# latentnetworks/vimure

Hardware: AMD Instinct MI355X
Metric: CAVI iterations/sec (L=4 N=2000 M=200 K=2 synthetic, mutuality on) (higher is better)
Workload: dtype f64

## Files before the change

include/vimure_hip.h:

```cpp
#ifndef VIMURE_HIP_H
#define VIMURE_HIP_H

#include <stdint.h>

#ifdef __cplusplus
extern "C" {
#endif

typedef struct vmr_ctx* vmr_handle;

enum {
  VMR_OK = 0,
  VMR_EINVAL = -1,
  VMR_EHIP = -2,
  VMR_ENAN = -3,
  VMR_ESTATE = -4
};

enum { VMR_STEP_GAMMA = 0, VMR_STEP_PHI = 1, VMR_STEP_RHO = 2, VMR_STEP_NU = 3 };

enum { VMR_READ_RHO_MAX = 0, VMR_READ_RHO_MEAN = 1, VMR_READ_THRESHOLD = 2 };

enum {
  VMR_KERNEL_GAMMA_MASK = 0,
  VMR_KERNEL_GAMMA_COUNTS = 1,
  VMR_KERNEL_PHI = 2,
  VMR_KERNEL_RHO = 3,
  VMR_KERNEL_ELBO = 4,
  VMR_KERNEL_FINALIZE = 5,
  VMR_KERNEL_RHO_ELBO = 6,
  VMR_KERNEL_RHO_NOSTORE = 7,
  VMR_KERNEL_COUNT = 8
};

int vmr_create(vmr_handle* out, int device, int L, int N, int M, int K, int mutuality,
               const uint8_t* X, const uint8_t* R, int data_on_device, double eps);

int vmr_create_coo(vmr_handle* out, int device, int L, int N, int M, int K, int mutuality,
                   int64_t nx, const int32_t* xl, const int32_t* xi, const int32_t* xj, const int32_t* xm, const int32_t* xv,
                   int64_t nr, const int32_t* rl, const int32_t* ri, const int32_t* rj, const int32_t* rm,
                   int data_on_device, double eps);

void vmr_destroy(vmr_handle h);

const char* vmr_last_error(vmr_handle h);

int vmr_data_stats(vmr_handle h, double* sum_x, uint8_t* coverage);

int vmr_set_priors(vmr_handle h, const double* alpha_theta, const double* beta_theta,
                   const double* alpha_lambda, const double* beta_lambda,
                   double alpha_eta, double beta_eta);

int vmr_set_state(vmr_handle h, const double* gamma_shp, const double* gamma_rte,
                  const double* phi_shp, const double* phi_rte, double nu_shp, double nu_rte,
                  const double* pr_rho, int pr_rho_on_device);

int vmr_draw_pr_rho(vmr_handle h, int nblk, const int64_t* tie_cuts, const uint32_t* mt_keys, const int32_t* mt_pos,
                    double bias0, int undirected, double* out, int out_on_device);

int vmr_step(vmr_handle h, int n_iters, double* elbo_out);

int vmr_fit_loop(vmr_handle h, int max_iter, double tol, int decision, int cap, int* n_rows, int* row_iter, double* row_elbo,
                 double* row_runtime, int* row_reached, double* elbo, int* iters, int* converged);

int vmr_fit_loop_batch(vmr_handle* hs, int n, int max_iter, double tol, int decision, int cap, int* n_rows, int* row_iter,
                       double* row_elbo, double* row_runtime, int* row_reached, double* elbo, int* iters, int* converged, int* rc);

int vmr_elbo(vmr_handle h, double* out);

int vmr_sweep_local(vmr_handle h, int want_elbo, double* out3);
int vmr_commit_nu(vmr_handle h, double nu_partial_total);

int vmr_sweep_local_dev(vmr_handle h, int want_elbo, double* out3_dev);
int vmr_commit_nu_dev(vmr_handle h, const double* nu_partial_total_dev);
void* vmr_stream(vmr_handle h);

int vmr_sub_step(vmr_handle h, int which);

int vmr_get_state(vmr_handle h, double* gamma_shp, double* gamma_rte, double* phi_shp,
                  double* phi_rte, double* nu_shp, double* nu_rte, double* rho);

int vmr_snapshot(vmr_handle h);
int vmr_restore(vmr_handle h);

int vmr_readout(vmr_handle h, int method, double threshold, void* out, int out_on_device);

int vmr_sample(vmr_handle h, uint64_t seed, int n_trials, uint8_t* out, int out_on_device);

int vmr_mean_poisson_size(vmr_handle h, int layer, uint64_t* n);
int vmr_mean_poisson(vmr_handle h, int layer, uint64_t n, int32_t* sl, int32_t* si, int32_t* sj, int32_t* sm,
                     double* vals, int out_on_device);

int vmr_report_auc(vmr_handle h, int layer, double* auc, uint64_t* n_pos, uint64_t* n_neg);

int vmr_sample_stats(vmr_handle h, uint64_t seed, int n_samples, int n_trials, const uint8_t* y_ref, int y_ref_on_device,
                     uint64_t* counts, int32_t* deg_out, int32_t* deg_in);

int vmr_expected_stats(vmr_handle h, double* out);

#define VMR_PPC_NSTAT 6
int vmr_ppc_replicates(vmr_handle h, int n_rep, uint64_t seed_y, uint64_t seed_x, int n_trials, const double* theta,
                       const double* lambda, const double* eta, uint64_t* counts, uint64_t* by_reporter);
int vmr_ppc_observed(vmr_handle h, uint64_t* counts, uint64_t* by_reporter);

enum { VMR_EDGE_REPORTED = 1, VMR_EDGE_INFERRED = 2 };
int vmr_edge_table_size(vmr_handle h, int method, double threshold, int select, int layer, uint64_t* n);
int vmr_edge_table(vmr_handle h, int method, double threshold, int select, int layer, uint64_t n,
                   int32_t* sl, int32_t* si, int32_t* sj,
                   uint8_t* y, double* prob, double* mean,
                   uint32_t* n_rep, uint64_t* total, uint32_t* n_mask, uint32_t* ego, uint32_t* alter,
                   uint8_t* y_T, uint32_t* n_rep_T, uint64_t* total_T, int out_on_device);

int vmr_get_geometric(vmr_handle h, double* g_theta, double* g_lambda, double* g_nu, double* g_nu_cache);

int vmr_sync(vmr_handle h);

int vmr_profile(vmr_handle h, int enable);
int vmr_profile_read(vmr_handle h, int kernel_class, double* total_ms, int64_t* launches);

int vmr_kernel_bytes(vmr_handle h, int kernel_class, double* bytes);

int vmr_data_format(vmr_handle h, int* sparse, uint64_t* nnz);

int vmr_mask_format(vmr_handle h, int* lists, uint64_t* listed);

int vmr_sweep_shape(vmr_handle h, int* passes, int* lds_levels, uint64_t* far_reports);

int vmr_generate_y(int device, int L, int N, int K, int C, const double* w, const int32_t* grp, uint64_t seed, uint8_t* Y_dev);
int vmr_generate_x(int device, int L, int N, int M, const uint8_t* Y_dev, const double* lam_dev, const double* theta, double eta,
                   double lambda_diff, uint64_t seed, int self_reporter, uint8_t* X_dev);

const char* vmr_version(void);

#ifdef __cplusplus
}
#endif
#endif
```

vimure_amd/_lib.py:

```python
import ctypes as C
import os

HERE = os.path.dirname(os.path.abspath(__file__))
LIB_PATH = os.environ.get("VMR_LIB", os.path.join(HERE, "libvimure_hip.so"))

VMR_OK, VMR_EINVAL, VMR_EHIP, VMR_ENAN, VMR_ESTATE = 0, -1, -2, -3, -4
STEP_GAMMA, STEP_PHI, STEP_RHO, STEP_NU = 0, 1, 2, 3
KERNEL_GAMMA_MASK, KERNEL_GAMMA_COUNTS, KERNEL_PHI, KERNEL_RHO, KERNEL_ELBO, KERNEL_FINALIZE, KERNEL_RHO_ELBO, KERNEL_RHO_NOSTORE = range(8)
READ_RHO_MAX, READ_RHO_MEAN, READ_THRESHOLD = 0, 1, 2
PPC_NSTAT = 6
EDGE_REPORTED, EDGE_INFERRED = 1, 2
PPC_STAT_NAMES = ["n_pos", "total", "sumsq", "mutual", "ties_reported", "ties_agreed"]
KERNEL_NAMES = ["gamma_mask", "gamma_counts", "phi", "rho", "elbo", "finalize", "rho_elbo", "rho_nostore"]

_dp = C.POINTER(C.c_double)
_u8p = C.c_void_p

SIGNATURES = {
    "vmr_create": (C.c_int, [C.POINTER(C.c_void_p), C.c_int, C.c_int, C.c_int, C.c_int, C.c_int, C.c_int,
                             _u8p, _u8p, C.c_int, C.c_double]),
    "vmr_create_coo": (C.c_int, [C.POINTER(C.c_void_p), C.c_int, C.c_int, C.c_int, C.c_int, C.c_int, C.c_int,
                                 C.c_int64, C.c_void_p, C.c_void_p, C.c_void_p, C.c_void_p, C.c_void_p,
                                 C.c_int64, C.c_void_p, C.c_void_p, C.c_void_p, C.c_void_p, C.c_int, C.c_double]),
    "vmr_destroy": (None, [C.c_void_p]),
    "vmr_last_error": (C.c_char_p, [C.c_void_p]),
    "vmr_data_stats": (C.c_int, [C.c_void_p, _dp, C.c_void_p]),
    "vmr_set_priors": (C.c_int, [C.c_void_p, C.c_void_p, C.c_void_p, C.c_void_p, C.c_void_p, C.c_double, C.c_double]),
    "vmr_set_state": (C.c_int, [C.c_void_p, C.c_void_p, C.c_void_p, C.c_void_p, C.c_void_p, C.c_double, C.c_double,
                                C.c_void_p, C.c_int]),
    "vmr_draw_pr_rho": (C.c_int, [C.c_void_p, C.c_int, C.c_void_p, C.c_void_p, C.c_void_p, C.c_double, C.c_int, C.c_void_p, C.c_int]),
    "vmr_step": (C.c_int, [C.c_void_p, C.c_int, _dp]),
    "vmr_elbo": (C.c_int, [C.c_void_p, _dp]),
    "vmr_fit_loop": (C.c_int, [C.c_void_p, C.c_int, C.c_double, C.c_int, C.c_int, C.POINTER(C.c_int), C.c_void_p, C.c_void_p,
                               C.c_void_p, C.c_void_p, _dp, C.POINTER(C.c_int), C.POINTER(C.c_int)]),
    "vmr_fit_loop_batch": (C.c_int, [C.POINTER(C.c_void_p), C.c_int, C.c_int, C.c_double, C.c_int, C.c_int, C.c_void_p, C.c_void_p, C.c_void_p,
                                     C.c_void_p, C.c_void_p, C.c_void_p, C.c_void_p, C.c_void_p, C.c_void_p]),
    "vmr_sub_step": (C.c_int, [C.c_void_p, C.c_int]),
    "vmr_sweep_local": (C.c_int, [C.c_void_p, C.c_int, _dp]),
    "vmr_commit_nu": (C.c_int, [C.c_void_p, C.c_double]),
    "vmr_sweep_local_dev": (C.c_int, [C.c_void_p, C.c_int, C.c_void_p]),
    "vmr_commit_nu_dev": (C.c_int, [C.c_void_p, C.c_void_p]),
    "vmr_stream": (C.c_void_p, [C.c_void_p]),
    "vmr_sample": (C.c_int, [C.c_void_p, C.c_uint64, C.c_int, C.c_void_p, C.c_int]),
    "vmr_sample_stats": (C.c_int, [C.c_void_p, C.c_uint64, C.c_int, C.c_int, C.c_void_p, C.c_int, C.c_void_p, C.c_void_p, C.c_void_p]),
    "vmr_expected_stats": (C.c_int, [C.c_void_p, C.c_void_p]),
    "vmr_ppc_replicates": (C.c_int, [C.c_void_p, C.c_int, C.c_uint64, C.c_uint64, C.c_int, C.c_void_p, C.c_void_p, C.c_void_p,
                                     C.c_void_p, C.c_void_p]),
    "vmr_ppc_observed": (C.c_int, [C.c_void_p, C.c_void_p, C.c_void_p]),
    "vmr_get_state": (C.c_int, [C.c_void_p] + [C.c_void_p] * 7),
    "vmr_get_geometric": (C.c_int, [C.c_void_p, C.c_void_p, C.c_void_p, C.c_void_p, C.c_void_p]),
    "vmr_sync": (C.c_int, [C.c_void_p]),
    "vmr_readout": (C.c_int, [C.c_void_p, C.c_int, C.c_double, C.c_void_p, C.c_int]),
    "vmr_mean_poisson_size": (C.c_int, [C.c_void_p, C.c_int, C.POINTER(C.c_uint64)]),
    "vmr_mean_poisson": (C.c_int, [C.c_void_p, C.c_int, C.c_uint64, C.c_void_p, C.c_void_p, C.c_void_p, C.c_void_p, C.c_void_p,
                                   C.c_int]),
    "vmr_report_auc": (C.c_int, [C.c_void_p, C.c_int, _dp, C.POINTER(C.c_uint64), C.POINTER(C.c_uint64)]),
    "vmr_edge_table_size": (C.c_int, [C.c_void_p, C.c_int, C.c_double, C.c_int, C.c_int, C.POINTER(C.c_uint64)]),
    "vmr_edge_table": (C.c_int, [C.c_void_p, C.c_int, C.c_double, C.c_int, C.c_int, C.c_uint64] + [C.c_void_p] * 14 + [C.c_int]),
    "vmr_snapshot": (C.c_int, [C.c_void_p]),
    "vmr_restore": (C.c_int, [C.c_void_p]),
    "vmr_profile": (C.c_int, [C.c_void_p, C.c_int]),
    "vmr_profile_read": (C.c_int, [C.c_void_p, C.c_int, _dp, C.POINTER(C.c_int64)]),
    "vmr_kernel_bytes": (C.c_int, [C.c_void_p, C.c_int, _dp]),
    "vmr_data_format": (C.c_int, [C.c_void_p, C.POINTER(C.c_int), C.POINTER(C.c_uint64)]),
    "vmr_mask_format": (C.c_int, [C.c_void_p, C.POINTER(C.c_int), C.POINTER(C.c_uint64)]),
    "vmr_sweep_shape": (C.c_int, [C.c_void_p, C.POINTER(C.c_int), C.POINTER(C.c_int), C.POINTER(C.c_uint64)]),
    "vmr_generate_y": (C.c_int, [C.c_int, C.c_int, C.c_int, C.c_int, C.c_int, C.c_void_p, C.c_void_p, C.c_uint64, C.c_void_p]),
    "vmr_generate_x": (C.c_int, [C.c_int, C.c_int, C.c_int, C.c_int, C.c_void_p, C.c_void_p, C.c_void_p, C.c_double, C.c_double,
                                 C.c_uint64, C.c_int, C.c_void_p]),
    "vmr_version": (C.c_char_p, []),
}

_lib = None


def load():
    global _lib
    if _lib is not None:
        return _lib
    if not os.path.exists(LIB_PATH):
        raise RuntimeError(
            f"{LIB_PATH} is missing: the HIP engine has not been built. Run `python -m vimure_amd.build` "
            "(needs hipcc, --offload-arch=gfx950). vimure_amd has no CPU fallback.")
    try:
        import torch
    except ImportError:
        pass
    lib = C.CDLL(LIB_PATH)
    for name, (res, args) in SIGNATURES.items():
        if os.environ.get("VMR_LIB_LAX") and not hasattr(lib, name):
            continue
        fn = getattr(lib, name)
        fn.restype = res
        fn.argtypes = args
    _lib = lib
    return lib
```

vimure_amd/csrc/sorted_lists.hip:

```cpp
#include "sweep_sl.h"

__global__ __launch_bounds__(256) void k_sl_keys(const unsigned* __restrict__ cnt, unsigned* __restrict__ keys, unsigned* __restrict__ vals, size_t T) {
  for (size_t t = (size_t)blockIdx.x * 256 + threadIdx.x; t < T; t += (size_t)gridDim.x * 256) { keys[t] = cnt[t]; vals[t] = (unsigned)t; }
}
__global__ __launch_bounds__(256) void k_sl_level_keys(unsigned* __restrict__ keys, const unsigned* __restrict__ rpl, const unsigned* __restrict__ E,
                                                       size_t T, unsigned rows0, int nb) {
  for (size_t t = (size_t)blockIdx.x * 256 + threadIdx.x; t < T; t += (size_t)gridDim.x * 256) {
    const unsigned r0 = rpl[t], n = rpl[t + 1] - r0;
    unsigned n1 = 0;
    for (unsigned r = 0; r < n; ++r) n1 += SL_YM(E[(size_t)r0 + r]) >= rows0 ? 1u : 0u;
    keys[t] = (n << nb) | n1;
  }
}
__global__ __launch_bounds__(256) void k_sl_steps(const unsigned* __restrict__ keys_sorted, const unsigned* __restrict__ vals_sorted,
                                                  unsigned* __restrict__ sz, unsigned* __restrict__ perm, size_t T, size_t NS, int nb) {
  for (size_t q = (size_t)blockIdx.x * 256 + threadIdx.x; q < NS * 64; q += (size_t)gridDim.x * 256) {
    perm[q] = q < T ? vals_sorted[q] : 0xffffffffu;
    if ((q & 63) == 0) sz[q >> 6] = 64u * (keys_sorted[q] >> nb);
  }
  if (blockIdx.x == 0 && threadIdx.x == 0) sz[NS] = 0u;
}
__global__ __launch_bounds__(256) void k_sl_place(const unsigned* __restrict__ perm, const unsigned* __restrict__ rpl ,
                                                  const unsigned* __restrict__ rsl, const unsigned* __restrict__ Ein,
                                                  unsigned* __restrict__ Eout, const unsigned* __restrict__ Ein2, unsigned* __restrict__ Eout2,
                                                  unsigned* __restrict__ syl, size_t T, size_t NS, int Mp) {
  const int lane = threadIdx.x & 63;
  for (size_t s = (size_t)blockIdx.x * 4 + (threadIdx.x >> 6); s < NS; s += (size_t)gridDim.x * 4) {
    const unsigned t = perm[s * 64 + lane];
    const bool ok = t != 0xffffffffu;
    const unsigned r0 = ok ? rpl[t] : 0u, n = ok ? rpl[t + 1] - r0 : 0u;
    const unsigned ea = rsl[s], R = (rsl[s + 1] - ea) >> 6;
    unsigned rot = 0;
    if (n > 1) { unsigned hsh = t * 0x9E3779B1u; hsh ^= hsh >> 15; hsh *= 0x85EBCA77u; hsh ^= hsh >> 13; rot = hsh % n; }
    unsigned ymx = 0;
    for (unsigned r = 0; r < R; ++r) {
      unsigned q = r + rot;
      if (q >= n) q -= n;
      const unsigned e = n > r ? Ein[(size_t)r0 + q] : 0u;
      Eout[(size_t)ea + r * 64 + lane] = e;
      if (Ein2) Eout2[(size_t)ea + r * 64 + lane] = n > r ? Ein2[(size_t)r0 + q] : 0u;
      ymx = max(ymx, (Ein2 ? e : SL_YM(e)) / (unsigned)Mp);
    }
#pragma unroll
    for (int o2 = 32; o2 > 0; o2 >>= 1) ymx = max(ymx, (unsigned)__shfl_xor((int)ymx, o2, 64));
    if (lane == 0) syl[s] = ymx;
  }
}

template <class V>
__global__ __launch_bounds__(256) void k_sl_gather(const unsigned* __restrict__ perm, const V* __restrict__ in, V* __restrict__ out,
                                                   size_t T, size_t NS, int L) {
  for (size_t q = (size_t)blockIdx.x * 256 + threadIdx.x; q < (size_t)L * T; q += (size_t)gridDim.x * 256) {
    const size_t l = q / T, pos = q - l * T;
    out[q] = in[l * T + perm[l * NS * 64 + pos]];
  }
}
__global__ __launch_bounds__(256) void k_sl_rows(const unsigned* __restrict__ perm, const double* __restrict__ in, double* __restrict__ out,
                                                 size_t T, size_t NS, int L, int K, int to_pos) {
  const size_t n = (size_t)L * T * K;
  for (size_t q = (size_t)blockIdx.x * 256 + threadIdx.x; q < n; q += (size_t)gridDim.x * 256) {
    const size_t row = q / K, k = q - row * K, l = row / T, pos = row - l * T;
    const size_t t = perm[l * NS * 64 + pos];
    if (to_pos) out[q] = in[(l * T + t) * K + k]; else out[(l * T + t) * K + k] = in[q];
  }
}

int sl_permute_u8(vmr_ctx* h, const uint8_t* in, uint8_t* out) {
  const Geo& g = h->g;
  const size_t T = (size_t)g.N * g.N, NS = (T + 63) / 64;
  hipLaunchKernelGGL(k_sl_gather<uint8_t>, dim3((unsigned)std::min<size_t>(8192, (g.L * T + 255) / 256)), dim3(256), 0, h->stream, h->perm, in, out, T, NS, g.L);
  CK(hipGetLastError());
  return VMR_OK;
}
int sl_permute_u32(vmr_ctx* h, const unsigned* in, unsigned* out) {
  const Geo& g = h->g;
  const size_t T = (size_t)g.N * g.N, NS = (T + 63) / 64;
  hipLaunchKernelGGL(k_sl_gather<unsigned>, dim3((unsigned)std::min<size_t>(8192, (g.L * T + 255) / 256)), dim3(256), 0, h->stream, h->perm, in, out, T, NS, g.L);
  CK(hipGetLastError());
  return VMR_OK;
}
int sl_permute_rows(vmr_ctx* h, const double* in, double* out, bool to_pos) {
  const Geo& g = h->g;
  const size_t T = (size_t)g.N * g.N, NS = (T + 63) / 64, n = (size_t)g.L * T * g.K;
  hipLaunchKernelGGL(k_sl_rows, dim3((unsigned)std::min<size_t>(16384, (n + 255) / 256)), dim3(256), 0, h->stream, h->perm, in, out, T, NS, g.L, g.K, to_pos ? 1 : 0);
  HIPCHK(h, hipGetLastError());
  return VMR_OK;
}

int sl_place_entries(vmr_ctx* h, unsigned* rp, const std::vector<unsigned long long>& nl, unsigned* etmp_all, unsigned* etmp2_all, const SlFill* fill) {
  Geo& g = h->g;
  const int L = g.L;
  const size_t T = (size_t)g.N * g.N, n = T + 1, NS = (T + 63) / 64;
  unsigned *keys = nullptr, *keys2 = nullptr, *vals = nullptr, *vals2 = nullptr, *bsum = nullptr, *etmp = nullptr, *etmp2 = nullptr;
  void* tmp = nullptr;
  const bool wide = g.wide != 0;
  auto cleanup = [&]() { void* p[] = {keys, keys2, vals, vals2, bsum, etmp, etmp2, tmp}; for (void* q : p) if (q) (void)hipFree(q); };
#define CKS(call) do { hipError_t e_ = (call); if (e_ != hipSuccess) { g_create_err = std::string(#call) + ": " + hipGetErrorString(e_); (void)hipGetLastError(); cleanup(); return VMR_EHIP; } } while (0)
  if (T >= 0x7fffffffull) return fail(nullptr, VMR_EINVAL, "more than 2^31 ties in one layer");
  CKS(hipMalloc(&keys, T * 4)); CKS(hipMalloc(&keys2, T * 4)); CKS(hipMalloc(&vals, T * 4)); CKS(hipMalloc(&vals2, T * 4));
  CKS(hipMalloc(&bsum, (std::max(n, NS + 1) + 2047) / 2048 * 4));
  CKS(hipMalloc(&h->rs, (size_t)L * (NS + 1) * 4));
  CKS(hipMalloc(&h->perm, (size_t)L * NS * 64 * 4));
  CKS(hipMalloc(&h->sy, (size_t)L * NS * 4));
  size_t tb = 0;
  int bits = 1;
  while (bits < 32 && (1ull << bits) <= (unsigned long long)g.M) ++bits;
  const bool level_keys_ok = !wide && g.mut && 2 * bits <= 30 && !h->opt.no_level_sort;
  CKS(hipcub::DeviceRadixSort::SortPairsDescending(nullptr, tb, keys, keys2, vals, vals2, (int)T, 0, level_keys_ok ? 2 * bits : bits, h->stream));
  CKS(hipMalloc(&tmp, tb ? tb : 8));
  const unsigned tgrid = (unsigned)std::min<size_t>(8192, (T + 255) / 256), sgrid = (unsigned)std::min<size_t>(8192, (NS + 3) / 4);
  if (!etmp_all) {
    unsigned long long nlmax = 0;
    for (int l = 0; l < L; ++l) nlmax = std::max(nlmax, nl[l]);
    CKS(hipMalloc(&etmp, ((size_t)nlmax + 64) * 4));
    if (wide) CKS(hipMalloc(&etmp2, ((size_t)nlmax + 64) * 4));
  }
  unsigned long long off1 = 0;
  for (int l = 0; l < L; ++l) {
    unsigned* rpl = rp + (size_t)l * n;
    unsigned* rsl = h->rs + (size_t)l * (NS + 1);
    const bool by_level = level_keys_ok && (double)nl[l] > (double)SL_PF * (double)T;
    const int nb = by_level ? bits : 0;
    int rc;
    hipLaunchKernelGGL(k_sl_keys, dim3(tgrid), dim3(256), 0, h->stream, rpl, keys, vals, T);
    if (by_level) {
      if ((rc = scan_u32(h, rpl, bsum, n))) { cleanup(); return rc; }
      if (!etmp_all) (*fill)(l, rpl, etmp, etmp2);
      hipLaunchKernelGGL(k_sl_level_keys, dim3(tgrid), dim3(256), 0, h->stream, keys, rpl, etmp_all ? etmp_all + off1 : etmp, T, (unsigned)g.Mp, nb);
    }
    CKS(hipcub::DeviceRadixSort::SortPairsDescending(tmp, tb, keys, keys2, vals, vals2, (int)T, 0, bits + nb, h->stream));
    hipLaunchKernelGGL(k_sl_steps, dim3((unsigned)std::min<size_t>(8192, (NS * 64 + 255) / 256)), dim3(256), 0, h->stream, keys2, vals2, rsl,
                       h->perm + (size_t)l * NS * 64, T, NS, nb);
    CKS(hipGetLastError());
    if ((rc = scan_u32(h, rsl, bsum, NS + 1)) || (!by_level && (rc = scan_u32(h, rpl, bsum, n)))) { cleanup(); return rc; }
    off1 += nl[l];
  }
  CKS(hipStreamSynchronize(h->stream));
  std::vector<unsigned> slots(L);
  for (int l = 0; l < L; ++l) CKS(hipMemcpy(&slots[l], h->rs + (size_t)l * (NS + 1) + NS, 4, hipMemcpyDeviceToHost));
  std::vector<unsigned long long> eb(L);
  h->n_slots = 0;
  for (int l = 0; l < L; ++l) {
    eb[l] = h->n_slots; h->n_slots += slots[l];
    if ((double)slots[l] < (double)nl[l]) { cleanup(); return fail(nullptr, VMR_EINVAL, "more than 2^32 report slots in one layer"); }
  }
  CKS(hipMalloc(&h->ebase, (size_t)L * 8));
  CKS(hipMemcpy(h->ebase, eb.data(), (size_t)L * 8, hipMemcpyHostToDevice));
  CKS(hipMalloc(&h->E, ((size_t)h->n_slots + SL_SLACK) * 4));
  CKS(hipMemsetAsync(h->E + h->n_slots, 0, (size_t)SL_SLACK * 4, h->stream));
  if (wide) {
    CKS(hipMalloc(&h->EX, ((size_t)h->n_slots + SL_SLACK) * 4));
    CKS(hipMemsetAsync(h->EX + h->n_slots, 0, (size_t)SL_SLACK * 4, h->stream));
  }
  unsigned long long off = 0;
  for (int l = 0; l < L; ++l) {
    unsigned* src = etmp_all ? etmp_all + off : etmp;
    unsigned* src2 = wide ? (etmp_all ? etmp2_all + off : etmp2) : nullptr;
    if (!etmp_all) (*fill)(l, rp + (size_t)l * n, etmp, etmp2);
    hipLaunchKernelGGL(k_sl_place, dim3(sgrid), dim3(256), 0, h->stream, h->perm + (size_t)l * NS * 64, rp + (size_t)l * n,
                       h->rs + (size_t)l * (NS + 1), src, h->E + eb[l], src2, wide ? h->EX + eb[l] : nullptr, h->sy + (size_t)l * NS, T, NS, g.Mp);
    off += nl[l];
  }
  CKS(hipGetLastError());
  CKS(hipStreamSynchronize(h->stream));
#undef CKS
  cleanup();
  return VMR_OK;
}

#define SL_DECL(K_) __attribute__((weak)) int vmr_sl_launch_k##K_(vmr_ctx* h, int mode, const SlShape& sh, SlArgs& a);
SL_DECL(2) SL_DECL(3) SL_DECL(4) SL_DECL(5) SL_DECL(6) SL_DECL(7) SL_DECL(8)
#define SL_DECLB(K_) __attribute__((weak)) int vmr_sl_launch_batch_k##K_(vmr_ctx* h, hipStream_t st, int mode, int allfull, const SlUnit* units, const int* blk_unit, int nblocks, int tpb, size_t smem);
SL_DECLB(2) SL_DECLB(3) SL_DECLB(4) SL_DECLB(5) SL_DECLB(6) SL_DECLB(7) SL_DECLB(8)
sl_launch_batch_fn vmr_sl_batch_launcher(int K) {
  switch (K) {
    case 2: return vmr_sl_launch_batch_k2; case 3: return vmr_sl_launch_batch_k3; case 4: return vmr_sl_launch_batch_k4; case 5: return vmr_sl_launch_batch_k5;
    case 6: return vmr_sl_launch_batch_k6; case 7: return vmr_sl_launch_batch_k7; case 8: return vmr_sl_launch_batch_k8;
    default: return nullptr;
  }
}
sl_launch_fn vmr_sl_launcher(int K) {
  switch (K) {
    case 2: return vmr_sl_launch_k2; case 3: return vmr_sl_launch_k3; case 4: return vmr_sl_launch_k4; case 5: return vmr_sl_launch_k5;
    case 6: return vmr_sl_launch_k6; case 7: return vmr_sl_launch_k7; case 8: return vmr_sl_launch_k8;
    default: return nullptr;
  }
}
```

vimure_amd/csrc/sweep_sl.h:

```cpp
#ifndef VMR_SWEEP_SL_H
#define VMR_SWEEP_SL_H

#include "vmr_internal.h"
#include <functional>

#define SL_YM(e) ((e) & 0xfffffu)
#define SL_INR(e) (((e) >> 20) & 1u)
#define SL_X(e) ((e) >> 21)
#define SL_XMAX 2047u
#define SL_YM_ROWS (1u << 20)
#define SL_PF 8
#ifndef SL_PFW
#define SL_PFW 8
#endif
constexpr int sl_pf(int K) { return K <= 2 ? SL_PF : SL_PFW; }
#define SL_SLACK (64 * 64)

struct SlArgs {
  const unsigned* E; const unsigned* rs; const unsigned long long* ebase; const unsigned* perm;
  const unsigned* sy;
  const uint8_t* cls;
  const unsigned* Qt;
  const uint64_t* Rb; const unsigned* rq; const unsigned short* Rm; const unsigned long long* rbase;
  const unsigned* rm2;
  double* rho; const double* logpr;
  const double* par; double* slotR; const double* lutg; double* Hg; double* slotF; double* slotA;
  int Gl;
  int do_hist;
  int yt, hc;
  int sum_a;
  double* nu_acc; double* elbo_dev; int commit_nu;
  int nu_stale;
  unsigned long long* det;
  int lp0;
  int farl;
  double* h0s;
  const unsigned* x0p;
  int lv0r;
  const unsigned* Ez;
  int elbo_cur;
  const double* lpd; const double* lpb;
#ifdef SL_DEBUG
  unsigned long long* dbg_t;
#endif
};

struct SlShape { int tpb, yt, hc; size_t smem; };
struct SlUnit { SlArgs a; Geo g; int blk0, nblk; };

#ifndef SL_LIGHT_UPD_K
#define SL_LIGHT_UPD_K 2
#endif
constexpr bool sl_light(int K, bool elbo, bool allfull, bool update) { return !elbo && allfull && (K <= SL_LIGHT_UPD_K || (!update && K <= 4)); }
#ifndef SL_ELBO3_K
#define SL_ELBO3_K 2
#endif
#ifndef SL_ELBO3
#define SL_ELBO3 1
#endif
constexpr int sl_tpb_max(int K, bool elbo, bool allfull, bool update = true) {
  return elbo ? ((SL_ELBO3 && K <= SL_ELBO3_K) ? 768 : (K <= 4 ? 512 : 256)) : (sl_light(K, elbo, allfull, update) ? 1024 : (K <= 3 ? 768 : (K <= 7 ? 512 : 256)));
}
constexpr int sl_tpb_max_b(int K, bool elbo, bool allfull) { return elbo ? sl_tpb_max(K, true, allfull) : (K <= 2 ? 768 : (K <= 7 ? 512 : 256)); }
constexpr int sl_wpe_b(int K, bool elbo, bool allfull) { return elbo ? ((SL_ELBO3 && K <= SL_ELBO3_K) ? 3 : (K <= 4 ? 2 : 1)) : (K <= 2 ? 3 : (K <= 7 ? 2 : 1)); }
constexpr int sl_wpe(int K, bool elbo, bool allfull, bool update = true) {
  return elbo ? ((SL_ELBO3 && K <= SL_ELBO3_K) ? 3 : (K <= 4 ? 2 : 1)) : (sl_light(K, elbo, allfull, update) ? 4 : (K <= 3 ? 3 : (K <= 7 ? 2 : 1)));
}

static inline size_t sl_smem(const Geo& g, int yt, int hc, bool update, bool elbo, bool hist) {
  const size_t lb = (size_t)g.Mp * g.K * 8;
  return (update ? (size_t)yt * lb : 0) + (hist ? (size_t)hc * lb : 0) + (size_t)g.Mp * 8 * (update ? 2 : 1) +
         (size_t)g.W * 8 + 128 + (g.ml ? lb + (size_t)g.Mp * 8 : 0) + (size_t)(64 + (elbo ? 256 : 0)) * 8 + 16;
}

typedef int (*sl_launch_fn)(vmr_ctx* h, int mode, const SlShape& sh, SlArgs& a);
sl_launch_fn vmr_sl_launcher(int K);
typedef int (*sl_launch_batch_fn)(vmr_ctx* h, hipStream_t st, int mode, int allfull, const SlUnit* units, const int* blk_unit, int nblocks,
                                  int tpb, size_t smem);
sl_launch_batch_fn vmr_sl_batch_launcher(int K);

typedef std::function<void(int l, const unsigned* rpl, unsigned* etmp, unsigned* etmp2)> SlFill;
int sl_place_entries(vmr_ctx* h, unsigned* rp, const std::vector<unsigned long long>& nl, unsigned* etmp_all, unsigned* etmp2_all, const SlFill* fill);
int sl_permute_u8(vmr_ctx* h, const uint8_t* in, uint8_t* out);
int sl_permute_u32(vmr_ctx* h, const unsigned* in, unsigned* out);
int sl_permute_rows(vmr_ctx* h, const double* in, double* out, bool to_pos);

#endif
```

vimure_amd/csrc/sweep_sl.hip:

```cpp
#include "sweep_sl.h"

#ifndef VMR_K
#error "compile with -DVMR_K=<number of categories>"
#endif
#ifndef SL_WPE
#define SL_WPE sl_wpe(2, false, true)
#endif

template <int K>
struct StepIn {
  double v[K];
  double w[K];
  unsigned cls, qt, tie;
  unsigned x0;
  unsigned e[sl_pf(K)];
};

template <int R> struct RC { static constexpr int value = R; };
template <class V> __device__ __forceinline__ const V* at_bytes(const V* p, unsigned off) {
  return reinterpret_cast<const V*>(reinterpret_cast<const char*>(p) + off);
}
template <class V> __device__ __forceinline__ V* at_bytes(V* p, unsigned off) {
  return reinterpret_cast<V*>(reinterpret_cast<char*>(p) + off);
}
__device__ __forceinline__ double rcp_nr2(double d) {
  double r = __builtin_amdgcn_rcp(d);
  r = fma(fma(-d, r, 1.0), r, r);
  return fma(fma(-d, r, 1.0), r, r);
}
#define SL_INL __attribute__((always_inline))
#ifndef SL_BATCH2
#define SL_BATCH2 8
#endif
template <int K> struct Batch { static constexpr int value = K <= 2 ? SL_BATCH2 : (K <= 4 ? 4 : 2); };

template <int K, bool UPDATE, bool ELBO, bool ALLFULL, bool STORE = true, bool DET = false, bool LPD = false>
__device__ __forceinline__ void sweep_body(const SlArgs& a, const Geo& g, const unsigned bx, const unsigned gx) {
  extern __shared__ __align__(16) unsigned char smem[];
  constexpr int PFK = sl_pf(K);
  constexpr bool LV0 = !UPDATE && !ELBO && !DET;
  constexpr bool LV0R = UPDATE && K >= 3;
  const int tid = threadIdx.x, lane = tid & 63, nthr = (int)blockDim.x;
  const int wv = __builtin_amdgcn_readfirstlane(tid >> 6), nw = nthr >> 6;
  const int Mp = g.Mp;
  const unsigned ytm = UPDATE ? (unsigned)a.yt * (unsigned)Mp : 0u;
  const unsigned hcm = a.do_hist ? (unsigned)a.hc * (unsigned)Mp : 0u;
  size_t off = 0;
  double* F = reinterpret_cast<double*>(smem + off); off += (size_t)ytm * K * 8;
  const int nHc = (int)hcm * K;
  double* Hc = reinterpret_cast<double*>(smem + off); off += (size_t)nHc * 8;
  double* Gth = reinterpret_cast<double*>(smem + off); off += (size_t)Mp * 8;
  double* Lth = reinterpret_cast<double*>(smem + off); off += UPDATE ? (size_t)Mp * 8 : 0;
  double* As = reinterpret_cast<double*>(smem + off); off += a.sum_a ? (size_t)Mp * K * 8 : 0;
  double* wsum = reinterpret_cast<double*>(smem + off); off += (size_t)g.W * 8;
  double* red = reinterpret_cast<double*>(smem + off); off += 16 * 8;
  double* xt = reinterpret_cast<double*>(smem + off); off += 64 * 8;
  double* lt = reinterpret_cast<double*>(smem + off); off += ELBO ? 256 * 8 : 0;
  double* EthL = reinterpret_cast<double*>(smem + off); off += a.rq ? (size_t)Mp * 8 : 0;
  const ParOff o = par_off(g.L, g.Mp, g.K);
  const int l = (int)bx / a.Gl, gb = (int)bx - l * a.Gl;
#ifdef SL_DEBUG
  unsigned long long* dbt = a.dbg_t ? a.dbg_t + ((size_t)bx * nw + wv) * 8 : nullptr;
  if (dbt && lane == 0) dbt[0] = wall_clock64();
#endif
  const size_t T = (size_t)g.N * g.N;
  const long long NS = (long long)((T + 63) / 64);
  const double gnu = a.par[o.sc + ((UPDATE || a.elbo_cur) ? SC_G_NU : SC_G_NU_STALE)];
  bool gz = false;
  for (int m = tid; m < Mp; m += nthr) {
    const double gv = a.par[o.G_th + (size_t)l * Mp + m];
    Gth[m] = gv;
    if (LV0 || LV0R) gz = gz || (m < g.M && gv == 0.0);
    if (UPDATE) Lth[m] = a.par[o.l_th + (size_t)l * Mp + m];
  }
  for (int q = tid; q < nHc; q += nthr) Hc[q] = 0.0;
  if (a.sum_a) for (int q = tid; q < Mp * K; q += nthr) As[q] = 0.0;
  if (a.rq) for (int m = tid; m < Mp; m += nthr) EthL[m] = m < g.M ? a.par[o.E_th + (size_t)l * Mp + m] : 0.0;
  if (UPDATE || ELBO) sp_math_tables(xt, lt, tid, nthr, ELBO);
  const double* lut = a.lutg + (size_t)l * g.W * 256;
  for (int w = tid; w < g.W; w += nthr) {
    double v = 0.0;
    for (int n = 0; n < 16; ++n) v += lut[(w * 16 + n) * 16 + 15];
    wsum[w] = v;
  }
  double Ela[K], Gla[K], Lla[K];
#pragma unroll
  for (int k = 0; k < K; ++k) { Ela[k] = a.par[o.E_la + l * K + k]; Gla[k] = a.par[o.G_la + l * K + k]; Lla[k] = a.par[o.l_la + l * K + k]; if (LV0 || LV0R) gz = gz || Gla[k] == 0.0; }
  const double eps = g.eps;
  const double sc_h = DET ? __builtin_amdgcn_ldexp(1.0, g.det_sh) : 0.0, sc_r = DET ? __builtin_amdgcn_ldexp(1.0, g.det_shr) : 0.0;
  const double sc_a = DET ? __builtin_amdgcn_ldexp(1.0, DET_SH_A) : 0.0;
  auto fxm = [](double v, double scale) SL_INL -> unsigned long long {
    return (unsigned long long)(__double_as_longlong(fma(v, scale, 6755399441055744.0)) - 0x4338000000000000ll);
  };
  auto lds_add = [&](double* p, double v, double scale) SL_INL {
    if (DET) atomicAdd(reinterpret_cast<unsigned long long*>(p), fxm(v, scale)); else atomicAdd(p, v);
  };
  const float rcp_mp = 1.0f / (float)Mp, hrcp_mp = 0.5f * rcp_mp;
  auto row_level = [&](unsigned ym) SL_INL -> unsigned { return (unsigned)__builtin_fmaf((float)ym, rcp_mp, hrcp_mp); };
  const double lp0_0 = log(1.0 + eps), lp0_k = log(eps);
  double e_lin = 0.0, e_q = 0.0, e_log = 0.0;
  double accF[K], acc0[K];
#pragma unroll
  for (int k = 0; k < K; ++k) { accF[k] = 0.0; acc0[k] = 0.0; }
  unsigned long long ie_lin = 0ull, ie_q = 0ull, ie_log = 0ull, iaccF[K];
#pragma unroll
  for (int k = 0; k < K; ++k) iaccF[k] = 0ull;
  double* Hl = a.Hg + ((size_t)l * NH + (gb % NH)) * g.Y * Mp * K;
  auto det_H = [&]() SL_INL { return a.det + (size_t)l * g.Y * Mp * K; };
  auto det_A = [&]() SL_INL { return a.det + (size_t)g.L * g.Y * Mp * K + (size_t)l * g.W * 64 * K; };
  auto det_F = [&]() SL_INL { return a.det + (size_t)g.L * g.Y * Mp * K + (size_t)g.L * g.W * 64 * K + (size_t)l * K; };
  auto det_R = [&]() SL_INL { return a.det + (size_t)g.L * g.Y * Mp * K + (size_t)g.L * g.W * 64 * K + (size_t)g.L * K; };
  const unsigned* rsl = a.rs + (size_t)l * (NS + 1);
  const unsigned* syl = a.sy + (size_t)l * NS;
  const unsigned* El = a.E + a.ebase[l];
  const unsigned* pl = (a.rm2 ? a.rm2 : a.perm) + (size_t)l * NS * 64;
  const uint8_t* cl = ALLFULL ? nullptr : a.cls + (size_t)l * T;
  const unsigned* Ql = a.Qt ? a.Qt + (size_t)l * T : nullptr;
  const uint64_t* Rl = a.Rb ? a.Rb + (size_t)l * T * g.W : nullptr;
  double* rl = a.rho + (size_t)l * T * K;
  double* rho_slack = a.rho + (size_t)g.L * T * K;
  const double* lpl = a.logpr + (size_t)l * T * K;
  constexpr bool LPDV = LPD && K == 2 && UPDATE && !ELBO;
  const double* lpdl = LPDV ? a.lpd + (size_t)l * T : nullptr;
  const double lpb0 = (K == 2 && UPDATE) ? a.lpb[2 * l] : 0.0, lpb1 = (K == 2 && UPDATE) ? a.lpb[2 * l + 1] : 0.0;
  const unsigned* rql = a.rq ? a.rq + (size_t)l * (T + 1) : nullptr;
  const unsigned short* Rml = a.rq ? a.Rm + a.rbase[l] : nullptr;
  const unsigned lim_y = UPDATE ? (a.do_hist ? (unsigned)min(a.yt, a.hc) : (unsigned)a.yt) : (a.do_hist ? (unsigned)a.hc : 0xffffffffu);
  const unsigned lim1 = (UPDATE && a.yt < g.Y) ? (unsigned)a.yt : 0xffffffffu;
  const unsigned lim2 = (a.do_hist && a.hc < g.Y) ? (unsigned)a.hc : 0xffffffffu;

  const long long Gl_ = a.Gl;
  unsigned* tick = reinterpret_cast<unsigned*>(smem + off); off += 16;
  if (tid == 0) { tick[0] = 2u * (unsigned)nw; tick[1] = 0u; }
  auto step_of = [&](unsigned t) SL_INL -> long long { return (long long)gb + (long long)t * Gl_; };
  auto draw = [&]() SL_INL -> long long {
    unsigned t = 0u;
    if (lane == 0) t = atomicAdd(tick, 1u);
    return step_of((unsigned)__builtin_amdgcn_readfirstlane((int)t));
  };
  long long s = step_of((unsigned)wv), sn = step_of((unsigned)(nw + wv));
  unsigned ea = 0;
  int R = 0;
  unsigned ymax = 0;
  unsigned rgv = 0;
  StepIn<K> P;

  const unsigned lane4 = (unsigned)lane * 4u, laneK8 = (unsigned)lane * (unsigned)(K * 8);
  const unsigned T32 = (unsigned)T;
  auto fetch_range = [&](long long st) SL_INL {
    const unsigned ra = rsl[st + (lane < 1 ? 0 : 1)], ry = syl[st];
    rgv = lane == 2 ? ry : ra;
  };
  auto fetch_tie = [&](StepIn<K>& d, long long st, const bool lp_const = false) SL_INL {
    const size_t row0 = (size_t)st * 64;
    const bool ok = (unsigned)row0 + (unsigned)lane < T32;
    d.qt = 0u; d.tie = 0u;
    if (ALLFULL) d.cls = ok ? 1u : 0u;
    else {
      const unsigned c = (unsigned)*at_bytes(cl + row0, (unsigned)lane);
      d.cls = ok ? c : 0u;
      d.tie = *at_bytes(pl + row0, lane4);
    }
    if (ELBO && Ql) d.qt = *at_bytes(Ql + row0, lane4);
    d.x0 = 0u;
    if (LV0 && a.x0p) d.x0 = *at_bytes(a.x0p + (size_t)l * NS * 64 + row0, lane4);
#pragma unroll
    for (int k = 0; k < K; ++k) { d.v[k] = 0.0; d.w[k] = 0.0; }
    if (LPDV) {
      if (lp_const) d.v[0] = lp0_k - lp0_0;
      else d.v[0] = *at_bytes(lpdl + row0, (unsigned)lane * 8u);
    } else if (UPDATE || ELBO) {
      if (lp_const) {
#pragma unroll
        for (int k = 0; k < K; ++k) d.v[k] = k == 0 ? lp0_0 : lp0_k;
      } else load_k<K>(at_bytes(lpl + row0 * K, laneK8), d.v);
    }
    if (!UPDATE && a.do_hist != 2) load_k<K>(at_bytes(static_cast<const double*>(rl) + row0 * K, laneK8), d.w);
  };
  auto fetch_ent = [&](StepIn<K>& d, unsigned base, auto cntc) SL_INL {
    constexpr int CNT = decltype(cntc)::value;
    const unsigned* pe = El + base;
#pragma unroll
    for (int j = 0; j < CNT; ++j) d.e[j] = *at_bytes(pe + j * 64, lane4);
  };

  if (s < NS) {
    ea = rsl[s];
    R = (int)((rsl[s + 1] - ea) >> 6);
    ymax = syl[s];
    fetch_range(sn < NS ? sn : s);
    fetch_tie(P, s);
    fetch_ent(P, ea, RC<PFK>{});
  }
#ifdef SL_DEBUG
  if (dbt && lane == 0) dbt[4] = wall_clock64();
#endif
  __builtin_amdgcn_s_waitcnt(0x0F70);
  bool lv0_off = false;
  if (LV0 || LV0R) lv0_off = __syncthreads_or(gz ? 1 : 0) != 0;
  else __syncthreads();
#ifdef SL_DEBUG
  if (dbt && lane == 0) dbt[5] = wall_clock64();
#endif
  const double gnu_f = a.par[o.sc + (a.nu_stale ? SC_G_NU_STALE : SC_G_NU)];
  if (UPDATE) {
    for (int q = tid; q < (int)ytm; q += nthr) {
      const int y = q / Mp, m = q - y * Mp;
#pragma unroll
      for (int k = 0; k < K; ++k) F[q * K + k] = (m < g.M) ? f_entry(g.mut, Lth[m], Gth[m], Lla[k], Gla[k], gnu_f, y) : 0.0;
    }
    __syncthreads();
  }
  double Tfull = 0.0;
  for (int w = 0; w < g.W; ++w) Tfull += wsum[w];
#ifdef SL_DEBUG
  if (dbt && lane == 0) dbt[1] = wall_clock64();
#endif

  auto add_lists = [&](unsigned t, bool on, const double (&rr)[K]) SL_INL {
    if (a.rm2) {
#pragma unroll
      for (int h_ = 0; h_ < 2; ++h_) {
        const unsigned m = h_ ? (t >> 16) : (t & 0xffffu);
        const bool v = on && m != 0xffffu;
        const unsigned long long vm = __ballot(v);
        if (vm == 0ull) continue;
        const int m0 = __builtin_amdgcn_readlane((int)m, __builtin_ctzll(vm));
        if (__all(!v || (int)m == m0)) {
#pragma unroll
          for (int k = 0; k < K; ++k) {
            const double sm_ = wave_sum(v ? rr[k] : 0.0);
            if (lane == 0) lds_add(&As[m0 * K + k], sm_, sc_a);
          }
        } else if (v) {
#pragma unroll
          for (int k = 0; k < K; ++k) lds_add(&As[m * K + k], rr[k], sc_a);
        }
      }
      return;
    }
    unsigned q0 = 0, q1 = 0;
    if (on) { q0 = rql[t]; q1 = rql[t + 1]; }
    for (unsigned i = 0;; ++i) {
      const bool v = q0 + i < q1;
      const unsigned long long vm = __ballot(v);
      if (vm == 0ull) break;
      const int m = v ? (int)Rml[q0 + i] : -1;
      const int m0 = __builtin_amdgcn_readlane(m, __builtin_ctzll(vm));
      if (__all(!v || m == m0)) {
#pragma unroll
        for (int k = 0; k < K; ++k) {
          const double sm_ = wave_sum(v ? rr[k] : 0.0);
          if (lane == 0) lds_add(&As[m0 * K + k], sm_, sc_a);
        }
      } else if (v) {
#pragma unroll
        for (int k = 0; k < K; ++k) lds_add(&As[m * K + k], rr[k], sc_a);
      }
    }
  };
  auto mask_sum = [&](unsigned cls, unsigned tie) SL_INL -> double {
    if (ALLFULL) return Tfull;
    double Tt = 0.0;
    if (cls == 1u) Tt = Tfull;
    else if (cls == 2u && a.rm2) {
      const unsigned m0 = tie & 0xffffu, m1 = tie >> 16;
      Tt = (m0 != 0xffffu ? EthL[m0] : 0.0) + (m1 != 0xffffu ? EthL[m1] : 0.0);
    } else if (cls == 2u && rql) {
      const unsigned q0 = rql[tie], q1 = rql[tie + 1];
      for (unsigned q = q0; q < q1; ++q) Tt += EthL[Rml[q]];
    } else if (cls == 2u) {
      const uint64_t* rwt = Rl + (size_t)tie * g.W;
      for (int w = 0; w < g.W; ++w) {
        uint64_t bits = rwt[w];
        if (bits == ~0ull) { Tt += wsum[w]; continue; }
        for (int n = 0; bits != 0; ++n, bits >>= 4) Tt += lut[((w * 16 + n) << 4) + (unsigned)(bits & 15u)];
      }
    }
    return Tt;
  };
  const double gnu_cur = a.par[o.sc + SC_G_NU];
  auto w2_at = [&](unsigned ym, int k) SL_INL -> double {
    const unsigned y = row_level(ym);
    const double z2 = gnu_cur * (double)y, den = Gth[ym - y * (unsigned)Mp] * Gla[k] + z2;
    return (y == 0u || den == 0.0) ? 0.0 : z2 / den;
  };
  auto f_far = [&](unsigned ym, double (&f)[K]) SL_INL {
    const unsigned y = row_level(ym);
    const unsigned m = ym - y * (unsigned)Mp;
    const double lt = Lth[m], gt = Gth[m];
#pragma unroll
    for (int k = 0; k < K; ++k) f[k] = f_entry(g.mut, lt, gt, Lla[k], Gla[k], gnu_f, (int)y);
  };
  auto elbo_inner = [&](unsigned ent, const double (&er)[2]) SL_INL -> double {
    const unsigned ym = SL_YM(ent);
    const unsigned y = row_level(ym);
    const double z2 = gnu * (double)y, gt = Gth[ym - y * (unsigned)Mp];
    const double inner = fma(gt, er[0], z2 * er[1]);
    return (SL_INR(ent) ? inner : 0.0) + eps;
  };
  auto walk1_near = [&](const unsigned* e, auto npc, double (&U)[K]) SL_INL {
    constexpr int NP = decltype(npc)::value, BT = Batch<K>::value;
#pragma unroll
    for (int j0 = 0; j0 < NP; j0 += BT) {
      double f[BT][K];
#pragma unroll
      for (int u = 0; u < BT; ++u) {
        if (j0 + u < NP) {
#pragma unroll
          for (int k = 0; k < K; ++k) f[u][k] = F[SL_YM(e[j0 + u]) * K + k];
        }
      }
#pragma unroll
      for (int u = 0; u < BT; ++u) {
        if (j0 + u < NP) {
          const double dx = (double)SL_X(e[j0 + u]);
#pragma unroll
          for (int k = 0; k < K; ++k) U[k] = fma(dx, f[u][k], U[k]);
        }
      }
    }
  };
  auto walk2_near = [&](const unsigned* e, auto npc, const double (&r)[K], const double (&er)[2]) SL_INL {
#ifndef SL_LG
#define SL_LG 2
#endif
    constexpr int NP = decltype(npc)::value, LG = SL_LG;
#pragma unroll
    for (int j0 = 0; j0 < NP; j0 += LG) {
      double in_[LG];
#pragma unroll
      for (int u = 0; u < LG; ++u) {
        if (j0 + u < NP) {
          const unsigned ym = SL_YM(e[j0 + u]);
          const double dx = (double)SL_X(e[j0 + u]);
          if (a.do_hist) {
#pragma unroll
            for (int k = 1; k < K; ++k) lds_add(&Hc[(unsigned)k * hcm + ym], dx * r[k], sc_h);
          }
          if (ELBO) in_[u] = elbo_inner(e[j0 + u], er);
        }
      }
      if (ELBO) {
#pragma unroll
        for (int u = 0; u < LG; ++u) if (j0 + u < NP) {
          const double term = (double)SL_X(e[j0 + u]) * log_tab(in_[u], lt);
          if (DET) ie_log += fxm(term, sc_r); else e_log += term;
        }
        __builtin_amdgcn_sched_barrier(0);
      }
    }
  };
  auto deficit = [&](unsigned ent, double dfc) SL_INL {
    lds_add(&Hc[SL_YM(ent)], (double)SL_X(ent) * dfc, sc_h);
  };
  auto compute = [&](auto rct, const StepIn<K>& cur, const size_t row0, const bool act, const unsigned ea_c, const int Rr, const unsigned sy_word) SL_INL {
    const unsigned ymax = sy_word & 0xffffu, nf = a.farl ? sy_word >> 16 : 0x7fffffffu;
    const unsigned n1 = (LV0 && a.h0s && !lv0_off) ? sy_word >> 16 : 0x7fffffffu;
    constexpr int RCT = decltype(rct)::value;
    constexpr int NP = RCT < 0 ? PFK : RCT;
    const unsigned cls = cur.cls, qt = cur.qt, tie = cur.tie;
    const unsigned* pe = El + ea_c;
    auto rounds = [&](auto gbc, auto&& use, const int Rr) SL_INL {
      constexpr int GB = decltype(gbc)::value;
      unsigned rg[PFK];
#pragma unroll
      for (int i = 0; i < PFK; ++i) rg[i] = i < Rr ? cur.e[i] : 0u;
      for (int j0 = 0; j0 < Rr; j0 += PFK) {
#pragma unroll
        for (int gi = 0; gi < PFK; gi += GB) {
          unsigned c[GB];
#pragma unroll
          for (int u = 0; u < GB; ++u) {
            c[u] = rg[gi + u];
            const int jn = j0 + gi + u + PFK;
            rg[gi + u] = *at_bytes(jn < Rr ? pe + (size_t)jn * 64 : a.Ez, lane4);
          }
          if (j0 + gi < Rr) use(c, (unsigned)(j0 + gi));
        }
      }
    };
    double r[K], er[2] = {0.0, 0.0};
#pragma unroll
    for (int k = 0; k < K; ++k) r[k] = act ? cur.w[k] : 0.0;
    if (a.do_hist == 2) {
#pragma unroll
      for (int k = 0; k < K; ++k) r[k] = (k == 1) ? 1.0 : 0.0;
    }
    double Tt = 0.0;
    if (UPDATE || ELBO) Tt = mask_sum(cls, tie);
    double dfc = 0.0;
    bool irr = false;

    if (UPDATE) {
      double U[K];
#pragma unroll
      for (int k = 0; k < K; ++k) U[k] = 0.0;
#ifdef SL_DEBUG
      if (g.dbg & 16) {} else
#endif
      if (RCT >= 0) walk1_near(cur.e, RC<NP>{}, U);
      else {
        constexpr int GB = Batch<K>::value < 4 ? Batch<K>::value : 4;
        const unsigned n1u = (LV0R && a.lv0r && !lv0_off) ? sy_word >> 16 : 0x7fffffffu;
        double sl0 = 0.0, sx1 = 0.0;
        rounds(RC<GB>{}, [&](const unsigned (&c)[GB], const unsigned j) SL_INL {
          if (LV0R && j >= n1u) {
            double l0[GB];
#pragma unroll
            for (int u = 0; u < GB; ++u) l0[u] = Lth[SL_YM(c[u])];
#pragma unroll
            for (int u = 0; u < GB; ++u) { const double dx = (double)SL_X(c[u]); sl0 = fma(dx, l0[u], sl0); sx1 += dx; }
            return;
          }
          if (ymax < lim1 || j >= nf) { walk1_near(c, RC<GB>{}, U); return; }
          double f[GB][K];
          bool fr[GB];
#pragma unroll
          for (int u = 0; u < GB; ++u) {
            const unsigned ym = SL_YM(c[u]);
            fr[u] = ym >= ytm;
#pragma unroll
            for (int k = 0; k < K; ++k) f[u][k] = F[(fr[u] ? 0u : ym) * K + k];
          }
#pragma unroll
          for (int u = 0; u < GB; ++u) {
            const double dx = fr[u] ? 0.0 : (double)SL_X(c[u]);
#pragma unroll
            for (int k = 0; k < K; ++k) U[k] = fma(dx, f[u][k], U[k]);
          }
#pragma unroll
          for (int u = 0; u < GB; ++u) {
            if (__any(fr[u])) {
              if (fr[u]) {
                double ff[K];
                f_far(SL_YM(c[u]), ff);
                const double dx = (double)SL_X(c[u]);
#pragma unroll
                for (int k = 0; k < K; ++k) U[k] = fma(dx, ff[k], U[k]);
              }
            }
          }
        }, Rr);
        if (LV0R && a.lv0r && !lv0_off) {
#pragma unroll
          for (int k = 0; k < K; ++k) U[k] += fma(Lla[k], sx1, sl0);
        }
      }
      double aa[K];
      bool done = false;
      if (K == 2) {
        double c[K];
#pragma unroll
        for (int k = 0; k < K; ++k) c[k] = fma(-Tt, Ela[k], U[k]);
        const double d = ((LPDV ? cur.v[0] : cur.v[K - 1] - cur.v[0]) + c[K - 1]) - c[0];
        bool safe = fabs(c[0]) + lpb0 < 700.0 && fabs(c[K - 1]) + lpb1 < 700.0 && fabs(d) < 700.0;
        if (!__all(safe)) {
          double v[K];
#pragma unroll
          for (int k = 0; k < K; ++k) v[k] = cur.v[k];
          if (LPDV) load_k<K>(at_bytes(lpl + row0 * K, laneK8), v);
#pragma unroll
          for (int k = 0; k < K; ++k) aa[k] = v[k] + c[k];
          safe = fabs(aa[0]) < 700.0 && fabs(aa[K - 1]) < 700.0 && fabs(d) < 700.0;
        }
        if (__all(safe)) {
          const double e = exp_tab(d, xt);
          r[0] = rcp_nr2(1.0 + e);
          r[K - 1] = e * r[0];
          done = true;
        }
      } else {
#pragma unroll
        for (int k = 0; k < K; ++k) aa[k] = (cur.v[k] + U[k]) - Tt * Ela[k];
      }
      if (!done) {
        double sum = 0.0;
        bool tame = true;
#pragma unroll
        for (int k = 0; k < K; ++k) tame = tame && fabs(aa[k]) < 700.0;
        tame = __all(tame);
        if (tame) {
#pragma unroll
          for (int k = 0; k < K; ++k) r[k] = exp_tab(aa[k], xt);
        } else {
#pragma unroll
          for (int k = 0; k < K; ++k) r[k] = exp(aa[k]);
        }
#pragma unroll
        for (int k = 0; k < K; ++k) sum += r[k];
        if (sum > 0.0) {
#pragma unroll
          for (int k = 0; k < K; ++k) r[k] /= sum;
        }
        if (a.do_hist) {
          double sm = 0.0;
#pragma unroll
          for (int k = 0; k < K; ++k) sm += r[k];
          dfc = 1.0 - sm;
          if (fabs(dfc) <= 1e-14 || !act) dfc = 0.0;
          irr = __any(dfc != 0.0);
          if (irr && lane == 0) tick[1] = 1u;
        }
      }
      if (STORE) store_k<K>(act ? at_bytes(rl + row0 * K, laneK8) : at_bytes(rho_slack, laneK8), r);
      if (act && (ALLFULL || cls == 1u)) {
#pragma unroll
        for (int k = 0; k < K; ++k) { if (DET) iaccF[k] += fxm(r[k], sc_a); else accF[k] += r[k]; }
      }
      if (!ALLFULL && a.sum_a) add_lists(tie, act && cls == 2u, r);
    } else if (a.do_hist) {
      double sm = 0.0;
#pragma unroll
      for (int k = 0; k < K; ++k) sm += r[k];
      dfc = 1.0 - sm;
      if (fabs(dfc) <= 1e-14 || !act) dfc = 0.0;
      irr = __any(dfc != 0.0);
      if (irr && lane == 0) tick[1] = 1u;
      if (!ELBO && a.do_hist == 1 && act && (ALLFULL || cls == 1u)) {
#pragma unroll
        for (int k = 0; k < K; ++k) { if (DET) iaccF[k] += fxm(r[k], sc_a); else accF[k] += r[k]; }
      }
      if (!ALLFULL && !ELBO && a.sum_a) add_lists(tie, act && cls == 2u, r);
    }
    if (ELBO) {
#pragma unroll
      for (int k = 0; k < K; ++k) { const double ek = exp_tab(r[k], xt); er[0] = fma(ek, Gla[k], er[0]); er[1] += ek; }
    }
#ifdef SL_DEBUG
    if (g.dbg & 32) {} else
#endif
    if (a.do_hist || ELBO) {
      if (RCT >= 0) {
        walk2_near(cur.e, RC<NP>{}, r, er);
        if (irr) {
#pragma unroll
          for (int j = 0; j < NP; ++j) deficit(cur.e[j], dfc);
        }
      } else {
        const bool skip0 = LV0 && a.x0p != nullptr && a.do_hist == 1 && n1 != 0x7fffffffu && !irr;
        const int Rw = skip0 ? min(Rr, (int)n1) : Rr;
        double sx0 = skip0 ? (double)cur.x0 : 0.0;
        rounds(RC<1>{}, [&](const unsigned (&c1)[1], const unsigned j) SL_INL {
          const unsigned c = c1[0], ym = SL_YM(c), x = SL_X(c);
          const bool far_round = j < nf && lim2 != 0xffffffffu;
          const bool fr = far_round && ym >= hcm;
          const double dx = (double)x;
          if (LV0 && a.do_hist && j >= n1) {
            sx0 += dx;
            if (irr) lds_add(&Hc[ym], dx * dfc, sc_h);
          } else if (a.do_hist) {
            if (!fr) {
              if (!(skip0 && ym < (unsigned)Mp)) {
#pragma unroll
                for (int k = 1; k < K; ++k) lds_add(&Hc[(unsigned)k * hcm + ym], dx * r[k], sc_h);
              }
              if (irr) lds_add(&Hc[ym], dx * dfc, sc_h);
            }
            if (far_round && !a.farl && __any(fr)) {
              if (fr && x != 0u) {
                if (DET) {
                  unsigned long long* d0 = a.det;
                  asm volatile("" : "+s"(d0));
                  unsigned long long* d = d0 + (size_t)l * g.Y * Mp * K + (size_t)ym * K;
#pragma unroll
                  for (int k = 1; k < K; ++k) atomicAdd(&d[k], fxm((double)x * r[k], sc_h));
                  if (dfc != 0.0) atomicAdd(&d[0], fxm((double)x * dfc, sc_h));
                } else {
                  double* d = Hl + (size_t)ym * K;
#pragma unroll
                  for (int k = 1; k < K; ++k) atomicAdd(&d[k], (double)x * r[k]);
                  if (dfc != 0.0) atomicAdd(&d[0], (double)x * dfc);
                }
              }
              asm volatile("" ::: "memory");
            }
          }
          if (ELBO) { const double term = (double)x * log_tab(elbo_inner(c, er), lt); if (DET) ie_log += fxm(term, sc_r); else e_log += term; }
        }, Rw);
        if (LV0 && a.h0s && a.do_hist == 1 && act) {
#pragma unroll
          for (int k = 1; k < K; ++k) acc0[k] = fma(r[k], sx0, acc0[k]);
        }
      }
    }
    if (ELBO && act) {
      double sr = 0.0, se = 0.0, en = 0.0;
#pragma unroll
      for (int k = 0; k < K; ++k) {
        sr += r[k]; se += r[k] * Ela[k];
        en += r[k] * cur.v[k] - r[k] * log_tab(r[k] + eps, lt);
      }
      if (DET) { ie_lin += det_fx(en - se * Tt, g.det_shr); if (Ql) ie_q += det_fx(sr * (double)qt, g.det_shr); }
      else { e_lin += en - se * Tt; if (Ql) e_q += sr * (double)qt; }
    }
  };
  auto body = [&](auto rct) SL_INL {
    constexpr int RCT = decltype(rct)::value;
    constexpr int NP = RCT < 0 ? PFK : RCT;
    const size_t row0 = (size_t)s * 64;
    const bool act = (unsigned)row0 + (unsigned)lane < T32;
    const unsigned ea_c = ea;
    const int Rr = RCT < 0 ? R : RCT;
    const StepIn<K> cur = P;
    const long long s2 = sn, s3 = draw();
    const bool more = s2 < NS;
    const unsigned ea2 = more ? (unsigned)__builtin_amdgcn_readlane((int)rgv, 0) : ea_c;
    const int R2 = more ? (int)(((unsigned)__builtin_amdgcn_readlane((int)rgv, 1) - ea2) >> 6) : 0;
    const unsigned ym2 = more ? (unsigned)__builtin_amdgcn_readlane((int)rgv, 2) : 0u;
    fetch_range(s3 < NS ? s3 : s);
    fetch_tie(P, more ? s2 : s, RCT == 0 && a.lp0 != 0);
    if (RCT >= 0 || PFK <= 8) fetch_ent(P, ea2, RC<NP>{});
    else {
      const unsigned* pe = El + ea2;
#pragma unroll
      for (int j0 = 0; j0 < PFK; j0 += 8) {
        if (j0 == 0 || j0 < R2) {
#pragma unroll
          for (int j = j0; j < j0 + 8; ++j) P.e[j] = *at_bytes(pe + j * 64, lane4);
        }
      }
    }
    compute(rct, cur, row0, act, ea_c, Rr, ymax);
    constexpr int NST = (UPDATE && STORE) ? (K % 2 == 0 ? K / 2 : K) : 0;
    static_assert(NST <= 8, "vmcnt immediate below");
    if (RCT >= 0) __builtin_amdgcn_s_waitcnt(0x0F70 | NST);
    else __builtin_amdgcn_s_waitcnt(0x0F70);
    s = s2; sn = s3; ea = ea2; R = R2; ymax = ym2;
  };
  auto run = [&](auto rct) SL_INL {
    constexpr int RCT = decltype(rct)::value;
    do { body(rct); } while (s < NS && R == RCT && (ymax & 0xffffu) < lim_y);
  };
  while (s < NS) {
    if (R > SL_PF || (ymax & 0xffffu) >= lim_y) { body(RC<-1>{}); continue; }
    switch (R) {
      case 0: run(RC<0>{}); break;
      case 1: run(RC<1>{}); break;
      case 2: run(RC<2>{}); break;
      case 3: run(RC<3>{}); break;
      case 4: run(RC<4>{}); break;
      case 5: run(RC<5>{}); break;
      case 6: run(RC<6>{}); break;
      case 7: run(RC<7>{}); break;
      default: run(RC<8>{}); break;
    }
  }

#ifdef SL_DEBUG
  if (dbt && lane == 0) dbt[2] = wall_clock64();
#endif
  const bool nu_here = a.nu_acc && a.do_hist == 1;
  if (nu_here) asm volatile("s_waitcnt vmcnt(0)" ::: "memory");
  __syncthreads();
  if (nu_here) {
    double a0p = 0.0;
    for (int q = (tick[1] ? 0 : (int)hcm) + tid; q < nHc; q += nthr) {
      const double v = DET ? det_back(reinterpret_cast<const unsigned long long*>(Hc)[q], g.det_sh) : Hc[q];
      if (v != 0.0) {
        const int k = q / (int)hcm;
        const unsigned ym = (unsigned)(q - k * (int)hcm);
        a0p += ((k ? w2_at(ym, k) : 0.0) - w2_at(ym, 0)) * v;
      }
    }
    a0p = block_sum_n(a0p, red);
    if (tid == 0) {
      if (DET) atomicAdd(&det_R()[4], det_fx(a0p, g.det_sh)); else atomicAdd(&a.nu_acc[0], a0p);
    }
  }
#ifdef SL_DEBUG
  if (dbt && lane == 0) dbt[6] = wall_clock64();
#endif
  const int f0 = (nu_here && nw > 1) ? 64 : 0;
#ifdef SL_DEBUG
  if (g.dbg & 8) {} else
#endif
  if (a.do_hist && tid >= f0) {
    for (int q = (tick[1] ? 0 : (int)hcm) + tid - f0; q < nHc; q += nthr - f0) {
      if (DET) {
        const unsigned long long iv = reinterpret_cast<const unsigned long long*>(Hc)[q];
        if (iv != 0ull) { const int k = q / (int)hcm, ym = q - k * (int)hcm; atomicAdd(&det_H()[(size_t)ym * K + k], iv); }
        continue;
      }
      const double v = Hc[q];
      if (v != 0.0) {
        const int k = q / (int)hcm, ym = q - k * (int)hcm;
        atomicAdd(&Hl[(size_t)ym * K + k], v);
      }
    }
  }
  if (a.sum_a && tid >= f0) {
    double* out = a.slotA + ((size_t)l * NSLOT + (gb % NSLOT)) * (size_t)g.W * 64 * K;
    for (int q = tid - f0; q < g.M * K; q += nthr - f0) {
      if (DET) { const unsigned long long iv = reinterpret_cast<const unsigned long long*>(As)[q]; if (iv != 0ull) atomicAdd(&det_A()[q], iv); continue; }
      const double v = As[q];
      if (v != 0.0) atomicAdd(&out[q], v);
    }
  }
#ifdef SL_DEBUG
  if (dbt && lane == 0) dbt[7] = wall_clock64();
#endif
  if (nu_here) {
    __shared__ int nu_last;
    if (tid == 0) {
      asm volatile("s_waitcnt vmcnt(0)" ::: "memory");
      const double t = atomicAdd(&a.nu_acc[1], 1.0);
      nu_last = (t == (double)(gx - 1u));
      if (nu_last) __builtin_amdgcn_fence(__ATOMIC_ACQUIRE, "agent");
      asm volatile("s_waitcnt vmcnt(0)" ::: "memory");
    }
    __syncthreads();
    if (nu_last && a.farl) {
      if (tid == 0) a.nu_acc[1] = 0.0;
    } else if (nu_last) {
      double far = 0.0;
      const size_t hcs = (size_t)g.Y * Mp * K;
      const int y0 = max(1, a.hc);
      if (a.hc < g.Y) {
        for (int ll = 0; ll < g.L; ++ll) {
          const double* H0 = a.Hg + (size_t)ll * NH * hcs;
          const double* gthl = a.par + o.G_th + (size_t)ll * Mp;
          for (int it = y0 * Mp + tid; it < g.Y * Mp; it += nthr) {
            const int y = it / Mp, m = it - y * Mp;
            double v0[NH], vk[NH][K > 1 ? K - 1 : 1];
#pragma unroll
            for (int c = 0; c < NH; ++c) {
              v0[c] = H0[(size_t)c * hcs + (size_t)it * K];
#pragma unroll
              for (int k = 1; k < K; ++k) vk[c][k - 1] = H0[(size_t)c * hcs + (size_t)it * K + k];
            }
            if (DET) {
              const unsigned long long* hi = a.det + (size_t)ll * hcs + (size_t)it * K;
              v0[0] += det_back(hi[0], g.det_sh);
#pragma unroll
              for (int k = 1; k < K; ++k) vk[0][k - 1] += det_back(hi[k], g.det_sh);
            }
            double h_[K];
#pragma unroll
            for (int k = 0; k < K; ++k) h_[k] = 0.0;
#pragma unroll
            for (int c = 0; c < NH; ++c) {
              h_[0] += v0[c];
#pragma unroll
              for (int k = 1; k < K; ++k) h_[k] += vk[c][k - 1];
            }
            bool any = h_[0] != 0.0;
#pragma unroll
            for (int k = 1; k < K; ++k) any = any || h_[k] != 0.0;
            if (any && m < g.M) {
              const double z2 = gnu_cur * (double)y, gt = gthl[m];
              const double d0 = gt * a.par[o.G_la + ll * K] + z2, w0 = d0 == 0.0 ? 0.0 : z2 / d0;
              far -= w0 * h_[0];
#pragma unroll
              for (int k = 1; k < K; ++k) {
                const double dk = gt * a.par[o.G_la + ll * K + k] + z2;
                far += ((dk == 0.0 ? 0.0 : z2 / dk) - w0) * h_[k];
              }
            }
          }
        }
      }
      far = block_sum_n(far, red);
      if (tid == 0) {
        double tot = far;
        if (DET) { unsigned long long* dR = det_R(); tot += det_back(atomicAdd(&dR[4], 0ull), g.det_sh); dR[4] = 0ull; } else tot += atomicAdd(&a.nu_acc[0], 0.0);
        for (int ll = 0; ll < g.L; ++ll) tot += a.nu_acc[2 + ll];
        a.nu_acc[0] = 0.0; a.nu_acc[1] = 0.0;
        a.elbo_dev[1] = tot;
        if (a.commit_nu) {
          double* sc = const_cast<double*>(a.par) + o.sc;
          sc[SC_G_NU_STALE] = sc[SC_G_NU];
          sc[SC_NU_SHP] = sc[SC_A_ETA] + tot;
          sc[SC_G_NU] = exp(digamma_pos(sc[SC_NU_SHP]) - log(sc[SC_NU_RTE]));
          sc[SC_E_NU] = sc[SC_NU_SHP] / sc[SC_NU_RTE];
        }
      }
    }
  }
  auto wave_isum = [&](unsigned long long v) SL_INL -> unsigned long long {
#pragma unroll
    for (int o2 = 32; o2 > 0; o2 >>= 1) {
      const unsigned lo = (unsigned)__shfl_xor((int)(unsigned)v, o2, 64), hi = (unsigned)__shfl_xor((int)(unsigned)(v >> 32), o2, 64);
      v += ((unsigned long long)hi << 32) | lo;
    }
    return v;
  };
  if ((UPDATE || (!ELBO && a.do_hist == 1)) && a.slotF) {
#pragma unroll
    for (int k = 0; k < K; ++k) {
      if (DET) { const unsigned long long v = wave_isum(iaccF[k]); if (lane == 0 && v != 0ull) atomicAdd(&det_F()[k], v); continue; }
      double v = block_sum_n(accF[k], red);
      if (tid == 0) atomicAdd(&a.slotF[((size_t)l * NSLOT + (gb % NSLOT)) * K + k], v);
    }
  }
  if (LV0 && a.h0s && a.do_hist == 1) {
#pragma unroll
    for (int k = 1; k < K; ++k) {
      const double v = block_sum_n(acc0[k], red);
      if (tid == 0 && v != 0.0) atomicAdd(&a.h0s[((size_t)l * NSLOT + (gb % NSLOT)) * K + k], v);
    }
  }
  if (ELBO) {
    if (DET) {
      const unsigned long long v1 = wave_isum(ie_lin), v2 = wave_isum(ie_log), v3 = wave_isum(ie_q);
      if (lane == 0) { unsigned long long* dR = det_R(); atomicAdd(&dR[1], v1); atomicAdd(&dR[2], v2); atomicAdd(&dR[3], v3); }
    } else {
      double v1 = block_sum_n(e_lin, red);
      double v2 = block_sum_n(e_log, red);
      double v3 = block_sum_n(e_q, red);
      if (tid == 0) {
        double* out = a.slotR + (size_t)(bx % NSLOT) * 4;
        atomicAdd(&out[1], v1); atomicAdd(&out[2], v2); atomicAdd(&out[3], v3);
      }
    }
  }
#ifdef SL_DEBUG
  if (dbt && lane == 0) dbt[3] = wall_clock64();
#endif
}

#define SL_BOUNDS(K, UPDATE, ELBO, ALLFULL) \
  __launch_bounds__(sl_tpb_max(K, ELBO, ALLFULL, UPDATE), (K == 2 && !ELBO && ALLFULL) ? SL_WPE : sl_wpe(K, ELBO, ALLFULL, UPDATE))
template <int K, bool UPDATE, bool ELBO, bool ALLFULL, bool STORE = true, bool DET = false, bool LPD = false>
__global__ SL_BOUNDS(K, UPDATE, ELBO, ALLFULL) void k_sweep_sl(SlArgs a, Geo g) {
  sweep_body<K, UPDATE, ELBO, ALLFULL, STORE, DET, LPD>(a, g, blockIdx.x, gridDim.x);
}
template <int K, bool UPDATE, bool ELBO, bool ALLFULL, bool STORE = true, bool LPD = false>
__global__ __launch_bounds__(sl_tpb_max_b(K, ELBO, ALLFULL), sl_wpe_b(K, ELBO, ALLFULL)) void k_sweep_sl_b(const SlUnit* __restrict__ units, const int* __restrict__ blk_unit) {
  const SlUnit& u = units[blk_unit[blockIdx.x]];
  sweep_body<K, UPDATE, ELBO, ALLFULL, STORE, false, LPD>(u.a, u.g, blockIdx.x - (unsigned)u.blk0, (unsigned)u.nblk);
}

template <bool UPDATE, bool ELBO, bool ALLFULL, bool STORE = true, bool DET = false, bool LPD = false>
static int sl_launch_one_(vmr_ctx* h, const SlShape& sh, SlArgs& a) {
  constexpr int K = VMR_K;
  const Geo& g = h->g;
  const long long NS = ((long long)g.N * g.N + 63) / 64, nw = sh.tpb / 64;
  int rc = grid_per_layer(h, k_sweep_sl<K, UPDATE, ELBO, ALLFULL, STORE, DET, LPD>, sh.smem, &a.Gl, (NS + nw - 1) / nw, sh.tpb);
  if (rc) return rc;
#ifdef SL_DEBUG
  static unsigned long long* dbg_buf = nullptr;
  const char* tf = h->opt.debug_times[0] ? h->opt.debug_times : nullptr;
  const size_t nwv = (size_t)g.L * a.Gl * nw;
  a.dbg_t = nullptr;
  if (tf) {
    if (!dbg_buf) (void)hipMalloc(&dbg_buf, (size_t)1 << 22);
    if (nwv * 64 <= ((size_t)1 << 22)) a.dbg_t = dbg_buf;
  }
#endif
  hipLaunchKernelGGL((k_sweep_sl<K, UPDATE, ELBO, ALLFULL, STORE, DET, LPD>), dim3(g.L * a.Gl), dim3(sh.tpb), sh.smem, h->stream, a, g);
#ifdef SL_DEBUG
  if (a.dbg_t) {
    std::vector<unsigned long long> t(nwv * 8);
    (void)hipStreamSynchronize(h->stream);
    (void)hipMemcpy(t.data(), dbg_buf, nwv * 64, hipMemcpyDeviceToHost);
    if (FILE* f = fopen(tf, "a")) {
      fprintf(f, "launch %d%d hist %d waves %zu tpb %d\n", (int)UPDATE, (int)ELBO, a.do_hist, nwv, sh.tpb);
      for (size_t i = 0; i < nwv; ++i) fprintf(f, "%llu %llu %llu %llu %llu %llu %llu %llu\n", t[i * 8], t[i * 8 + 1], t[i * 8 + 2], t[i * 8 + 3], t[i * 8 + 4], t[i * 8 + 5], t[i * 8 + 6], t[i * 8 + 7]);
      fclose(f);
    }
  }
#endif
  return VMR_OK;
}

template <bool UPDATE, bool ELBO, bool ALLFULL, bool STORE = true, bool DET = false>
static int sl_launch_one(vmr_ctx* h, const SlShape& sh, SlArgs& a) {
  if (VMR_K == 2 && UPDATE && !ELBO && a.lpd) return sl_launch_one_<UPDATE, ELBO, ALLFULL, STORE, DET, VMR_K == 2 && UPDATE && !ELBO>(h, sh, a);
  return sl_launch_one_<UPDATE, ELBO, ALLFULL, STORE, DET>(h, sh, a);
}

#define SL_CAT2(a, b) a##b
#define SL_CAT(a, b) SL_CAT2(a, b)
int SL_CAT(vmr_sl_launch_k, VMR_K)(vmr_ctx* h, int mode, const SlShape& sh, SlArgs& a) {
  if (a.det) {
    if (a.cls == nullptr) {
      switch (mode) {
        case 0: return sl_launch_one<true, false, true, true, true>(h, sh, a);
        case 4: return sl_launch_one<true, false, true, false, true>(h, sh, a);
        case 1: return sl_launch_one<true, true, true, true, true>(h, sh, a);
        case 2: return sl_launch_one<false, true, true, true, true>(h, sh, a);
        default: return sl_launch_one<false, false, true, true, true>(h, sh, a);
      }
    }
    switch (mode) {
      case 0: return sl_launch_one<true, false, false, true, true>(h, sh, a);
      case 4: return sl_launch_one<true, false, false, false, true>(h, sh, a);
      case 1: return sl_launch_one<true, true, false, true, true>(h, sh, a);
      case 2: return sl_launch_one<false, true, false, true, true>(h, sh, a);
      default: return sl_launch_one<false, false, false, true, true>(h, sh, a);
    }
  }
  if (a.cls == nullptr) {
    switch (mode) {
      case 0: return sl_launch_one<true, false, true>(h, sh, a);
      case 1: return sl_launch_one<true, true, true>(h, sh, a);
      case 2: return sl_launch_one<false, true, true>(h, sh, a);
      case 4: return sl_launch_one<true, false, true, false>(h, sh, a);
      default: return sl_launch_one<false, false, true>(h, sh, a);
    }
  }
  switch (mode) {
    case 0: return sl_launch_one<true, false, false>(h, sh, a);
    case 1: return sl_launch_one<true, true, false>(h, sh, a);
    case 2: return sl_launch_one<false, true, false>(h, sh, a);
    case 4: return sl_launch_one<true, false, false, false>(h, sh, a);
    default: return sl_launch_one<false, false, false>(h, sh, a);
  }
}

template <bool UPDATE, bool ELBO, bool ALLFULL, bool STORE = true, bool LPD = false>
static int sl_launch_batch_one_(vmr_ctx* h, hipStream_t st, const SlUnit* units, const int* blk_unit, int nblocks, int tpb, size_t smem) {
  constexpr int K = VMR_K;
  if (smem > 48 * 1024)
    HIPCHK(h, hipFuncSetAttribute(reinterpret_cast<const void*>(k_sweep_sl_b<K, UPDATE, ELBO, ALLFULL, STORE, LPD>), hipFuncAttributeMaxDynamicSharedMemorySize, (int)smem));
  hipLaunchKernelGGL((k_sweep_sl_b<K, UPDATE, ELBO, ALLFULL, STORE, LPD>), dim3(nblocks), dim3(tpb), smem, st, units, blk_unit);
  return VMR_OK;
}
template <bool UPDATE, bool ELBO, bool ALLFULL, bool STORE = true>
static int sl_launch_batch_one(vmr_ctx* h, hipStream_t st, bool lpd, const SlUnit* units, const int* blk_unit, int nblocks, int tpb, size_t smem) {
  if (VMR_K == 2 && UPDATE && !ELBO && lpd) return sl_launch_batch_one_<UPDATE, ELBO, ALLFULL, STORE, VMR_K == 2 && UPDATE && !ELBO>(h, st, units, blk_unit, nblocks, tpb, smem);
  return sl_launch_batch_one_<UPDATE, ELBO, ALLFULL, STORE>(h, st, units, blk_unit, nblocks, tpb, smem);
}
int SL_CAT(vmr_sl_launch_batch_k, VMR_K)(vmr_ctx* h, hipStream_t st, int mode, int allfull, const SlUnit* units, const int* blk_unit, int nblocks,
                                          int tpb, size_t smem) {
  const bool lpd = h->lpd != nullptr;
  if (mode == 3) return allfull ? sl_launch_batch_one<false, false, true>(h, st, lpd, units, blk_unit, nblocks, tpb, smem)
                                : sl_launch_batch_one<false, false, false>(h, st, lpd, units, blk_unit, nblocks, tpb, smem);
  if (mode == 4) return allfull ? sl_launch_batch_one<true, false, true, false>(h, st, lpd, units, blk_unit, nblocks, tpb, smem)
                                : sl_launch_batch_one<true, false, false, false>(h, st, lpd, units, blk_unit, nblocks, tpb, smem);
  if (allfull) return mode ? sl_launch_batch_one<true, true, true>(h, st, lpd, units, blk_unit, nblocks, tpb, smem)
                           : sl_launch_batch_one<true, false, true>(h, st, lpd, units, blk_unit, nblocks, tpb, smem);
  return mode ? sl_launch_batch_one<true, true, false>(h, st, lpd, units, blk_unit, nblocks, tpb, smem)
              : sl_launch_batch_one<true, false, false>(h, st, lpd, units, blk_unit, nblocks, tpb, smem);
}
```

vimure_amd/csrc/vimure_hip.hip:

```cpp
#include "vmr_internal.h"
#include "sweep_sl.h"
#include "sweep_gen.h"
#include "sample_draw.h"

thread_local std::string g_create_err;



template <int SH>
__device__ __forceinline__ unsigned nz_flags16(uint4 v) {
  const unsigned M = 0x7f7f7f7fu;
  unsigned t0 = ((v.x & M) + M) | v.x, t1 = ((v.y & M) + M) | v.y;
  unsigned t2 = ((v.z & M) + M) | v.z, t3 = ((v.w & M) + M) | v.w;
  unsigned f = (t0 >> (7 - SH)) & (0x01010101u << SH);
  f |= (t1 >> (6 - SH)) & (0x02020202u << SH);
  f |= (t2 >> (5 - SH)) & (0x04040404u << SH);
  f |= (t3 >> (4 - SH)) & (0x08080808u << SH);
  return f;
}
__device__ __forceinline__ void flag_pos(int bit, int& chunk, int& byte) {
  const int lo = bit & 31;
  chunk = ((bit >> 5) << 1) | ((lo >> 2) & 1);
  byte = ((lo & 3) << 2) | (lo >> 3);
}
// ... 1421 lines not shown
    }
  }
  if (do_elbo) {
    for (int m = gs * TPB + threadIdx.x; m < g.M; m += FR_G * TPB) {
      const size_t q = (size_t)l * g.Mp + m;
      gt += gamma_elbo_term(par[o.a_th + q], par[o.b_th + q], par[o.g_shp + q], par[o.g_rte + q]);
    }
    if (gs == 0) {
      for (int k = threadIdx.x; k < g.K; k += TPB) {
        const int q = l * g.K + k;
        gt += gamma_elbo_term(par[o.a_la + q], par[o.b_la + q], par[o.p_shp + q], par[o.p_rte + q]);
      }
    }
  }
  a0 = block_sum(a0, red);
  gt = block_sum(gt, red);
  if (threadIdx.x == 0) {
    if (slots) { slots[2 * bx] = a0; slots[2 * bx + 1] = gt; __builtin_amdgcn_fence(__ATOMIC_RELEASE, "agent"); }
    else { atomicAdd(&fin[0], a0); atomicAdd(&fin[1], gt); }
    asm volatile("s_waitcnt vmcnt(0)" ::: "memory");
    const double t = atomicAdd(&fin[2], 1.0);
    last = (t == (double)(gx - 1));
  }
  __syncthreads();
  if (!last) return;
  double a1 = 0, a2 = 0, a3 = 0;
  if (g.gen && g.det) {
    if (threadIdx.x == 0) {
      unsigned long long* pi = reinterpret_cast<unsigned long long*>(slotR);
      unsigned long long s[6] = {0ull, 0ull, 0ull, 0ull, 0ull, 0ull};
      for (int q = 0; q < NSLOT; ++q) {
        const int w = q < NSLOT / 2 ? 0 : 3;
        for (int i = 1; i <= 3; ++i) { s[w + i - 1] += pi[q * 4 + i]; pi[q * 4 + i] = 0ull; }
        pi[q * 4] = 0ull;
      }
      a1 = det_back(s[0], g.det_shr) + det_back(s[3], g.det_shr + DET_SH2);
      a2 = det_back(s[1], g.det_shr) + det_back(s[4], g.det_shr + DET_SH2);
      a3 = det_back(s[2], g.det_shr) + det_back(s[5], g.det_shr + DET_SH2);
    }
  } else if (threadIdx.x < NSLOT) {
    double* ps = slotR + (size_t)threadIdx.x * 4;
    a1 = ps[1]; a2 = ps[2]; a3 = ps[3];
    ps[0] = ps[1] = ps[2] = ps[3] = 0.0;
  }
  a1 = block_sum(a1, red); a2 = block_sum(a2, red); a3 = block_sum(a3, red);
  if (threadIdx.x == 0) {
    if (slots) {
      __builtin_amdgcn_fence(__ATOMIC_ACQUIRE, "agent");
      a0 = 0.0; gt = 0.0;
      for (int q = 0; q < gx; ++q) { a0 += __builtin_nontemporal_load(&slots[2 * q]); gt += __builtin_nontemporal_load(&slots[2 * q + 1]); }
    } else {
      a0 = atomicAdd(&fin[0], 0.0);
      gt = atomicAdd(&fin[1], 0.0);
    }
    fin[0] = 0.0; fin[1] = 0.0; fin[2] = 0.0;
    if (do_nu && g.mut) {
      sc[SC_G_NU_STALE] = sc[SC_G_NU];
      sc[SC_NU_SHP] = sc[SC_A_ETA] + a0;
      sc[SC_G_NU] = exp(digamma_pos(sc[SC_NU_SHP]) - log(sc[SC_NU_RTE]));
      sc[SC_E_NU] = sc[SC_NU_SHP] / sc[SC_NU_RTE];
    }
    if (do_elbo) {
      double e = a1 + a2 - sc[SC_E_NU] * a3 + gt;
      e += gamma_elbo_term(sc[SC_A_ETA], sc[SC_B_ETA], sc[SC_NU_SHP], sc[SC_NU_RTE]);
      elbo_out[0] = e;
    }
    if (!skip_nu) elbo_out[1] = a0;
    elbo_out[2] = a1 + a2 + gt;
    elbo_out[3] = a3;
  }
}
__global__ __launch_bounds__(TPB) void k_fin_rho(double* par, double* Hg, const double* Cg, double* slotR, double* elbo_out,
                                                 double* fin, int do_nu, int do_elbo, int fold, int skip_nu, Geo g, double* slots) {
  fin_rho_body(par, Hg, Cg, slotR, elbo_out, fin, do_nu, do_elbo, fold, skip_nu, g, (int)blockIdx.x, (int)gridDim.x, slots);
}
__global__ __launch_bounds__(TPB) void k_fin_rho_b(const FinUnit* __restrict__ units, const int* __restrict__ blk_unit) {
  const FinUnit& u = units[blk_unit[blockIdx.x]];
  fin_rho_body(u.par, u.Hg, u.Cg, u.slotR, u.elbo, u.elbo + 4, 0, 1, 0, 1, u.g, (int)blockIdx.x - u.fr_blk0, u.fr_nblk);
}

__global__ void k_commit_nu(double* par, double nu_partial_total, const double* total_dev, Geo g) {
  const ParOff o = par_off(g.L, g.Mp, g.K);
  double* sc = par + o.sc;
  if (total_dev) nu_partial_total = total_dev[0];
  if (threadIdx.x == 0 && blockIdx.x == 0 && g.mut) {
    sc[SC_G_NU_STALE] = sc[SC_G_NU];
    sc[SC_NU_SHP] = sc[SC_A_ETA] + nu_partial_total;
    sc[SC_G_NU] = exp(digamma_pos(sc[SC_NU_SHP]) - log(sc[SC_NU_RTE]));
    sc[SC_E_NU] = sc[SC_NU_SHP] / sc[SC_NU_RTE];
  }
}

__global__ __launch_bounds__(256) void k_readout(const double* __restrict__ rho, void* __restrict__ out, size_t ties, int K,
                                                 int method, double threshold, const unsigned* __restrict__ perm, size_t T, size_t NS) {
  for (size_t q = (size_t)blockIdx.x * blockDim.x + threadIdx.x; q < ties; q += (size_t)gridDim.x * blockDim.x) {
    const double* r = rho + q * K;
    size_t t = q;
    if (perm) { const size_t l = q / T, pos = q - l * T; t = l * T + perm[l * NS * 64 + pos]; }
    if (method == VMR_READ_RHO_MAX) {
      int best = 0;
      double bv = r[0];
      for (int k = 1; k < K; ++k) if (r[k] > bv) { bv = r[k]; best = k; }
      reinterpret_cast<uint8_t*>(out)[t] = (uint8_t)best;
    } else if (method == VMR_READ_RHO_MEAN) {
      double m = 0.0;
      for (int k = 1; k < K; ++k) m += (double)k * r[k];
      reinterpret_cast<double*>(out)[t] = m;
    } else {
      reinterpret_cast<uint8_t*>(out)[t] = r[1] >= threshold ? 1 : 0;
    }
  }
}


__global__ __launch_bounds__(256) void k_sample(const double* __restrict__ rho, uint8_t* __restrict__ out, size_t ties, int K, int n_trials,
                                                unsigned long long seed, const unsigned* __restrict__ perm, size_t T, size_t NS) {
  for (size_t q = (size_t)blockIdx.x * blockDim.x + threadIdx.x; q < ties; q += (size_t)gridDim.x * blockDim.x) {
    const double* r = rho + q * K;
    size_t t = q;
    if (perm) { const size_t l = q / T, pos = q - l * T; t = l * T + perm[l * NS * 64 + pos]; }
    const int best = draw_tie<false>(r, K, n_trials, seed, t, nullptr);
    out[t] = (uint8_t)best;
  }
}


static size_t shmem_ct(const Geo& g) { return g.mut ? (size_t)g.Mp * g.K * 8 : 0; }
static size_t shmem_q() { return (size_t)(TPB / 64) * 64 * QCAP * 2; }
static size_t shmem_hc(const Geo& g) { return (size_t)g.hc * g.Mp * g.K * 8; }
static size_t shmem_hist(const Geo& g) {
  return (size_t)g.nt * g.stride + (size_t)g.nt * g.K * 8 + shmem_hc(g) + shmem_q() + 16;
}
static size_t shmem_rho(const Geo& g, bool update, bool elbo) {
  size_t n = (size_t)g.nt * g.stride + (size_t)g.nt * g.W * 8 + (size_t)g.W * 8 + (size_t)g.Mp * 8 + 64 + shmem_ct(g) +
             2 * (size_t)g.nt * g.K * 8 + shmem_q();
  if (update && !g.two_pass) n += shmem_hc(g);
  if (elbo) n += (size_t)g.Mp * 8 + (size_t)g.nt * 4;
  return n + 16;
}

#define SP_LDS_MAX (160 * 1024)

static SlShape sl_shape(const vmr_ctx* h, bool update, bool elbo, bool hist) {
  const Geo& g = h->g;
  SlShape s{std::max(64, std::min((update || elbo) ? h->sp_tpb : h->st_tpb, sl_tpb_max(g.K, elbo, h->all_full != 0, update)) & ~63), update ? g.yt : 0, hist ? g.hc : 0, 0};
  auto bytes = [&]() { return sl_smem(g, s.yt, s.hc, update, elbo, hist); };
  while (bytes() > SP_LDS_MAX && (s.yt > 0 || s.hc > 0)) { if (s.yt >= s.hc && s.yt > 0) --s.yt; else --s.hc; }
  s.smem = bytes();
  return s;
}
static SlArgs sl_args(const vmr_ctx* h, const SlShape& sh, int do_hist, int sum_a = 0) {
  return SlArgs{h->E, h->rs, h->ebase, h->perm, h->sy, h->cls_p, h->Qt_p, h->Rb, h->rq, h->Rm, h->rbase, h->rm2, h->rho, h->logpr, h->par, h->slotR,
                h->lutg, h->Hg, h->slotF, h->slotA, 1, do_hist, sh.yt, sh.hc, sum_a, nullptr, nullptr, 0, 0, nullptr, h->lp0 ? 1 : 0, h->g.farl, (do_hist == 1 && h->g.two_pass && sh.hc >= 1) ? h->h0s : nullptr, (do_hist == 1 && h->g.two_pass && sh.hc >= 1 && h->h0s) ? h->x0p : nullptr,
                (h->h0s && h->g.two_pass && !h->opt.no_lv0r) ? 1 : 0, h->E + h->n_slots, 0, h->lpd, h->lpb};
}
static int sl_launch(vmr_ctx* h, int mode, const SlShape& sh, SlArgs& a) {
  sl_launch_fn fn = vmr_sl_launcher(h->g.K);
  if (!fn) return fail(h, VMR_EINVAL, "this build of libvimure_hip.so holds no sweep kernel for this K");
  return fn(h, mode, sh, a);
}

#ifdef VMR_DEV
#define DISPATCH_K(K_, ...)                         \
  switch (K_) {                                     \
    case 2: { constexpr int KK = 2; __VA_ARGS__; } break; \
    default: break;                                 \
  }
#else
#define DISPATCH_K(K_, ...)                         \
  switch (K_) {                                     \
    case 2: { constexpr int KK = 2; __VA_ARGS__; } break; \
    case 3: { constexpr int KK = 3; __VA_ARGS__; } break; \
    case 4: { constexpr int KK = 4; __VA_ARGS__; } break; \
    case 5: { constexpr int KK = 5; __VA_ARGS__; } break; \
    case 6: { constexpr int KK = 6; __VA_ARGS__; } break; \
    case 7: { constexpr int KK = 7; __VA_ARGS__; } break; \
    case 8: { constexpr int KK = 8; __VA_ARGS__; } break; \
    default: break;                                 \
  }
#endif
#define DISPATCH_KP(K_, PF_, ...)                                     \
  switch (PF_) {                                                      \
    case 4: { constexpr int PP = 4; DISPATCH_K(K_, __VA_ARGS__); } break;   \
    case 8: { constexpr int PP = 8; DISPATCH_K(K_, __VA_ARGS__); } break;   \
    default: { constexpr int PP = 12; DISPATCH_K(K_, __VA_ARGS__); } break; \
  }



__global__ __launch_bounds__(256) void k_stat_slots(const unsigned* __restrict__ rsl, const unsigned* __restrict__ syl, size_t NS, unsigned long long* __restrict__ out) {
  unsigned long long v = 0;
  for (size_t s = (size_t)blockIdx.x * 256 + threadIdx.x; s < NS; s += (size_t)gridDim.x * 256) {
    const unsigned R = (rsl[s + 1] - rsl[s]) >> 6, n1 = syl[s] >> 16;
    v += 64ull * (unsigned long long)min(R, n1);
  }
  if (v) atomicAdd(out, v);
}
__global__ __launch_bounds__(256) void k_far_first(unsigned* __restrict__ E, const unsigned* __restrict__ rsl, unsigned* __restrict__ syl, size_t NS, unsigned rows_near,
                                                   unsigned* __restrict__ x0) {
  const int lane = threadIdx.x & 63;
  for (size_t s = (size_t)blockIdx.x * 4 + (threadIdx.x >> 6); s < NS; s += (size_t)gridDim.x * 4) {
    const unsigned ea = rsl[s], R = (rsl[s + 1] - ea) >> 6;
    unsigned* col = E + (size_t)ea + lane;
    unsigned f = 0;
    unsigned xs = 0;
    for (unsigned r = 0; r < R; ++r) {
      const unsigned e = col[(size_t)r * 64];
      if (e != 0u && SL_YM(e) >= rows_near) {
        if (f != r) { const unsigned o = col[(size_t)f * 64]; col[(size_t)f * 64] = e; col[(size_t)r * 64] = o; }
        ++f;
      } else xs += SL_X(e);
    }
    if (x0) x0[s * 64 + (unsigned)lane] = xs;
#pragma unroll
    for (int o2 = 32; o2 > 0; o2 >>= 1) f = max(f, (unsigned)__shfl_xor((int)f, o2, 64));
    if (lane == 0) syl[s] = (syl[s] & 0xffffu) | (min(f, 0xffffu) << 16);
  }
}

__global__ __launch_bounds__(256) void k_far_collect(const unsigned* __restrict__ E, const unsigned* __restrict__ rsl, size_t NS, unsigned rows_near,
                                                     unsigned* __restrict__ far_pos, unsigned* __restrict__ far_ent, unsigned long long* __restrict__ counter) {
  const int lane = threadIdx.x & 63;
  for (size_t s = (size_t)blockIdx.x * 4 + (threadIdx.x >> 6); s < NS; s += (size_t)gridDim.x * 4) {
    const unsigned ea = rsl[s], R = (rsl[s + 1] - ea) >> 6;
    for (unsigned r = 0; r < R; ++r) {
      const unsigned e = E[(size_t)ea + r * 64 + lane];
      const bool far = e != 0u && SL_X(e) != 0u && SL_YM(e) >= rows_near;
      const unsigned long long bal = __ballot(far);
      if (bal == 0ull) continue;
      unsigned long long base = 0ull;
      if (lane == 0) base = atomicAdd(counter, (unsigned long long)__popcll(bal));
      base = ((unsigned long long)(unsigned)__shfl((int)(unsigned)(base >> 32), 0, 64) << 32) | (unsigned)__shfl((int)(unsigned)base, 0, 64);
      if (far) {
        const unsigned long long at = base + (unsigned long long)__popcll(bal & ((1ull << lane) - 1ull));
        far_pos[at] = (unsigned)(s * 64 + (unsigned)lane);
        far_ent[at] = e;
      }
    }
  }
}

template <int K>
__global__ __launch_bounds__(1024) void k_far_hist(const unsigned* __restrict__ far_pos, const unsigned* __restrict__ far_ent,
                                                   const unsigned long long* __restrict__ fbase, const double* __restrict__ rho, double* Hg, double* par,
                                                   double* nu_acc, double* elbo_dev, int count, int commit_nu, int Gl, int LF, Geo g) {
  extern __shared__ double Hf[];
  const int Mp = g.Mp, tid = threadIdx.x, nthr = (int)blockDim.x;
  const int l = (int)blockIdx.x / Gl, gb = (int)blockIdx.x - l * Gl;
  const unsigned lfm = (unsigned)LF * (unsigned)Mp, hcm = (unsigned)g.hc * (unsigned)Mp;
  double* red = Hf + (size_t)K * lfm;
  for (unsigned q = tid; q < (unsigned)K * lfm; q += nthr) Hf[q] = 0.0;
  __syncthreads();
  const ParOff o = par_off(g.L, Mp, g.K);
  const size_t T = (size_t)g.N * g.N;
  double Gla[K];
#pragma unroll
  for (int k = 0; k < K; ++k) Gla[k] = par[o.G_la + l * K + k];
  const double gnu = par[o.sc + SC_G_NU];
  const double* gth = par + o.G_th + (size_t)l * Mp;
  const double* rl = rho + (size_t)l * T * K;
  double* Hl = Hg + ((size_t)l * NH + (gb % NH)) * g.Y * Mp * K;
  double share = 0.0;
  const unsigned long long i1 = fbase[l + 1];
  constexpr int FB = 4;
  for (unsigned long long i0 = fbase[l] + (unsigned long long)gb * nthr * FB + tid; i0 < i1; i0 += (unsigned long long)Gl * nthr * FB) {
    unsigned pos[FB], ent[FB];
    double r[FB][K];
#pragma unroll
    for (int u = 0; u < FB; ++u) {
      const unsigned long long i = i0 + (unsigned long long)u * nthr;
      const bool on = i < i1;
      pos[u] = on ? far_pos[i] : 0u;
      ent[u] = on ? far_ent[i] : 0u;
    }
#pragma unroll
    for (int u = 0; u < FB; ++u) {
#pragma unroll
      for (int k = 0; k < K; ++k) r[u][k] = count ? (k == 1 ? 1.0 : 0.0) : (ent[u] ? rl[(size_t)pos[u] * K + k] : 0.0);
    }
#pragma unroll
    for (int u = 0; u < FB; ++u) {
      if (ent[u] == 0u) continue;
      const unsigned ym = SL_YM(ent[u]), rel = ym - hcm;
      const double dx = (double)SL_X(ent[u]);
      double sm = 0.0;
#pragma unroll
      for (int k = 0; k < K; ++k) sm += r[u][k];
      double dfc = 1.0 - sm;
      if (fabs(dfc) <= 1e-14) dfc = 0.0;
      if (rel < lfm) {
#pragma unroll
        for (int k = 1; k < K; ++k) atomicAdd(&Hf[(unsigned)k * lfm + rel], dx * r[u][k]);
        if (dfc != 0.0) atomicAdd(&Hf[rel], dx * dfc);
      } else {
        double* d = Hl + (size_t)ym * K;
#pragma unroll
        for (int k = 1; k < K; ++k) atomicAdd(&d[k], dx * r[u][k]);
        if (dfc != 0.0) atomicAdd(&d[0], dx * dfc);
      }
      if (nu_acc) {
        const unsigned y = ym / (unsigned)Mp, m = ym - y * (unsigned)Mp;
        const double z2 = gnu * (double)y, gt = gth[m];
        const double d0 = gt * Gla[0] + z2, w0 = d0 == 0.0 ? 0.0 : z2 / d0;
        share -= w0 * dx * dfc;
#pragma unroll
        for (int k = 1; k < K; ++k) {
          const double dk = gt * Gla[k] + z2;
          share += ((dk == 0.0 ? 0.0 : z2 / dk) - w0) * dx * r[u][k];
        }
      }
    }
  }
  __syncthreads();
  for (unsigned q = tid; q < (unsigned)K * lfm; q += nthr) {
    const double v = Hf[q];
    if (v != 0.0) { const unsigned k = q / lfm, rel = q - k * lfm; atomicAdd(&Hl[(size_t)(hcm + rel) * K + k], v); }
  }
  if (!nu_acc) return;
  share = block_sum_n(share, red);
  __shared__ int last;
  if (tid == 0) {
    atomicAdd(&nu_acc[0], share);
    asm volatile("s_waitcnt vmcnt(0)" ::: "memory");
    const double t = atomicAdd(&nu_acc[1], 1.0);
    last = (t == (double)(gridDim.x - 1u));
    if (last) {
      __builtin_amdgcn_fence(__ATOMIC_ACQUIRE, "agent");
      asm volatile("s_waitcnt vmcnt(0)" ::: "memory");
      double tot = atomicAdd(&nu_acc[0], 0.0);
      for (int ll = 0; ll < g.L; ++ll) tot += nu_acc[2 + ll];
      nu_acc[0] = 0.0; nu_acc[1] = 0.0;
      elbo_dev[1] = tot;
      if (commit_nu) {
        double* sc = par + o.sc;
        sc[SC_G_NU_STALE] = sc[SC_G_NU];
        sc[SC_NU_SHP] = sc[SC_A_ETA] + tot;
        sc[SC_G_NU] = exp(digamma_pos(sc[SC_NU_SHP]) - log(sc[SC_NU_RTE]));
        sc[SC_E_NU] = sc[SC_NU_SHP] / sc[SC_NU_RTE];
      }
    }
  }
}
__global__ __launch_bounds__(256) void k_level0_spread(double* Hg, const double* __restrict__ Cg, double* h0s, Geo g) {
  __shared__ double Sk[KMAX];
  const int l = blockIdx.x, K = g.K, Mp = g.Mp;
  if ((int)threadIdx.x < K) {
    double s = 0.0;
    for (int sl = 0; sl < NSLOT; ++sl) { s += h0s[((size_t)l * NSLOT + sl) * K + threadIdx.x]; h0s[((size_t)l * NSLOT + sl) * K + threadIdx.x] = 0.0; }
    const double tot = h0s[(size_t)g.L * NSLOT * K + l];
    Sk[threadIdx.x] = tot > 0.0 ? s / tot : 0.0;
  }
  __syncthreads();
  double* H0 = Hg + (size_t)l * NH * g.Y * Mp * K;
  const double* C0 = Cg + (size_t)l * g.Y * Mp;
  for (int q = threadIdx.x; q < g.M * (K - 1); q += 256) {
    const int m = q / (K - 1), k = 1 + (q - m * (K - 1));
    const double c = C0[m];
    if (c != 0.0 && Sk[k] != 0.0) H0[(size_t)m * K + k] += c * Sk[k];
  }
}
__global__ __launch_bounds__(256) void k_level0_total(const double* __restrict__ Cg, double* h0s, Geo g) {
  __shared__ double red[16];
  const int l = blockIdx.x;
  double s = 0.0;
  for (int m = threadIdx.x; m < g.M; m += 256) s += Cg[(size_t)l * g.Y * g.Mp + m];
  s = block_sum_n(s, red);
  if (threadIdx.x == 0) h0s[(size_t)g.L * NSLOT * g.K + l] = s;
}

static int launch_far(vmr_ctx* h, int count, int nu) {
  const Geo& g = h->g;
  if (!g.farl || h->far_off.empty() || h->far_off.back() == 0ull) {
    if (nu >= 0 && g.farl) return fail(h, VMR_ESTATE, "far lists missing");
    return VMR_OK;
  }
  const size_t lb = (size_t)g.Mp * g.K * 8;
  const int LF = (int)std::max<size_t>(1, std::min<size_t>((size_t)(g.Y - g.hc), ((size_t)150 * 1024 - 256) / lb));
  const size_t sm = (size_t)LF * lb + 16 * 8;
  unsigned long long most = 0;
  for (int l = 0; l < g.L; ++l) most = std::max(most, h->far_off[l + 1] - h->far_off[l]);
  const int Gl = (int)std::max<unsigned long long>(1, std::min<unsigned long long>((most + 4095) / 4096, std::max(1, h->ncu / g.L)));
  double* nu_acc = (nu >= 0 && g.mut) ? h->nu_acc : nullptr;
  Prof p(h, VMR_KERNEL_GAMMA_COUNTS);
  DISPATCH_K(g.K, if (sm > 48 * 1024) HIPCHK(h, hipFuncSetAttribute(reinterpret_cast<const void*>(k_far_hist<KK>), hipFuncAttributeMaxDynamicSharedMemorySize, (int)sm));
             hipLaunchKernelGGL((k_far_hist<KK>), dim3(g.L * Gl), dim3(1024), sm, h->stream, h->far_pos, h->far_ent, h->far_base, h->rho, h->Hg, h->par,
                                nu_acc, h->elbo_dev, count, nu > 0 ? 1 : 0, Gl, LF, g));
  HIPCHK(h, hipGetLastError());
  return VMR_OK;
}

static int launch_fin_rho(vmr_ctx* h, int do_nu, int do_elbo, int skip_nu = 0) {
  const Geo& g = h->g;
  const int fold = (!skip_nu && h->h_valid && !h->h_reduced && !g.gen) ? 1 : 0;
  {
    Prof p(h, VMR_KERNEL_FINALIZE);
    hipLaunchKernelGGL(k_fin_rho, dim3(g.L * FR_G), dim3(TPB), 0, h->stream, h->par, h->Hg, h->Cg, h->slotR, h->elbo_dev,
                       h->elbo_dev + 4, do_nu, do_elbo, fold, skip_nu, g, g.det ? h->fr_slots : nullptr);
  }
  HIPCHK(h, hipGetLastError());
  if (fold) h->h_reduced = true;
  return VMR_OK;
}
static int ensure_h_folded(vmr_ctx* h) {
  if (h->h_reduced) return VMR_OK;
  const Geo& g = h->g;
  const size_t n = (size_t)g.L * g.Y * g.Mp * g.K;
  hipLaunchKernelGGL(k_h_reduce, dim3((unsigned)std::min<size_t>(1024, (n + TPB - 1) / TPB)), dim3(TPB), 0, h->stream, h->Hg, h->Cg, g);
  HIPCHK(h, hipGetLastError());
  h->h_reduced = true;
  return VMR_OK;
}

static int begin_sum_a(vmr_ctx* h, hipStream_t st) {
  const Geo& g = h->g;
  if (!h->a_zero) HIPCHK(h, hipMemsetAsync(h->slotA, 0, (size_t)g.L * NSLOT * g.W * 64 * g.K * 8, st));
  h->a_zero = false;
  return VMR_OK;
}
__global__ __launch_bounds__(256) void k_det_fold(unsigned long long* __restrict__ d, double* __restrict__ Hg, double* __restrict__ slotA,
                                                 double* __restrict__ slotF, double* __restrict__ slotR, Geo g) {
  const size_t nH = (size_t)g.Y * g.Mp * g.K, nA = (size_t)g.W * 64 * g.K, L = (size_t)g.L, K = (size_t)g.K;
  const size_t tot = L * nH + L * nA + L * K + 4;
  for (size_t q = (size_t)blockIdx.x * 256 + threadIdx.x; q < tot; q += (size_t)gridDim.x * 256) {
    const unsigned long long u = d[q];
    if (u == 0ull) continue;
    d[q] = 0ull;
    if (q < L * nH) { const size_t l = q / nH, i = q - l * nH; Hg[l * NH * nH + i] += det_back(u, g.det_sh); }
    else if (q < L * nH + L * nA) { const size_t r = q - L * nH, l = r / nA, i = r - l * nA; slotA[l * NSLOT * nA + i] += det_back(u, DET_SH_A); }
    else if (q < L * nH + L * nA + L * K) { const size_t r = q - L * nH - L * nA, l = r / K, k = r - l * K; slotF[l * NSLOT * K + k] += det_back(u, DET_SH_A); }
    else { const size_t r = q - L * nH - L * nA - L * K; slotR[r] += det_back(u, g.det_shr); }
  }
}
static int det_fold(vmr_ctx* h) {
  const Geo& g = h->g;
  if (!g.det) return VMR_OK;
  const size_t tot = (size_t)g.L * g.Y * g.Mp * g.K + (size_t)g.L * g.W * 64 * g.K + (size_t)g.L * g.K + 4;
  hipLaunchKernelGGL(k_det_fold, dim3((unsigned)std::min<size_t>(1024, (tot + 255) / 256)), dim3(256), 0, h->stream, h->det_buf, h->Hg, h->slotA, h->slotF,
                     h->slotR, g);
  HIPCHK(h, hipGetLastError());
  return VMR_OK;
}

static int ensure_rho(vmr_ctx* h) {
  if (!h->rho_stale) return VMR_OK;
  const SlShape shs = sl_shape(h, true, false, false);
  SlArgs as = sl_args(h, shs, 0, 0);
  as.slotF = nullptr; as.slotA = nullptr;
  as.nu_stale = h->g.mut ? 1 : 0;
  int rc = sl_launch(h, 0, shs, as);
  if (rc) return rc;
  HIPCHK(h, hipGetLastError());
  h->rho_stale = false;
  return VMR_OK;
}

int ensure_rho_ext(vmr_ctx* h) { return ensure_rho(h); }

static int launch_hist(vmr_ctx* h, int nu = -1) {
  const Geo& g = h->g;
  if (g.gen) return gen_hist(h);
  { int rce = ensure_rho(h); if (rce) return rce; }
  HIPCHK(h, hipMemsetAsync(h->Hg, 0, (size_t)g.L * NH * g.Y * g.Mp * g.K * 8, h->stream));
  if (h->sparse) {
    HIPCHK(h, hipMemsetAsync(h->slotF, 0, (size_t)g.L * NSLOT * g.K * 8, h->stream));
    h->f_valid = g.fuse_full != 0;
    if (g.ml) { int rc = begin_sum_a(h, h->stream); if (rc) return rc; h->a_valid = true; }
    Prof p(h, VMR_KERNEL_GAMMA_COUNTS);
    const SlShape shs = sl_shape(h, false, false, true);
    SlArgs as = sl_args(h, shs, 1, g.ml);
    if (nu >= 0 && g.mut) { as.nu_acc = h->nu_acc; as.elbo_dev = h->elbo_dev; as.commit_nu = nu; }
    as.det = g.det ? h->det_buf : nullptr;
    int rcs = sl_launch(h, 3, shs, as);
    if (rcs) return rcs;
    HIPCHK(h, hipGetLastError());
    if (g.farl && (rcs = launch_far(h, 0, (nu >= 0 && g.mut) ? nu : -1))) return rcs;
    if (as.h0s) {
      hipLaunchKernelGGL(k_level0_spread, dim3(g.L), dim3(256), 0, h->stream, h->Hg, h->Cg, h->h0s, g);
      HIPCHK(h, hipGetLastError());
    }
    if ((rcs = det_fold(h))) return rcs;
  } else {
    Prof p(h, VMR_KERNEL_GAMMA_COUNTS);
    HistArgs a{h->X, h->rho, h->Hg, 1};
    size_t sm = shmem_hist(g);
    int rc = VMR_OK;
    if (g.mut) {
      DISPATCH_KP(g.K, g.pf, if ((rc = grid_per_layer(h, k_hist<KK, true, PP>, sm, &a.Gl))) return rc;
                  hipLaunchKernelGGL((k_hist<KK, true, PP>), dim3(g.L * a.Gl), dim3(TPB), sm, h->stream, a, g));
    } else {
      DISPATCH_KP(g.K, g.pf, if ((rc = grid_per_layer(h, k_hist<KK, false, PP>, sm, &a.Gl))) return rc;
                  hipLaunchKernelGGL((k_hist<KK, false, PP>), dim3(g.L * a.Gl), dim3(TPB), sm, h->stream, a, g));
    }
  }
  HIPCHK(h, hipGetLastError());
  h->h_valid = true;
  h->h_zero = false;
  h->h_reduced = false;
  return VMR_OK;
}

static int launch_gamma(vmr_ctx* h, bool with_phi) {
  const Geo& g = h->g;
  if (g.gen) return gen_gamma(h, with_phi);
  if (h->sparse && !h->h_valid) {
    int rc = launch_hist(h);
    if (rc) return rc;
  }
  hipStream_t ms = h->h_valid ? h->stream : h->stream2;
  if (ms != h->stream) {
    HIPCHK(h, hipEventRecord(h->ev_fork, h->stream));
    HIPCHK(h, hipStreamWaitEvent(ms, h->ev_fork, 0));
  }
  const int skip_full = (g.fuse_full && h->f_valid) ? 1 : 0;
  if (skip_full && h->n_partial > 0 && h->rq && h->a_valid) {
  } else if (skip_full && h->n_partial > 0 && h->rq) {
    { int rc = begin_sum_a(h, ms); if (rc) return rc; }
    Prof p(h, VMR_KERNEL_GAMMA_MASK, ms);
    const size_t T_ = (size_t)g.N * g.N;
    int gl = (int)std::min<size_t>(std::max<size_t>(1, (size_t)h->ncu / g.L), (T_ + 4 * TPB - 1) / (4 * TPB));
    const size_t lsm = (size_t)g.Mp * g.K * 8;
    if (lsm > 48 * 1024 && !h->ml_attr) {
      DISPATCH_K(g.K, HIPCHK(h, hipFuncSetAttribute(reinterpret_cast<const void*>(k_mask_lists<KK>),
                                                    hipFuncAttributeMaxDynamicSharedMemorySize, (int)lsm)));
      h->ml_attr = true;
    }
    DISPATCH_K(g.K, hipLaunchKernelGGL((k_mask_lists<KK>), dim3(g.L * gl), dim3(TPB), lsm, ms, h->rq, h->Rm, h->rbase,
                                       h->rcls, h->rho, h->slotA, gl, h->perm, g));
  } else if (!skip_full || h->n_partial > 0) {
    Prof p(h, VMR_KERNEL_GAMMA_MASK, ms);
    dim3 grid(g.L * g.Gm), blk(TPB);
    switch (g.W >= 4 ? 4 : g.W) {
      case 1: DISPATCH_K(g.K, hipLaunchKernelGGL((k_gamma_mask<KK, 1>), grid, blk, 0, ms, h->Rb, h->rho, h->rcls, h->slotA, skip_full, h->perm, g)); break;
      case 2: DISPATCH_K(g.K, hipLaunchKernelGGL((k_gamma_mask<KK, 2>), grid, blk, 0, ms, h->Rb, h->rho, h->rcls, h->slotA, skip_full, h->perm, g)); break;
      case 3: DISPATCH_K(g.K, hipLaunchKernelGGL((k_gamma_mask<KK, 3>), grid, blk, 0, ms, h->Rb, h->rho, h->rcls, h->slotA, skip_full, h->perm, g)); break;
      default: DISPATCH_K(g.K, hipLaunchKernelGGL((k_gamma_mask<KK, 4>), grid, blk, 0, ms, h->Rb, h->rho, h->rcls, h->slotA, skip_full, h->perm, g)); break;
    }
  }
  if (ms != h->stream) {
    HIPCHK(h, hipEventRecord(h->ev_join, ms));
    int rc = launch_hist(h);
    if (rc) return rc;
    HIPCHK(h, hipStreamWaitEvent(h->stream, h->ev_join, 0));
  } else if (!h->h_valid) {
    int rc = launch_hist(h);
    if (rc) return rc;
  }
  {
    Prof p(h, VMR_KERNEL_FINALIZE);
    const int consume = (with_phi && !g.two_pass) ? 1 : 0;
    const int nh = h->h_reduced ? 1 : NH;
    const size_t fsm = (size_t)2 * ((g.M + FG_G - 1) / FG_G) * 8;
    hipLaunchKernelGGL(g.det ? k_fin_gamma_det : k_fin_gamma, dim3(g.L * FG_G), dim3(FIN_TPB), fsm, h->stream, h->par, h->Hg, h->sparse ? h->Cg : nullptr,
                       (h->sparse && skip_full && h->n_partial == 0) ? nullptr : h->slotA,
                       h->slotF, h->lutg, nullptr, h->fin_g, h->sparse ? h->nu_acc : nullptr, nh,
                       with_phi ? 1 : 0, consume, g);
    h->a_valid = false; h->a_zero = true;
    if (consume) { h->h_valid = false; h->f_valid = false; h->h_zero = true; }
  }
  HIPCHK(h, hipGetLastError());
  return VMR_OK;
}

static int launch_phi(vmr_ctx* h) {
  const Geo& g = h->g;
  if (g.gen) return gen_phi(h);
  if (!g.mut) return VMR_OK;
  if (!h->h_valid) { int rc = launch_hist(h); if (rc) return rc; }
  { int rc = ensure_h_folded(h); if (rc) return rc; }
  {
    Prof p(h, VMR_KERNEL_FINALIZE);
    hipLaunchKernelGGL(k_fin_phi, dim3(g.L), dim3(TPB), 0, h->stream, h->par, h->Hg, g);
  }
  HIPCHK(h, hipGetLastError());
  return VMR_OK;
}

static int launch_rho(vmr_ctx* h, int mode, bool commit_nu, bool raw_nu = false, bool store = true) {
  const Geo& g = h->g;
  if (g.gen) return gen_rho(h, mode, commit_nu, raw_nu, [](vmr_ctx* hh, int do_nu, int do_elbo, int skip_nu) { return launch_fin_rho(hh, do_nu, do_elbo, skip_nu); });
  if (h->sparse && g.farl && h->elbo_split && mode == 1) {
    int rc2 = launch_rho(h, 0, commit_nu, raw_nu, true);
    if (rc2) return rc2;
    const SlShape she = sl_shape(h, false, true, false);
    SlArgs ae = sl_args(h, she, 0, 0);
    ae.elbo_cur = commit_nu ? 0 : 1;
    {
      Prof p(h, VMR_KERNEL_ELBO);
      if ((rc2 = sl_launch(h, 2, she, ae))) return rc2;
    }
    HIPCHK(h, hipGetLastError());
    return launch_fin_rho(h, 0, 1, 1);
  }
  RhoArgs a{h->X, h->Rb, h->rho, h->logpr, h->par, h->slotR, h->lutg, h->Hg, h->slotF, 1};
  size_t sm = shmem_rho(g, mode != 2, mode != 0);
  dim3 blk(TPB);
  int rc = VMR_OK;
  if (mode != 2 && !h->h_zero) {
    if (g.fuse_full) HIPCHK(h, hipMemsetAsync(h->slotF, 0, (size_t)g.L * NSLOT * g.K * 8, h->stream));
    if (!g.two_pass) HIPCHK(h, hipMemsetAsync(h->Hg, 0, (size_t)g.L * NH * g.Y * g.Mp * g.K * 8, h->stream));
  }
  if (mode != 2) h->h_zero = false;
  const bool nu_in_pass = h->sparse && g.mut && mode != 2 && (commit_nu || raw_nu);
  if (mode == 2 && (rc = ensure_rho(h))) return rc;
  if (h->sparse) {
    const int do_hist = (mode != 2 && !g.two_pass) ? 1 : 0;
    const int sum_a = (g.ml && do_hist) ? 1 : 0;
    if (mode != 2) h->a_valid = false;
    if (sum_a) { if ((rc = begin_sum_a(h, h->stream))) return rc; h->a_valid = true; }
    const SlShape shs = sl_shape(h, mode != 2, mode != 0, do_hist != 0);
    SlArgs as = sl_args(h, shs, do_hist, sum_a);
    if (nu_in_pass && do_hist) { as.nu_acc = h->nu_acc; as.elbo_dev = h->elbo_dev; as.commit_nu = commit_nu ? 1 : 0; }
    as.det = g.det ? h->det_buf : nullptr;
    const bool lazy = !store && mode == 0 && do_hist && (nu_in_pass ? commit_nu : !g.mut) && g.fuse_full && (h->n_partial == 0 || g.ml) &&
                      !g.farl && !h->opt.always_store_rho;
    {
      Prof p(h, lazy ? VMR_KERNEL_RHO_NOSTORE : mode == 2 ? VMR_KERNEL_ELBO : mode == 1 ? VMR_KERNEL_RHO_ELBO : VMR_KERNEL_RHO);
      if ((rc = sl_launch(h, lazy ? 4 : mode, shs, as))) return rc;
    }
    if (mode != 2) h->rho_stale = lazy;
    if (g.farl && do_hist && (rc = launch_far(h, 0, nu_in_pass ? (commit_nu ? 1 : 0) : -1))) return rc;
    if ((rc = det_fold(h))) return rc;
  } else {
    Prof p(h, mode == 2 ? VMR_KERNEL_ELBO : mode == 1 ? VMR_KERNEL_RHO_ELBO : VMR_KERNEL_RHO);
#define LRHO(MUT_, UPD_, ELB_)                                                                  \
  DISPATCH_KP(g.K, g.pf, if ((rc = grid_per_layer(h, k_rho<KK, MUT_, UPD_, ELB_, PP>, sm, &a.Gl))) return rc; \
              hipLaunchKernelGGL((k_rho<KK, MUT_, UPD_, ELB_, PP>), dim3(g.L * a.Gl), blk, sm, h->stream, a, g))
    if (g.mut) {
      if (mode == 0) { LRHO(true, true, false); } else if (mode == 1) { LRHO(true, true, true); } else { LRHO(true, false, true); }
    } else {
      if (mode == 0) { LRHO(false, true, false); } else if (mode == 1) { LRHO(false, true, true); } else { LRHO(false, false, true); }
    }
#undef LRHO
  }
  if (mode != 2) {
    h->f_valid = g.fuse_full != 0;
    h->h_valid = !g.two_pass;
    if (!g.two_pass) h->h_reduced = false;
    if (g.two_pass && (rc = launch_hist(h, nu_in_pass ? (commit_nu ? 1 : 0) : -1))) return rc;
  }
  HIPCHK(h, hipGetLastError());
  if (nu_in_pass || (h->sparse && mode != 2 && !g.mut)) {
    if (mode != 0 && (rc = launch_fin_rho(h, 0, 1, 1))) return rc;
  } else if (mode != 0 || commit_nu) {
    if ((rc = launch_fin_rho(h, (mode != 2 && commit_nu) ? 1 : 0, mode != 0 ? 1 : 0))) return rc;
  }
  return VMR_OK;
}

static int choose_geo(Geo& g, int ncu, std::string& err, bool lists_only) {
  g.Mp = (g.M + 15) / 16 * 16;
  g.nchunk = g.Mp / 16;
  g.stride = (g.nchunk % 2 == 1) ? g.Mp : g.Mp + 16;
  g.W = (g.M + 63) / 64;
  const size_t budget = 48 * 1024;
  const size_t tables = (size_t)g.Mp * 8 * (2 + (g.mut ? g.K : 0)) + (size_t)g.W * 8 + shmem_q() + 256;
  auto lds = [&](int b_) { return (size_t)2 * b_ * b_ * (g.stride + (size_t)g.W * 8 + 2 * g.K * 8 + 4) + tables; };
  int b = 8;
  while (b > 1 && ((size_t)2 * b * b * g.stride > budget || lds(b) > 160 * 1024)) b >>= 1;
  if ((size_t)2 * b * b * g.stride > budget && !lists_only) { err = "M too large for the LDS tile (M <= ~24500 supported)"; return VMR_EINVAL; }
  g.b = b; g.lb = (b == 8) ? 3 : (b == 4) ? 2 : (b == 2) ? 1 : 0;
  g.nb = (g.N + b - 1) / b;
  g.nt = 2 * b * b;
  g.S = TPB / g.nt; if (g.S > 64) g.S = 64;
  g.lS = 0; while ((1 << g.lS) < g.S) ++g.lS;
  g.P = (long long)g.nb * (g.nb + 1) / 2;
  g.Gl = 0;
  g.Y = 1;
  g.hc = 0;
  g.two_pass = 0;
  g.farl = 0;
  g.fuse_full = 0;
  long long T = (long long)g.N * g.N;
  long long gm = (long long)ncu * 8 / g.L; if (gm < 1) gm = 1;
  long long maxgm = (T + 255) / 256; if (gm > maxgm) gm = maxgm; if (gm < 1) gm = 1;
  g.Gm = (int)gm;
  int need = (g.nt * g.nchunk + TPB - 1) / TPB;
  g.pf = need <= 4 ? 4 : need <= 8 ? 8 : 12;
  return VMR_OK;
}

extern "C" {

const char* vmr_version(void) { return VMR_VERSION; }

const char* vmr_last_error(vmr_handle h) { return h ? h->err.c_str() : g_create_err.c_str(); }

}


static void read_opts(VmrOpts& o) {
  memset(&o, 0, sizeof o);
  auto set = [](const char* n) { return getenv(n) != nullptr; };
  auto num = [](const char* n, int dflt) { const char* e = getenv(n); return e ? atoi(e) : dflt; };
  if (const char* f = getenv("VMR_FORMAT")) o.format = !strcmp(f, "dense") ? 1 : !strcmp(f, "sparse") ? 2 : 0;
  o.deterministic = num("VMR_DETERMINISTIC", 0) != 0;
  o.graph = num("VMR_GRAPH", 0) != 0;
  o.debug = num("VMR_DEBUG", 0);
  o.levels = num("VMR_LEVELS", 64);
  o.two_pass = num("VMR_TWO_PASS", 0);
  o.farl = num("VMR_FARL", 0);
  o.yt = set("VMR_YT") ? std::max(0, num("VMR_YT", 0)) : -1;
  o.hc = set("VMR_HC") ? std::max(0, num("VMR_HC", 0)) : -1;
  o.tpb = num("VMR_TPB", 0);
  o.st_tpb = num("VMR_ST_TPB", 0);
  o.no_level0 = set("VMR_NO_LEVEL0");
  o.no_x0 = set("VMR_NO_X0");
  o.no_lv0r = set("VMR_NO_LV0R");
  o.no_level_sort = set("VMR_NO_LEVEL_SORT");
  o.no_rlists = set("VMR_NO_RLISTS");
  o.no_rm2 = set("VMR_NO_RM2");
  o.no_lp0 = set("VMR_NO_LP0");
  o.no_lpd = set("VMR_NO_LPD");
  o.always_store_rho = set("VMR_ALWAYS_STORE_RHO");
  o.debug_lazy_rho = set("VMR_DEBUG_LAZY_RHO");
  o.gen_hsum = num("VMR_GEN_HSUM", 0);
  o.gen_no_lds_h = set("VMR_GEN_NO_LDS_H");
  o.gen_dbg = num("VMR_GEN_DBG", 0);
  o.netstats_chunk = std::max(0, num("VMR_NETSTATS_CHUNK", 0));
  o.batch_fg = set("VMR_BATCH_FG") ? std::max(1, std::min(FG_G, num("VMR_BATCH_FG", 0))) : 0;
  if (const char* t = getenv("VMR_DEBUG_TIMES")) snprintf(o.debug_times, sizeof o.debug_times, "%s", t);
}

static int create_ctx(vmr_ctx** out, hipDeviceProp_t* prop, int device, int L, int N, int M, int K, int mutuality, double eps, bool lists_only = false) {
  if (L < 1 || N < 1 || M < 1) return fail(nullptr, VMR_EINVAL, "L, N, M must be positive");
  if (K < 2 || K > KGEN_MAX) return fail(nullptr, VMR_EINVAL, "K must be in [2, 256]");
  int ndev = 0;
  CK(hipGetDeviceCount(&ndev));
  if (device < 0 || device >= ndev) return fail(nullptr, VMR_EINVAL, "no such HIP device");
  CK(hipSetDevice(device));
  CK(hipGetDeviceProperties(prop, device));
  vmr_ctx* h = new vmr_ctx();
  *out = h;
  h->device = device;
  Geo& g = h->g;
  g.L = L; g.N = N; g.M = M; g.K = K; g.mut = mutuality ? 1 : 0; g.eps = eps;
  g.gen = K > KMAX ? 1 : 0; g.wide = 0;
  read_opts(h->opt);
  g.dbg = h->opt.debug;
  g.det = h->opt.deterministic ? 1 : 0; g.det_sh = 0; g.det_shr = 0; g.det_sha = 0;
  std::string err;
  if (choose_geo(g, prop->multiProcessorCount, err, lists_only) != VMR_OK) return fail(nullptr, VMR_EINVAL, err.c_str());
  memset(h->prof_ms, 0, sizeof h->prof_ms); memset(h->prof_n, 0, sizeof h->prof_n);
  CK(hipStreamCreateWithFlags(&h->stream, hipStreamNonBlocking));
  CK(hipStreamCreateWithFlags(&h->stream2, hipStreamNonBlocking));
  CK(hipEventCreateWithFlags(&h->ev_fork, hipEventDisableTiming));
  CK(hipEventCreateWithFlags(&h->ev_join, hipEventDisableTiming));
  h->ncu = prop->multiProcessorCount;
  h->use_graphs = h->opt.graph;
  const size_t rows = (size_t)L * N * N;
  CK(hipMalloc(&h->cov, rows));
  CK(hipMalloc(&h->rcls, rows));
  CK(hipMalloc(&h->sumx, 8));
  CK(hipMemsetAsync(h->sumx, 0, 8, h->stream));
  CK(hipMalloc(&h->xmax, 4));
  CK(hipMemsetAsync(h->xmax, 0, 4, h->stream));
  CK(hipMalloc(&h->npartial, 16));
  CK(hipMemsetAsync(h->npartial, 0, 16, h->stream));
  return VMR_OK;
}

static int create_state(vmr_ctx* h, unsigned* xm_out) {
  Geo& g = h->g;
  const size_t rows = (size_t)g.L * g.N * g.N;
  CK(hipMalloc(&h->rho, (rows + 64) * g.K * 8));
  CK(hipMalloc(&h->logpr, (rows + 64) * g.K * 8));
  CK(hipMemsetAsync(h->rho + rows * g.K, 0, (size_t)64 * g.K * 8, h->stream));
  CK(hipMemsetAsync(h->logpr + rows * g.K, 0, (size_t)64 * g.K * 8, h->stream));
  ParOff o = par_off(g.L, g.Mp, g.K);
  h->par_doubles = o.total;
  CK(hipMalloc(&h->par, o.total * 8));
  CK(hipMemsetAsync(h->par, 0, o.total * 8, h->stream));
  const size_t nA = (size_t)g.L * NSLOT * g.W * 64 * g.K * 8;
  CK(hipMalloc(&h->slotA, nA)); CK(hipMemsetAsync(h->slotA, 0, nA, h->stream));
  CK(hipMalloc(&h->slotR, NSLOT * 4 * 8)); CK(hipMemsetAsync(h->slotR, 0, NSLOT * 4 * 8, h->stream));
  g.fuse_full = 1;
  CK(hipMalloc(&h->slotF, (size_t)g.L * NSLOT * g.K * 8));
  CK(hipMemsetAsync(h->slotF, 0, (size_t)g.L * NSLOT * g.K * 8, h->stream));
  CK(hipStreamSynchronize(h->stream));
  unsigned xm = 0;
  unsigned long long np2[2] = {0, 0};
  CK(hipMemcpy(&xm, h->xmax, 4, hipMemcpyDeviceToHost));
  CK(hipMemcpy(np2, h->npartial, 16, hipMemcpyDeviceToHost));
  h->n_partial = np2[0];
  h->all_full = (np2[0] == 0 && np2[1] == 0) ? 1 : 0;
  g.Y = g.mut ? (int)xm + 1 : 1;
  *xm_out = xm;
  return VMR_OK;
}

int scan_u32(vmr_ctx* h, unsigned* a, unsigned* bsum, size_t n) {
  const unsigned nb = (unsigned)((n + 2047) / 2048);
  hipLaunchKernelGGL(k_scan_local, dim3(nb), dim3(256), 0, h->stream, a, bsum, n);
  hipLaunchKernelGGL(k_scan_bsum, dim3(1), dim3(256), 0, h->stream, bsum, (int)nb);
  hipLaunchKernelGGL(k_scan_add, dim3(nb), dim3(256), 0, h->stream, a, bsum, n);
  CK(hipGetLastError());
  return VMR_OK;
}


static int mask_lists_from_words(vmr_ctx* h) {
  Geo& g = h->g;
  const int L = g.L, K = g.K;
  const size_t T = (size_t)g.N * g.N, n = T + 1, rows = (size_t)L * T;
  if (!(h->n_partial > 0) || h->opt.no_rlists) return VMR_OK;
  unsigned long long* tot_dev = nullptr;
  unsigned* max_dev = nullptr;
  unsigned* bsum = nullptr;
  CK(hipMalloc(&h->rq, (size_t)L * n * 4));
  CK(hipMalloc(&tot_dev, (size_t)L * 8));
  CK(hipMalloc(&max_dev, 4));
  CK(hipMalloc(&bsum, (n + 2047) / 2048 * 4));
  CK(hipMemsetAsync(tot_dev, 0, (size_t)L * 8, h->stream));
  CK(hipMemsetAsync(max_dev, 0, 4, h->stream));
  const unsigned rgrid = (unsigned)std::min<size_t>(4096, (T + 255) / 256);
  for (int l = 0; l < L; ++l)
    hipLaunchKernelGGL(k_rm_count, dim3(rgrid), dim3(256), 0, h->stream, h->Rb + (size_t)l * T * g.W,
                       h->rcls + (size_t)l * T, h->rq + (size_t)l * n, tot_dev + l, max_dev, T, g.W);
  CK(hipGetLastError());
  CK(hipStreamSynchronize(h->stream));
  std::vector<unsigned long long> rl_(L), rb_(L);
  unsigned maxrow = 0;
  CK(hipMemcpy(rl_.data(), tot_dev, (size_t)L * 8, hipMemcpyDeviceToHost));
  CK(hipMemcpy(&maxrow, max_dev, 4, hipMemcpyDeviceToHost));
  h->rm_maxrow = maxrow;
  CK(hipFree(tot_dev));
  CK(hipFree(max_dev));
  bool ok32 = true;
  h->n_rm = 0;
  for (int l = 0; l < L; ++l) { rb_[l] = h->n_rm; h->n_rm += rl_[l]; ok32 = ok32 && rl_[l] < 0xffffffffull; }
  const double list_bytes = 2.0 * (double)h->n_rm + 4.0 * (double)rows, word_bytes = (double)h->n_partial * g.W * 8.0;
  if (ok32 && maxrow <= 64 && (list_bytes * 4.0 <= word_bytes || g.N <= 1024) && (size_t)g.Mp * K * 8 <= 160 * 1024) {
    for (int l = 0; l < L; ++l) { int rc = scan_u32(h, h->rq + (size_t)l * n, bsum, n); if (rc) return rc; }
    CK(hipMalloc(&h->rbase, (size_t)L * 8));
    CK(hipMemcpyAsync(h->rbase, rb_.data(), (size_t)L * 8, hipMemcpyHostToDevice, h->stream));
    CK(hipMalloc(&h->Rm, ((size_t)h->n_rm + 64) * 2));
    for (int l = 0; l < L; ++l)
      hipLaunchKernelGGL(k_rm_fill, dim3(rgrid), dim3(256), 0, h->stream, h->Rb + (size_t)l * T * g.W,
                         h->rcls + (size_t)l * T, h->rq + (size_t)l * n, h->Rm + rb_[l], T, g.W);
    CK(hipGetLastError());
    CK(hipStreamSynchronize(h->stream));
  } else {
    CK(hipFree(h->rq));
    h->rq = nullptr;
    h->n_rm = 0;
  }
  CK(hipFree(bsum));
  return VMR_OK;
}

__global__ __launch_bounds__(256) void k_level_hist(const unsigned* __restrict__ E, unsigned long long n, int Mp, unsigned long long* __restrict__ hist) {
  __shared__ unsigned long long sh[65];
  for (int i = threadIdx.x; i < 65; i += 256) sh[i] = 0;
  __syncthreads();
  for (unsigned long long i = (unsigned long long)blockIdx.x * 256 + threadIdx.x; i < n; i += (unsigned long long)gridDim.x * 256) {
    const unsigned e = E[i];
    if (e == 0u) continue;
    const unsigned y = SL_YM(e) / (unsigned)Mp;
    atomicAdd(&sh[y < 64u ? y : 64u], 1ull);
  }
  __syncthreads();
  for (int i = threadIdx.x; i < 65; i += 256) if (sh[i]) atomicAdd(&hist[i], sh[i]);
}

static int build_far_lists(vmr_ctx* h) {
  const Geo& g = h->g;
  const size_t T = (size_t)g.N * g.N, NS = (T + 63) / 64;
  unsigned long long* cnt = nullptr;
  unsigned long long* hd = nullptr;
  struct Tmp { unsigned long long*& a; unsigned long long*& b; ~Tmp() { if (a) (void)hipFree(a); if (b) (void)hipFree(b); } } tmp_guard{cnt, hd};
  CK(hipMalloc(&cnt, 8));
  std::vector<unsigned long long> hist(65, 0);
  CK(hipMalloc(&hd, 65 * 8));
  CK(hipMemsetAsync(hd, 0, 65 * 8, h->stream));
  hipLaunchKernelGGL(k_level_hist, dim3(1024), dim3(256), 0, h->stream, h->E, h->n_slots, g.Mp, hd);
  CK(hipGetLastError());
  CK(hipMemcpyAsync(hist.data(), hd, 65 * 8, hipMemcpyDeviceToHost, h->stream));
  CK(hipStreamSynchronize(h->stream));
  unsigned long long far = 0;
  for (int y = std::min(g.hc, 64); y < 65; ++y) far += hist[y];
  CK(hipMalloc(&h->far_pos, (size_t)(far + 64) * 4));
  CK(hipMalloc(&h->far_ent, (size_t)(far + 64) * 4));
  h->far_off.assign(g.L + 1, 0ull);
  std::vector<unsigned long long> eb(g.L);
  CK(hipMemcpy(eb.data(), h->ebase, (size_t)g.L * 8, hipMemcpyDeviceToHost));
  for (int l = 0; l < g.L; ++l) {
    hipLaunchKernelGGL(k_far_first, dim3((unsigned)std::min<size_t>(8192, (NS + 3) / 4)), dim3(256), 0, h->stream, h->E + eb[l], h->rs + (size_t)l * (NS + 1),
                       h->sy + (size_t)l * NS, NS, (unsigned)g.hc * (unsigned)g.Mp, (unsigned*)nullptr);
    CK(hipGetLastError());
    CK(hipMemsetAsync(cnt, 0, 8, h->stream));
    hipLaunchKernelGGL(k_far_collect, dim3((unsigned)std::min<size_t>(8192, (NS + 3) / 4)), dim3(256), 0, h->stream, h->E + eb[l], h->rs + (size_t)l * (NS + 1), NS,
                       (unsigned)g.hc * (unsigned)g.Mp, h->far_pos + h->far_off[l], h->far_ent + h->far_off[l], cnt);
    CK(hipGetLastError());
    unsigned long long n = 0;
    CK(hipMemcpyAsync(&n, cnt, 8, hipMemcpyDeviceToHost, h->stream));
    CK(hipStreamSynchronize(h->stream));
    h->far_off[l + 1] = h->far_off[l] + n;
    if (h->far_off[l + 1] > far) return fail(nullptr, VMR_EHIP, "far lists: more reports than counted");
  }
  CK(hipMalloc(&h->far_base, (size_t)(g.L + 1) * 8));
  CK(hipMemcpy(h->far_base, h->far_off.data(), (size_t)(g.L + 1) * 8, hipMemcpyHostToDevice));
  return VMR_OK;
}

__global__ __launch_bounds__(256) void k_rm2(const unsigned* __restrict__ perm, const unsigned* __restrict__ rq, const unsigned short* __restrict__ Rm,
                                             const unsigned long long* __restrict__ rbase, unsigned* __restrict__ out, size_t T, size_t NS, int L) {
  const size_t n = (size_t)L * NS * 64;
  for (size_t q = (size_t)blockIdx.x * 256 + threadIdx.x; q < n; q += (size_t)gridDim.x * 256) {
    const size_t l = q / (NS * 64);
    const unsigned tie = perm[q];
    unsigned w = 0xffffffffu;
    if (tie != 0xffffffffu) {
      const unsigned q0 = rq[l * (T + 1) + tie], q1 = rq[l * (T + 1) + tie + 1];
      const unsigned short* r = Rm + rbase[l];
      const unsigned m0 = q1 > q0 ? r[q0] : 0xffffu, m1 = q1 > q0 + 1 ? r[q0 + 1] : 0xffffu;
      w = m0 | (m1 << 16);
    }
    out[q] = w;
  }
}

static int sl_finish(vmr_ctx* h) {
  const Geo& g = h->g;
  const size_t rows = (size_t)g.L * g.N * g.N;
  int rc = VMR_OK;
  if (!h->all_full) {
    CK(hipMalloc(&h->cls_p, rows + 64));
    CK(hipMemsetAsync(h->cls_p + rows, 0, 64, h->stream));
    if ((rc = sl_permute_u8(h, h->rcls, h->cls_p))) return rc;
  }
  if (g.mut && h->Qt) {
    CK(hipMalloc(&h->Qt_p, (rows + 64) * 4));
    CK(hipMemsetAsync(h->Qt_p + rows, 0, 64 * 4, h->stream));
    if ((rc = sl_permute_u32(h, h->Qt, h->Qt_p))) return rc;
    CK(hipStreamSynchronize(h->stream));
    CK(hipFree(h->Qt)); h->Qt = nullptr;
  }
  return VMR_OK;
}

static int det_scales(vmr_ctx* h, int xbits) {
  Geo& g = h->g;
  unsigned long long sx = 0;
  CK(hipMemcpyAsync(&sx, h->sumx, 8, hipMemcpyDeviceToHost, h->stream));
  CK(hipStreamSynchronize(h->stream));
  int bits = 1;
  while (bits < 62 && (sx >> bits) != 0ull) ++bits;
  g.det_sh = std::max(0, std::min(51 - xbits, 61 - bits));
  const unsigned long long eb = 64ull * (sx + (unsigned long long)g.L * g.N * g.N * g.K);
  int rbits = 1;
  while (rbits < 62 && (eb >> rbits) != 0ull) ++rbits;
  g.det_shr = std::min(34, std::max(0, 61 - rbits));
  return VMR_OK;
}

static int create_tail(vmr_ctx* h, const hipDeviceProp_t& prop) {
  Geo& g = h->g;
  const int L = g.L, K = g.K;
  g.ml = (h->sparse && h->rq) ? 1 : 0;
  if (g.ml && (!g.gen || g.Mp > 8192) && h->rm_maxrow <= 2 && !h->opt.no_rm2) {
    const size_t T_ = (size_t)g.N * g.N, NS_ = (T_ + 63) / 64, n_ = (size_t)L * NS_ * 64;
    CK(hipMalloc(&h->rm2, n_ * 4));
    hipLaunchKernelGGL(k_rm2, dim3((unsigned)std::min<size_t>(4096, (n_ + 255) / 256)), dim3(256), 0, h->stream, h->perm, h->rq, h->Rm, h->rbase, h->rm2, T_, NS_, L);
    CK(hipGetLastError());
  }
  if (g.gen) {
    g.ml = 0; g.hc = 0; g.yt = 0; g.two_pass = 0;
    const double hb = (double)L * g.Y * g.Mp * K * 8.0;
    size_t fr = 0, tot = 0;
    CK(hipMemGetInfo(&fr, &tot));
    if (hb > 0.5 * (double)fr) {
      char msg[256];
      snprintf(msg, sizeof msg, "the statistics table H[L][max count + 1][M][K] would take %.1f GB (largest count %d, M = %d, K = %d): more than half "
               "of the device memory left", hb / 1e9, g.Y - 1, g.M, K);
      return fail(nullptr, VMR_EINVAL, msg);
    }
    CK(hipMalloc(&h->Hg, (size_t)hb));
    CK(hipMemsetAsync(h->Hg, 0, (size_t)hb, h->stream));
    CK(hipMalloc(&h->gen_s1, (size_t)L * (g.Mp + K + 1) * 8));
    CK(hipMemsetAsync(h->gen_s1, 0, (size_t)L * (g.Mp + K + 1) * 8, h->stream));
    CK(hipMalloc(&h->elbo_dev, 8 * 8));
    CK(hipMemsetAsync(h->elbo_dev, 0, 8 * 8, h->stream));
    CK(hipMalloc(&h->nu_acc, (size_t)(3 + L) * 8));
    CK(hipMemsetAsync(h->nu_acc, 0, (size_t)(3 + L) * 8, h->stream));
    CK(hipMalloc(&h->lutg, (size_t)L * g.W * 256 * 8));
    CK(hipMemsetAsync(h->lutg, 0, (size_t)L * g.W * 256 * 8, h->stream));
    if (g.det) {
      if (!h->sparse) return fail(nullptr, VMR_EINVAL, "VMR_DETERMINISTIC=1 needs the report lists (a sparse tensor)");
      unsigned xm = 0;
      CK(hipMemcpyAsync(&xm, h->xmax, 4, hipMemcpyDeviceToHost, h->stream));
      CK(hipStreamSynchronize(h->stream));
      int xbits = 1;
      while (xbits < 32 && (xm >> xbits) != 0u) ++xbits;
      int rc = det_scales(h, xbits);
      if (rc) return rc;
      const unsigned long long T_ = (unsigned long long)g.N * g.N;
      int tbits = 1;
      while (tbits < 62 && (T_ >> tbits) != 0ull) ++tbits;
      g.det_sha = std::min(50, 62 - tbits);
      CK(hipMalloc(&h->fr_slots, (size_t)L * FR_G * 2 * 8));
      CK(hipMemsetAsync(h->fr_slots, 0, (size_t)L * FR_G * 2 * 8, h->stream));
    }
    CK(hipStreamSynchronize(h->stream));
    return VMR_OK;
  }
  g.hc = g.Y < HC_MAX ? g.Y : HC_MAX;
  g.yt = 0;
  g.two_pass = 0;
  size_t need = 0;
  if (h->sparse) {
    const VmrOpts& o = h->opt;
    const int want = std::max(1, std::min(g.Y, o.levels));
    auto cap_of = [&](bool upd) { return sl_tpb_max(K, false, h->all_full != 0, upd); };
    auto wcu_of = [&](bool upd) { return 4 * sl_wpe(K, false, h->all_full != 0, upd); };
    auto waves = [&](int tpb, int yt, int hc, bool upd, bool hist) {
      const size_t b = sl_smem(g, yt, hc, upd, false, hist);
      if (b > SP_LDS_MAX || tpb > cap_of(upd)) return 0;
      const int nw = tpb / 64, wgs = std::min((int)(SP_LDS_MAX / b), wcu_of(upd) / nw);
      return wgs * nw;
    };
    auto best = [&](bool upd, bool hist, int min_waves, int& lv_out, int& tpb_out) {
      min_waves = std::min(min_waves, wcu_of(upd));
      for (int lv = want; lv >= 1; --lv) {
        int bw = 0, bt = 256;
        for (int tpb : {1024, 768, 512, 256}) { const int w = waves(tpb, upd ? lv : 0, hist ? lv : 0, upd, hist); if (w > bw) { bw = w; bt = tpb; } }
        if (bw >= min_waves) { lv_out = lv; tpb_out = bt; return true; }
      }
      return false;
    };
    int lv1 = 0, t1 = 256, lvr = 0, tr = 256, lvh = 0, th = 256;
    bool want_farl = false;
    bool one = best(true, true, 16, lv1, t1);
    if (one && lv1 < want && g.N > 1024) {
      std::vector<unsigned long long> hist(65, 0);
      unsigned long long* hd = nullptr;
      CK(hipMalloc(&hd, 65 * 8));
      CK(hipMemsetAsync(hd, 0, 65 * 8, h->stream));
      hipLaunchKernelGGL(k_level_hist, dim3(1024), dim3(256), 0, h->stream, h->E, h->n_slots, g.Mp, hd);
      CK(hipGetLastError());
      CK(hipMemcpyAsync(hist.data(), hd, 65 * 8, hipMemcpyDeviceToHost, h->stream));
      CK(hipStreamSynchronize(h->stream));
      CK(hipFree(hd));
      unsigned long long tot = 0, far = 0;
      for (int y = 0; y < 65; ++y) { tot += hist[y]; if (y >= lv1) far += hist[y]; }
      if ((double)far > (double)tot / 1024.0) {
        if (g.mut && !g.det && o.farl && (double)far <= 0.125 * (double)tot) want_farl = true;
        else one = false;
      }
    }
    one = one && !o.two_pass;
    if (one) { g.yt = g.hc = lv1; h->sp_tpb = h->st_tpb = t1; g.farl = want_farl ? 1 : 0; }
    else {
      g.two_pass = 1;
      if (!best(true, false, 16, lvr, tr) && !best(true, false, 4, lvr, tr)) { lvr = 0; tr = 256; }
      if (!best(false, true, 16, lvh, th) && !best(false, true, 4, lvh, th)) { lvh = 0; th = 256; }
      g.yt = lvr; g.hc = lvh; h->sp_tpb = tr; h->st_tpb = th;
    }
    {
      const long long NS = ((long long)g.N * g.N + 63) / 64;
      for (int* t : {&h->sp_tpb, &h->st_tpb})
        while (*t > 64 && NS * L < (long long)h->ncu * (*t / 64)) *t = std::max(64, (*t / 2) & ~63);
    }
    g.yt = std::max(0, std::min(g.Y, o.yt >= 0 ? o.yt : g.yt));
    g.hc = std::max(0, std::min(g.Y, o.hc >= 0 ? o.hc : g.hc));
    if (o.tpb >= 64 && o.tpb <= 1024 && o.tpb % 64 == 0) h->sp_tpb = o.tpb;
    if (o.st_tpb >= 64 && o.st_tpb <= 1024 && o.st_tpb % 64 == 0) h->st_tpb = o.st_tpb;
    for (int v = 0; v < 4; ++v) need = std::max(need, sl_shape(h, v != 3, v == 1 || v == 2, v == 0 || v == 1 || v == 3).smem);
    if (g.two_pass && g.mut && !g.det && g.Y > 1 && !o.no_level0) {
      const size_t T_ = (size_t)g.N * g.N, NS_ = (T_ + 63) / 64;
      std::vector<unsigned long long> eb(L);
      CK(hipMemcpy(eb.data(), h->ebase, (size_t)L * 8, hipMemcpyDeviceToHost));
      if (!o.no_x0) CK(hipMalloc(&h->x0p, (size_t)L * NS_ * 64 * 4));
      for (int l = 0; l < L; ++l)
        hipLaunchKernelGGL(k_far_first, dim3((unsigned)std::min<size_t>(8192, (NS_ + 3) / 4)), dim3(256), 0, h->stream, h->E + eb[l], h->rs + (size_t)l * (NS_ + 1),
                           h->sy + (size_t)l * NS_, NS_, (unsigned)g.Mp, h->x0p ? h->x0p + (size_t)l * NS_ * 64 : nullptr);
      CK(hipGetLastError());
      if (h->x0p) {
        unsigned long long* ss = nullptr;
        CK(hipMalloc(&ss, 8));
        CK(hipMemsetAsync(ss, 0, 8, h->stream));
        for (int l = 0; l < L; ++l)
          hipLaunchKernelGGL(k_stat_slots, dim3(256), dim3(256), 0, h->stream, h->rs + (size_t)l * (NS_ + 1), h->sy + (size_t)l * NS_, NS_, ss);
        hipError_t es = hipMemcpyAsync(&h->stat_slots, ss, 8, hipMemcpyDeviceToHost, h->stream);
        if (es == hipSuccess) es = hipStreamSynchronize(h->stream);
        (void)hipFree(ss);
        CK(es);
      }
      const size_t n0 = (size_t)L * NSLOT * K + L;
      CK(hipMalloc(&h->h0s, n0 * 8));
      CK(hipMemsetAsync(h->h0s, 0, n0 * 8, h->stream));
    }
    if (g.farl) {
      bool same = g.hc >= 1 && g.hc < g.Y;
      for (int v : {0, 3}) same = same && sl_shape(h, v != 3, false, true).hc == g.hc;
      h->elbo_split = sl_shape(h, true, true, true).hc != g.hc || sl_shape(h, true, true, true).yt != g.yt;
      if (!same) g.farl = 0;
      else { int rcf = build_far_lists(h); if (rcf) return rcf; }
    }
  } else {
    if (shmem_rho(g, true, false) > 80000) {
      g.two_pass = 1;
      while (g.hc > 0 && shmem_hist(g) > 160000) --g.hc;
    }
    need = std::max(shmem_rho(g, true, true), shmem_hist(g));
  }
  if (need > (size_t)prop.sharedMemPerBlock && need > 160 * 1024) {
    char msg[256];
    snprintf(msg, sizeof msg, "M = %d reporters with K = %d%s needs %zu bytes of LDS per workgroup (limit %d): "
             "reduce M or K", g.M, K, g.mut ? " and mutuality" : "", need, 160 * 1024);
    return fail(nullptr, VMR_EINVAL, msg);
  }
  CK(hipMalloc(&h->Hg, (size_t)L * NH * g.Y * g.Mp * K * 8));
  CK(hipMemsetAsync(h->Hg, 0, (size_t)L * NH * g.Y * g.Mp * K * 8, h->stream));
  CK(hipMalloc(&h->elbo_dev, 8 * 8));
  CK(hipMemsetAsync(h->elbo_dev, 0, 8 * 8, h->stream));
  CK(hipMalloc(&h->nu_acc, (size_t)(3 + L) * 8));
  CK(hipMemsetAsync(h->nu_acc, 0, (size_t)(3 + L) * 8, h->stream));
  CK(hipMalloc(&h->fin_g, ((size_t)L * (2 * KMAX + 2) + (size_t)L * FG_G * 2 * KMAX) * 8));
  CK(hipMemsetAsync(h->fin_g, 0, ((size_t)L * (2 * KMAX + 2) + (size_t)L * FG_G * 2 * KMAX) * 8, h->stream));
  if (g.det) {
    if (!h->sparse) return fail(nullptr, VMR_EINVAL, "VMR_DETERMINISTIC=1 needs the report lists (a sparse tensor with M <= 8192, counts <= 2047)");
    int rc = det_scales(h, 11);
    if (rc) return rc;
    const size_t nd = (size_t)L * g.Y * g.Mp * K + (size_t)L * g.W * 64 * K + (size_t)L * K + 5;
    CK(hipMalloc(&h->det_buf, nd * 8));
    CK(hipMemsetAsync(h->det_buf, 0, nd * 8, h->stream));
    CK(hipMalloc(&h->fr_slots, (size_t)L * FR_G * 2 * 8));
    CK(hipMemsetAsync(h->fr_slots, 0, (size_t)L * FR_G * 2 * 8, h->stream));
  }
  CK(hipMalloc(&h->lutg, (size_t)L * g.W * 256 * 8));
  CK(hipMemsetAsync(h->lutg, 0, (size_t)L * g.W * 256 * 8, h->stream));
  if (h->sparse) {
    CK(hipMalloc(&h->Cg, (size_t)L * g.Y * g.Mp * 8));
    int rc = VMR_OK;
    {
      const SlShape sh = sl_shape(h, false, false, true);
      SlArgs a = sl_args(h, sh, 2);
      rc = sl_launch(h, 3, sh, a);
      if (rc == VMR_OK && g.farl) rc = launch_far(h, 1, -1);
    }
    if (rc != VMR_OK) { g_create_err = h->err; return rc; }
    CK(hipGetLastError());
    const size_t nit = (size_t)L * g.Y * g.Mp;
    hipLaunchKernelGGL(k_take_counts, dim3((unsigned)std::min<size_t>(1024, (nit + TPB - 1) / TPB)), dim3(TPB), 0, h->stream, h->Hg, h->Cg, g);
    CK(hipGetLastError());
    if (h->h0s) {
      hipLaunchKernelGGL(k_level0_total, dim3(L), dim3(256), 0, h->stream, h->Cg, h->h0s, g);
      CK(hipGetLastError());
    }

  }
  CK(hipStreamSynchronize(h->stream));
  return VMR_OK;
}

static int create_dense(vmr_ctx* h, const hipDeviceProp_t& prop, const uint8_t* X, const uint8_t* R, int data_on_device) {
  Geo& g = h->g;
  const int L = g.L, N = g.N, M = g.M;
  const size_t T = (size_t)N * N, rows = (size_t)L * T, raw = rows * M;
  const size_t slack = (size_t)g.b * N + g.b;
  CK(hipMalloc(&h->X, (rows + slack) * g.Mp));
  CK(hipMemsetAsync(h->X + rows * g.Mp, 0, slack * g.Mp, h->stream));
  CK(hipMalloc(&h->Rb, (rows + slack) * g.W * 8));
  CK(hipMemsetAsync(h->Rb + rows * g.W, 0, slack * g.W * 8, h->stream));
  {
    uint8_t* tmp = nullptr;
    const uint8_t* src = X;
    if (!data_on_device) { CK(hipMalloc(&tmp, raw)); CK(hipMemcpyAsync(tmp, X, raw, hipMemcpyHostToDevice, h->stream)); src = tmp; }
    hipLaunchKernelGGL(k_pack_x, dim3(4096), dim3(256), 0, h->stream, src, h->X, rows, M, g.Mp);
    CK(hipGetLastError());
    CK(hipStreamSynchronize(h->stream));
    if (tmp) CK(hipFree(tmp));
    tmp = nullptr; src = R;
    if (R && !data_on_device) { CK(hipMalloc(&tmp, raw)); CK(hipMemcpyAsync(tmp, R, raw, hipMemcpyHostToDevice, h->stream)); src = tmp; }
    hipLaunchKernelGGL(k_pack_r, dim3(4096), dim3(256), 0, h->stream, src, h->Rb, rows, M, g.W);
    CK(hipGetLastError());
    hipLaunchKernelGGL(k_stats, dim3(2048), dim3(256), 0, h->stream, h->X, h->Rb, h->cov, h->rcls, h->sumx, h->xmax, h->npartial, rows, g.Mp, g.W, M);
    CK(hipGetLastError());
    CK(hipStreamSynchronize(h->stream));
    if (tmp) CK(hipFree(tmp));
  }
  unsigned xm = 0;
  int rc = create_state(h, &xm);
  if (rc) return rc;
  const bool force_dense = h->opt.format == 1, force_sparse = h->opt.format == 2;
  const bool packed_ok = g.Mp <= 8192 && xm <= SL_XMAX && (size_t)(xm + 1) * g.Mp <= SL_YM_ROWS;
  const bool need_lists = g.K > KMAX;
  if (need_lists && force_dense) return fail(nullptr, VMR_EINVAL, "VMR_FORMAT=dense: the dense tile kernels hold at most 8 categories");
  bool dense_fits = true;
  {
    Geo t = g;
    t.Y = g.Y; t.hc = t.Y < HC_MAX ? t.Y : HC_MAX;
    if (shmem_rho(t, true, false) > 80000) { t.two_pass = 1; while (t.hc > 0 && shmem_hist(t) > 160000) --t.hc; }
    dense_fits = std::max(shmem_rho(t, true, true), shmem_hist(t)) <= (size_t)160 * 1024;
  }
  const bool can_list = packed_ok || need_lists || force_sparse || !dense_fits;
  if (!force_dense && can_list) {
    g.wide = packed_ok ? 0 : 1;
    unsigned* rp = nullptr;
    CK(hipMalloc(&rp, (size_t)L * (T + 1) * 4));
    unsigned long long* nnz_dev = nullptr;
    CK(hipMalloc(&nnz_dev, (size_t)L * 8));
    CK(hipMemsetAsync(nnz_dev, 0, (size_t)L * 8, h->stream));
    const unsigned cgrid = (unsigned)std::min<size_t>(8192, (T + 15) / 16);
    for (int l = 0; l < L; ++l)
      hipLaunchKernelGGL(k_sp_count, dim3(cgrid), dim3(256), 0, h->stream, h->X + (size_t)l * T * g.Mp,
                         rp + (size_t)l * (T + 1), nnz_dev + l, g);
    CK(hipGetLastError());
    CK(hipStreamSynchronize(h->stream));
    std::vector<unsigned long long> nl(L);
    CK(hipMemcpy(nl.data(), nnz_dev, (size_t)L * 8, hipMemcpyDeviceToHost));
    CK(hipFree(nnz_dev));
    bool fits = true;
    h->nnz = 0;
    for (int l = 0; l < L; ++l) { h->nnz += nl[l]; fits = fits && nl[l] < 0xffffffffull; }
    const double sparse_bytes = 4.0 * (double)h->nnz + 4.0 * (double)rows, dense_bytes = (double)rows * g.Mp;
    if (need_lists && !fits) { (void)hipFree(rp); return fail(nullptr, VMR_EINVAL, "more than 2^32 reports in one layer"); }
    h->sparse = fits && (force_sparse || need_lists || !dense_fits || sparse_bytes <= 0.5 * dense_bytes);
    if (!h->sparse) g.wide = 0;
    g.gen = (h->sparse && (need_lists || g.wide)) ? 1 : 0;
    if (h->sparse) {
      CK(hipMalloc(&h->Qt, rows * 4));
      CK(hipMemsetAsync(h->Qt, 0, rows * 4, h->stream));
      auto fill_layer = [&](int l, const unsigned* rpl, unsigned* etmp, unsigned* etmp2) {
        if (g.mut)
          hipLaunchKernelGGL(k_sp_fill<true>, dim3(cgrid), dim3(256), 0, h->stream, h->X + (size_t)l * T * g.Mp,
                             h->Rb + (size_t)l * T * g.W, rpl, etmp, etmp2, h->Qt + (size_t)l * T, g);
        else
// ... 1017 lines not shown
  }
  HIPCHK(h, hipStreamSynchronize(h->stream));
  return VMR_OK;
}

int vmr_get_geometric(vmr_handle h, double* g_theta, double* g_lambda, double* g_nu, double* g_nu_cache) {
  if (!h) return VMR_EINVAL;
  HIPCHK(h, hipSetDevice(h->device));
  const Geo& g = h->g;
  ParOff o = par_off(g.L, g.Mp, g.K);
  int rc;
  std::vector<double> buf;
  if ((rc = fetch_par(h, buf))) return rc;
  if (g_theta) rows_lm(g, buf, o.G_th, g_theta);
  if (g_lambda) memcpy(g_lambda, &buf[o.G_la], (size_t)g.L * g.K * 8);
  if (g_nu) *g_nu = buf[o.sc + SC_G_NU];
  if (g_nu_cache) *g_nu_cache = buf[o.sc + SC_G_NU_STALE];
  return VMR_OK;
}

int vmr_snapshot(vmr_handle h) {
  if (!h) return VMR_EINVAL;
  if (!h->have_state) return fail(h, VMR_ESTATE, "vmr_set_state must be called before vmr_snapshot");
  HIPCHK(h, hipSetDevice(h->device));
  { const int rce = ensure_rho(h); if (rce) return rce; }
  const Geo& g = h->g;
  const size_t nr = (size_t)g.L * g.N * g.N * g.K * 8, np_ = h->par_doubles * 8;
  if (!h->rho_snap) { HIPCHK(h, hipMalloc(&h->rho_snap, nr)); HIPCHK(h, hipMalloc(&h->par_snap, np_)); }
  HIPCHK(h, hipMemcpyAsync(h->rho_snap, h->rho, nr, hipMemcpyDeviceToDevice, h->stream));
  HIPCHK(h, hipMemcpyAsync(h->par_snap, h->par, np_, hipMemcpyDeviceToDevice, h->stream));
  h->have_snap = true;
  return VMR_OK;
}

int vmr_restore(vmr_handle h) {
  if (!h) return VMR_EINVAL;
  if (!h->have_snap) return fail(h, VMR_ESTATE, "vmr_snapshot must be called before vmr_restore");
  HIPCHK(h, hipSetDevice(h->device));
  const Geo& g = h->g;
  HIPCHK(h, hipMemcpyAsync(h->rho, h->rho_snap, (size_t)g.L * g.N * g.N * g.K * 8, hipMemcpyDeviceToDevice, h->stream));
  HIPCHK(h, hipMemcpyAsync(h->par, h->par_snap, h->par_doubles * 8, hipMemcpyDeviceToDevice, h->stream));
  h->h_valid = false; h->f_valid = false; h->a_valid = false; h->h_zero = false;
  h->restored = true;
  h->rho_stale = false;
  HIPCHK(h, hipMemsetAsync(h->slotF, 0, (size_t)g.L * NSLOT * g.K * 8, h->stream));
  hipLaunchKernelGGL(k_build_lut, dim3(g.L), dim3(256), 0, h->stream, h->par, h->lutg, g);
  HIPCHK(h, hipGetLastError());
  return VMR_OK;
}

int vmr_readout(vmr_handle h, int method, double threshold, void* out, int out_on_device) {
  if (!h || !out) return VMR_EINVAL;
  if (!h->have_state) return fail(h, VMR_ESTATE, "vmr_set_state must be called before vmr_readout");
  if (method < VMR_READ_RHO_MAX || method > VMR_READ_THRESHOLD) return fail(h, VMR_EINVAL, "unknown read-out method");
  HIPCHK(h, hipSetDevice(h->device));
  { const int rce = ensure_rho(h); if (rce) return rce; }
  const Geo& g = h->g;
  const size_t ties = (size_t)g.L * g.N * g.N, bytes = ties * (method == VMR_READ_RHO_MEAN ? 8 : 1);
  void* dst = out;
  if (!out_on_device) HIPCHK(h, hipMalloc(&dst, bytes));
  const size_t T_ = (size_t)g.N * g.N;
  hipLaunchKernelGGL(k_readout, dim3((unsigned)std::min<size_t>(4096, (ties + 255) / 256)), dim3(256), 0, h->stream, h->rho, dst, ties,
                     g.K, method, threshold, h->perm, T_, (T_ + 63) / 64);
  hipError_t e = hipGetLastError();
  if (e == hipSuccess && !out_on_device) e = hipMemcpyAsync(out, dst, bytes, hipMemcpyDeviceToHost, h->stream);
  if (e == hipSuccess) e = hipStreamSynchronize(h->stream);
  if (!out_on_device) (void)hipFree(dst);
  if (e != hipSuccess) { h->err = std::string("vmr_readout: ") + hipGetErrorString(e); (void)hipGetLastError(); return VMR_EHIP; }
  return VMR_OK;
}

int vmr_sample(vmr_handle h, uint64_t seed, int n_trials, uint8_t* out, int out_on_device) {
  if (!h || !out) return VMR_EINVAL;
  if (!h->have_state) return fail(h, VMR_ESTATE, "vmr_set_state must be called before vmr_sample");
  if (n_trials < 1) return fail(h, VMR_EINVAL, "n_trials must be positive");
  HIPCHK(h, hipSetDevice(h->device));
  { const int rce = ensure_rho(h); if (rce) return rce; }
  const Geo& g = h->g;
  const size_t T_ = (size_t)g.N * g.N, ties = (size_t)g.L * T_;
  uint8_t* dst = out;
  if (!out_on_device) HIPCHK(h, hipMalloc(&dst, ties));
  if (g.K > KMAX) { const int rcg = gen_sample(h, (unsigned long long)seed, n_trials, dst); if (rcg) { if (!out_on_device) (void)hipFree(dst); return rcg; } }
  else hipLaunchKernelGGL(k_sample, dim3((unsigned)std::min<size_t>(4096, (ties + 255) / 256)), dim3(256), 0, h->stream, h->rho, dst, ties, g.K,
                          n_trials, (unsigned long long)seed, h->perm, T_, (T_ + 63) / 64);
  hipError_t e = hipGetLastError();
  if (e == hipSuccess && !out_on_device) e = hipMemcpyAsync(out, dst, ties, hipMemcpyDeviceToHost, h->stream);
  if (e == hipSuccess) e = hipStreamSynchronize(h->stream);
  if (!out_on_device) (void)hipFree(dst);
  if (e != hipSuccess) { h->err = std::string("vmr_sample: ") + hipGetErrorString(e); (void)hipGetLastError(); return VMR_EHIP; }
  return VMR_OK;
}

int vmr_sync(vmr_handle h) {
  if (!h) return VMR_EINVAL;
  HIPCHK(h, hipSetDevice(h->device));
  HIPCHK(h, hipStreamSynchronize(h->stream));
  return VMR_OK;
}

static int prof_collect(vmr_ctx* h) {
  HIPCHK(h, hipStreamSynchronize(h->stream));
  for (auto& e : h->evs) {
    float ms = 0.f;
    if (hipEventElapsedTime(&ms, e.a, e.b) == hipSuccess) { h->prof_ms[e.cls] += ms; h->prof_n[e.cls] += 1; }
    (void)hipEventDestroy(e.a); (void)hipEventDestroy(e.b);
  }
  h->evs.clear();
  return VMR_OK;
}

int vmr_profile(vmr_handle h, int enable) {
  if (!h) return VMR_EINVAL;
  HIPCHK(h, hipSetDevice(h->device));
  int rc = prof_collect(h);
  if (rc) return rc;
  h->prof = enable != 0;
  h->prof_mask = enable == 2 ? ((1u << VMR_KERNEL_GAMMA_COUNTS) | (1u << VMR_KERNEL_RHO) | (1u << VMR_KERNEL_ELBO) | (1u << VMR_KERNEL_RHO_ELBO) | (1u << VMR_KERNEL_RHO_NOSTORE)) : ~0u;
  if (enable) { memset(h->prof_ms, 0, sizeof h->prof_ms); memset(h->prof_n, 0, sizeof h->prof_n); }
  return VMR_OK;
}

int vmr_profile_read(vmr_handle h, int kernel_class, double* total_ms, int64_t* launches) {
  if (!h || kernel_class < 0 || kernel_class >= VMR_KERNEL_COUNT) return VMR_EINVAL;
  HIPCHK(h, hipSetDevice(h->device));
  int rc = prof_collect(h);
  if (rc) return rc;
  if (total_ms) *total_ms = h->prof_ms[kernel_class];
  if (launches) *launches = h->prof_n[kernel_class];
  return VMR_OK;
}

int vmr_data_format(vmr_handle h, int* sparse, uint64_t* nnz) {
  if (!h) return VMR_EINVAL;
  if (sparse) *sparse = h->sparse;
  if (nnz) *nnz = h->nnz;
  return VMR_OK;
}

int vmr_mask_format(vmr_handle h, int* lists, uint64_t* listed) {
  if (!h) return VMR_EINVAL;
  if (lists) *lists = h->rq ? 1 : 0;
  if (listed) *listed = h->n_rm;
  return VMR_OK;
}

int vmr_sweep_shape(vmr_handle h, int* passes, int* lds_levels, uint64_t* far_reports) {
  if (!h) return VMR_EINVAL;
  if (passes) *passes = h->g.two_pass ? 2 : 1;
  if (lds_levels) *lds_levels = h->g.gen ? 0 : h->g.hc;
  if (far_reports) *far_reports = (h->g.farl && !h->far_off.empty()) ? h->far_off.back() : 0ull;
  return VMR_OK;
}

int vmr_kernel_bytes(vmr_handle h, int kernel_class, double* bytes) {
  if (!h || !bytes) return VMR_EINVAL;
  const Geo& g = h->g;
  const double V = (double)g.L * g.N * g.N * g.M;
  const double SX = V, SR = V / 8.0, Srho = 8.0 * g.L * (double)g.N * g.N * g.K;
  if (h->sparse) {
    const double ties = (double)g.L * g.N * g.N;
    const double E = (g.wide ? 8.0 : 4.0) * (double)h->nnz, RP = 4.0 * (ties / 64.0 + g.L);
    const double mask = h->all_full ? 0.0 : ties + (h->rq ? 4.0 * ties + 2.0 * (double)h->n_rm : (double)h->n_partial * g.W * 8.0);
    const double Q = g.mut ? 4.0 * ties : 0.0;
    const double Slp = h->lpd ? 8.0 * ties : Srho;
    switch (kernel_class) {
      case VMR_KERNEL_GAMMA_MASK: *bytes = ties + (h->rq ? 4.0 * ties + 2.0 * (double)h->n_rm : (double)h->n_partial * g.W * 8.0) + Srho; break;
      case VMR_KERNEL_GAMMA_COUNTS:
        *bytes = ((h->x0p && g.two_pass) ? 4.0 * (double)h->stat_slots + 4.0 * ties : E) + RP + Srho;
        break;
      case VMR_KERNEL_RHO: *bytes = E + RP + mask + Slp + Srho; break;
      case VMR_KERNEL_RHO_NOSTORE: *bytes = E + RP + mask + Slp; break;
      case VMR_KERNEL_ELBO: *bytes = E + RP + mask + Q + 2.0 * Srho; break;
      case VMR_KERNEL_RHO_ELBO: *bytes = E + RP + mask + Q + 2.0 * Srho; break;
      default: *bytes = 0.0; break;
    }
    return VMR_OK;
  }
  switch (kernel_class) {
    case VMR_KERNEL_GAMMA_MASK: *bytes = SR + Srho; break;
    case VMR_KERNEL_GAMMA_COUNTS: *bytes = SX + Srho; break;
    case VMR_KERNEL_PHI: *bytes = 0.0; break;
    case VMR_KERNEL_RHO: *bytes = SX + SR + 2.0 * Srho; break;
    case VMR_KERNEL_ELBO: *bytes = SX + SR + 2.0 * Srho; break;
    case VMR_KERNEL_RHO_ELBO: *bytes = SX + SR + 2.0 * Srho; break;
    default: *bytes = 0.0; break;
  }
  return VMR_OK;
}

}
```

vimure_amd/csrc/vmr_internal.h:

```cpp
#ifndef VMR_INTERNAL_H
#define VMR_INTERNAL_H
#include <hip/hip_runtime.h>
#include <hipcub/hipcub.hpp>
#include <stdint.h>
#include <stdio.h>
#include <string.h>
#include <math.h>
#include <stdlib.h>
#include <string>
#include <vector>
#include <utility>
#include <algorithm>
#include <chrono>
#include <type_traits>

#include "vimure_hip.h"

#define VMR_VERSION "vimure_hip 0.1 (gfx950)"
#define TPB 256
#ifndef VMR_LB_COUNTS
#define VMR_LB_COUNTS 4
#endif
#ifndef VMR_LB_RHO
#define VMR_LB_RHO 3
#endif
#ifndef VMR_NR_STEPS
#define VMR_NR_STEPS 1
#endif
#define KMAX 8
#define KGEN_MAX 256

struct Geo {
  int L, N, M, K, mut;
  int Mp;
  int nchunk;
  int stride;
  int W;
  int b, lb;
  int nb;
  int nt;
  int S, lS;
  long long P;
  int Gl;
  int Gm;
  int Y;
  int hc;
  int yt;
  int fuse_full;
  int ml;
  int two_pass;
  int pf;
  int dbg;
  double eps;
  int det;
  int det_sh;
  int det_shr;
  int gen;
  int farl;
  int wide;
  int det_sha;
};
#define DET_SH_A 30
#define DET_SH2 30
__device__ __forceinline__ unsigned long long det_fx(double v, int sh) { return (unsigned long long)__double2ll_rn(ldexp(v, sh)); }
__device__ __forceinline__ double det_back(unsigned long long u, int sh) { return ldexp((double)(long long)u, -sh); }

#define NSLOT 8

struct VmrOpts {
  int format;
  bool deterministic, graph;
  int debug, levels;
  int two_pass, farl;
  int yt, hc;
  int tpb, st_tpb;
  bool no_level0, no_x0, no_lv0r, no_level_sort, no_rlists, no_rm2, no_lp0, no_lpd;
  bool always_store_rho, debug_lazy_rho;
  int gen_hsum;
  bool gen_no_lds_h;
  int gen_dbg;
  int batch_fg;
  int netstats_chunk;
  char debug_times[256];
};

struct vmr_ctx {
  Geo g;
  VmrOpts opt;
  int device;
  hipStream_t stream;
  hipStream_t stream2 = nullptr;
  hipEvent_t ev_fork = nullptr, ev_join = nullptr;
  std::string err;
  uint8_t* X = nullptr;
  uint64_t* Rb = nullptr;
  uint8_t* cov = nullptr;
  void* drw = nullptr;
  size_t drw_cap = 0;
  uint8_t* rcls = nullptr;
  int sparse = 0;
  unsigned* E = nullptr;
  unsigned* EX = nullptr;
  double* gen_s1 = nullptr;
  unsigned* rs = nullptr;
  double* Cg = nullptr;
  int sp_tpb = 256;
  int st_tpb = 256;
  unsigned* Qt = nullptr;
  unsigned long long* ebase = nullptr;
  unsigned long long nnz = 0;
  unsigned long long n_slots = 0;
  int all_full = 0;
  unsigned* perm = nullptr;
  unsigned* sy = nullptr;
  unsigned* far_pos = nullptr;
  unsigned* far_ent = nullptr;
  unsigned long long* far_base = nullptr;
  std::vector<unsigned long long> far_off;
  double* h0s = nullptr;
  unsigned long long stat_slots = 0;
  unsigned* x0p = nullptr;
  bool elbo_split = false;
  uint8_t* cls_p = nullptr;
  unsigned* Qt_p = nullptr;
  double* nat = nullptr;
  unsigned* rq = nullptr;
  unsigned short* Rm = nullptr;
  unsigned long long* rbase = nullptr;
  unsigned long long n_rm = 0;
  unsigned rm_maxrow = 0;
  unsigned* rm2 = nullptr;
  int coo_mb = 13;
  unsigned long long* sumx = nullptr;
  double *rho = nullptr, *logpr = nullptr;
  double *lpd = nullptr, *lpb = nullptr;
  double* par = nullptr;
  struct GraphEntry { int n; bool lazy_last; unsigned sig0, sig1; hipGraphExec_t ex; };
  std::vector<GraphEntry> graphs;
  bool use_graphs = false;
  unsigned long long* det_buf = nullptr;
  double* fr_slots = nullptr;
  double *rho_snap = nullptr, *par_snap = nullptr;
  bool have_snap = false;
  bool lp0 = false;
  bool rho_stale = false;
  bool restored = false;
  size_t par_doubles = 0;
  double *slotA = nullptr, *slotR = nullptr;
  double* Hg = nullptr;
  bool h_valid = false;
  double* slotF = nullptr;
  bool f_valid = false;
  bool a_valid = false;
  bool a_zero = true;
  bool h_reduced = false;
  bool h_zero = false;
  bool fin_attr = false, ml_attr = false;
  unsigned long long* npartial = nullptr;
  unsigned long long n_partial = 0;
  unsigned* xmax = nullptr;
  double* elbo_dev = nullptr;
  double* fin_g = nullptr;
  double* nu_acc = nullptr;
  double* lutg = nullptr;
  bool have_priors = false, have_state = false;
  int ncu = 256;
  std::vector<std::pair<const void*, int>> occ;
  bool prof = false;
  unsigned prof_mask = ~0u;
  struct Ev { int cls; hipEvent_t a, b; };
  std::vector<Ev> evs;
  double prof_ms[VMR_KERNEL_COUNT];
  int64_t prof_n[VMR_KERNEL_COUNT];
};

extern thread_local std::string g_create_err;

struct ParOff {
  size_t a_th, b_th, g_shp, g_rte, E_th, G_th, l_th;
  size_t a_la, b_la, p_shp, p_rte, p_rte_pend, E_la, G_la, l_la;
  size_t sc;
  size_t total;
};
enum { SC_A_ETA = 0, SC_B_ETA, SC_NU_SHP, SC_NU_RTE, SC_G_NU, SC_G_NU_STALE, SC_E_NU, SC_COUNT = 8 };

__host__ __device__ static inline ParOff par_off(int L, int Mp, int K) {
  ParOff o;
  size_t LM = (size_t)L * Mp, LK = (size_t)L * K, p = 0;
  o.a_th = p; p += LM; o.b_th = p; p += LM; o.g_shp = p; p += LM; o.g_rte = p; p += LM;
  o.E_th = p; p += LM; o.G_th = p; p += LM; o.l_th = p; p += LM;
  o.a_la = p; p += LK; o.b_la = p; p += LK; o.p_shp = p; p += LK; o.p_rte = p; p += LK;
  o.p_rte_pend = p; p += LK; o.E_la = p; p += LK; o.G_la = p; p += LK; o.l_la = p; p += LK;
  o.sc = p; p += SC_COUNT;
  o.total = p;
  return o;
}

#define HIPCHK(h, call)                                                              \
  do {                                                                               \
    hipError_t e_ = (call);                                                          \
    if (e_ != hipSuccess) {                                                          \
      char buf_[512];                                                                \
      snprintf(buf_, sizeof buf_, "%s failed: %s (%s:%d)", #call, hipGetErrorString(e_), __FILE__, __LINE__); \
      if (h) (h)->err = buf_; else g_create_err = buf_;                              \
      (void)hipGetLastError();  \
      return VMR_EHIP;                                                               \
    }                                                                                \
  } while (0)

__device__ __forceinline__ double digamma_pos(double x) {
  double r = 0.0;
  while (x < 10.0) { r -= 1.0 / x; x += 1.0; }
  double f = 1.0 / (x * x);
  double t = f * (-1.0 / 12.0 + f * (1.0 / 120.0 + f * (-1.0 / 252.0 + f * (1.0 / 240.0 +
             f * (-1.0 / 132.0 + f * (691.0 / 32760.0 + f * (-1.0 / 12.0)))))));
  return r + log(x) - 0.5 / x + t;
}

__device__ __forceinline__ double wave_sum(double v) {
#pragma unroll
  for (int o = 32; o > 0; o >>= 1) v += __shfl_xor(v, o, 64);
  return v;
}

__device__ __forceinline__ double group_sum(double v, int S) {
  for (int o = S >> 1; o > 0; o >>= 1) v += __shfl_xor(v, o, 64);
  return v;
}
__device__ __forceinline__ unsigned group_sum_u(unsigned v, int S) {
  for (int o = S >> 1; o > 0; o >>= 1) v += __shfl_xor(v, o, 64);
  return v;
}

__device__ __forceinline__ double block_sum(double v, double* red) {
  v = wave_sum(v);
  __syncthreads();
  if ((threadIdx.x & 63) == 0) red[threadIdx.x >> 6] = v;
  __syncthreads();
  double r = 0.0;
  if (threadIdx.x == 0) {
    for (int w = 0; w < TPB / 64; ++w) r += red[w];
  }
  return r;
}


__device__ __forceinline__ double w1_of(double z1, double z2) {
  double den = z1 + z2;
  den = (den == 0.0) ? 1.0 : den;
  return z1 / den;
}


__device__ __forceinline__ double fast_rcp(double d) {
  double r = __builtin_amdgcn_rcp(d);
#pragma unroll
  for (int i = 0; i < VMR_NR_STEPS; ++i) r = fma(fma(-d, r, 1.0), r, r);
  return r;
}

__device__ __forceinline__ uint64_t readlane64(uint64_t v, int lane) {
  unsigned lo = __builtin_amdgcn_readlane((int)(unsigned)v, lane);
  unsigned hi = __builtin_amdgcn_readlane((int)(unsigned)(v >> 32), lane);
  return ((uint64_t)hi << 32) | lo;
}
__device__ __forceinline__ double readlane_f64(double v, int lane) {
  return __longlong_as_double((long long)readlane64((uint64_t)__double_as_longlong(v), lane));
}


#ifndef NH
#define NH 8
#endif
#ifndef HC_MAX
// ... 157 lines not shown
```

vimure_amd/engine.py:

```python
import ctypes as C

import numpy as np

from . import _lib


class EngineError(RuntimeError):
    pass


class EdgeTableArgumentError(EngineError, ValueError):
    """An argument `edge_table` / `edge_table_size` refuse (VMR_EINVAL): a method that gives no categories, an empty or
    unknown selection, outputs shorter than the table."""


EDGE_COLUMNS = (("l", np.int32), ("i", np.int32), ("j", np.int32), ("y", np.uint8), ("prob", np.float64), ("mean", np.float64),
                ("n_rep", np.uint32), ("total", np.uint64), ("n_mask", np.uint32), ("ego", np.uint32), ("alter", np.uint32),
                ("y_T", np.uint8), ("n_rep_T", np.uint32), ("total_T", np.uint64))
_TORCH_NAME = {"uint32": "int32", "uint64": "int64"}


def _f64(a):
    return np.ascontiguousarray(a, dtype=np.float64)

# ... 351 lines not shown
        la = self._layer_arg(layer)
        n = self.mean_poisson_size(layer)
        if device:
            import torch
            dev = torch.device("cuda", self.device)
            subs = [torch.empty(n, dtype=torch.int32, device=dev) for _ in range(4)]
            vals = torch.empty(n, dtype=torch.float64, device=dev)
            torch.cuda.synchronize(dev)
            ptrs, vp = [t.data_ptr() for t in subs], vals.data_ptr()
        else:
            subs = [np.empty(n, np.int32) for _ in range(4)]
            vals = np.empty(n, np.float64)
            ptrs, vp = [a.ctypes.data for a in subs], vals.ctypes.data
        if n:
            self._check(self.lib.vmr_mean_poisson(self._h, la, n, *ptrs, vp, int(bool(device))))
        return tuple(subs), vals

    def report_auc(self, layer=None):
        a, p, q = C.c_double(), C.c_uint64(), C.c_uint64()
        self._check(self.lib.vmr_report_auc(self._h, self._layer_arg(layer), C.byref(a), C.byref(p), C.byref(q)))
        return a.value, int(p.value), int(q.value)

    def ppc_replicates(self, theta, lam, eta, seed_y, seed_x, n_trials=1, by_reporter=False):
        theta, lam = _f64(theta), _f64(lam)
        eta = _f64(np.atleast_1d(eta))
        n_rep = int(eta.shape[0])
        if theta.shape != (n_rep, self.L, self.M) or lam.shape != (n_rep, self.L, self.K) or eta.ndim != 1:
            raise ValueError(f"theta {theta.shape}, lam {lam.shape}, eta {eta.shape}: expected (n_rep, {self.L}, {self.M}), "
                             f"(n_rep, {self.L}, {self.K}), (n_rep,)")
        counts = np.zeros((n_rep, self.L, _lib.PPC_NSTAT), np.uint64)
        rep = np.zeros((n_rep, self.L, self.M, 2), np.uint64) if by_reporter else None
        self._check(self.lib.vmr_ppc_replicates(self._h, n_rep, int(seed_y) & (2 ** 64 - 1), int(seed_x) & (2 ** 64 - 1), int(n_trials),
                                                theta.ctypes.data, lam.ctypes.data, eta.ctypes.data, counts.ctypes.data,
                                                rep.ctypes.data if by_reporter else None))
        counts = counts.astype(np.int64)
        return (counts, rep.astype(np.int64)) if by_reporter else counts

    def ppc_observed(self, by_reporter=False):
        counts = np.zeros((self.L, _lib.PPC_NSTAT), np.uint64)
        rep = np.zeros((self.L, self.M, 2), np.uint64) if by_reporter else None
        self._check(self.lib.vmr_ppc_observed(self._h, counts.ctypes.data, rep.ctypes.data if by_reporter else None))
        counts = counts.astype(np.int64)
        return (counts, rep.astype(np.int64)) if by_reporter else counts

    def _edge_args(self, method, threshold, select, layer):
        codes = {"rho_max": _lib.READ_RHO_MAX, "rho_mean": _lib.READ_RHO_MEAN, "threshold": _lib.READ_THRESHOLD}
        if method not in codes:
            raise ValueError("'method' should be one of \"rho_max\", \"threshold\".")
        if isinstance(select, str):
            select = (select,)
        if isinstance(select, (int, np.integer)):
            sel = int(select)
        else:
            bits = {"reported": _lib.EDGE_REPORTED, "inferred": _lib.EDGE_INFERRED}
            sel = 0
            for s in select:
                if s not in bits:
                    raise ValueError("'select' holds \"reported\", \"inferred\" or both.")
                sel |= bits[s]
        return codes[method], float(threshold), sel, self._layer_arg(layer)

    def _check_edge(self, rc):
        if rc == _lib.VMR_EINVAL:
            raise EdgeTableArgumentError(self.lib.vmr_last_error(self._h).decode())
        self._check(rc)

    def edge_table_size(self, method="rho_max", threshold=0.0, select=("reported", "inferred"), layer=None):
        code, thr, sel, la = self._edge_args(method, threshold, select, layer)
        n = C.c_uint64()
        self._check_edge(self.lib.vmr_edge_table_size(self._h, code, thr, sel, la, C.byref(n)))
        return int(n.value)

    def edge_table(self, method="rho_max", threshold=0.0, select=("reported", "inferred"), layer=None, device=False, out=None):
        code, thr, sel, la = self._edge_args(method, threshold, select, layer)
        if out is not None:
            cap = {int(a.shape[0]) for a in out.values()}
            if len(cap) != 1:
                raise ValueError("out: arrays of one length expected")
            n, cols = cap.pop(), out
        else:
            n = self.edge_table_size(method, threshold, sel, layer)
            if device:
                import torch
                dev = torch.device("cuda", self.device)
                cols = {c: torch.empty(n, dtype=getattr(torch, _TORCH_NAME.get(np.dtype(t).name, np.dtype(t).name)), device=dev)
                        for c, t in EDGE_COLUMNS}
            else:
                cols = {c: np.empty(n, t) for c, t in EDGE_COLUMNS}
        ptrs = []
        for c, t in EDGE_COLUMNS:
            a = cols.get(c)
            if a is None:
                ptrs.append(None)
            elif _is_torch(a):
                assert a.is_cuda and a.is_contiguous() and a.element_size() == np.dtype(t).itemsize
                ptrs.append(a.data_ptr())
            else:
                assert a.dtype == np.dtype(t) and a.flags.c_contiguous
                ptrs.append(a.ctypes.data)
        on_dev = any(_is_torch(a) for a in cols.values())
        if on_dev:
            import torch
            torch.cuda.synchronize(torch.device("cuda", self.device))
        if n or out is not None:
            self._check_edge(self.lib.vmr_edge_table(self._h, code, thr, sel, la, n, *ptrs, int(on_dev)))
        return cols

    def snapshot(self):
        self._check(self.lib.vmr_snapshot(self._h))

    def restore(self):
        self._check(self.lib.vmr_restore(self._h))

    def get_state(self, rho=True, rho_out=None):
        out = {
            "gamma_shp": np.empty((self.L, self.M)), "gamma_rte": np.empty((self.L, self.M)),
            "phi_shp": np.empty((self.L, self.K)), "phi_rte": np.empty((self.L, self.K)),
        }
        ns, nr = C.c_double(), C.c_double()
        r = None
        if rho:
            r = rho_out if rho_out is not None else np.empty((self.L, self.N, self.N, self.K))
            assert r.dtype == np.float64 and r.flags.c_contiguous and r.size == self.L * self.N * self.N * self.K
            r = r.reshape(self.L, self.N, self.N, self.K)
        self._check(self.lib.vmr_get_state(
            self._h, out["gamma_shp"].ctypes.data, out["gamma_rte"].ctypes.data, out["phi_shp"].ctypes.data,
            out["phi_rte"].ctypes.data, C.addressof(ns), C.addressof(nr), r.ctypes.data if rho else None))
        out["nu_shp"], out["nu_rte"] = ns.value, nr.value
        if rho:
            out["rho"] = r
        return out

    def get_geometric(self):
        gt, gl, gn, gc = np.empty((self.L, self.M)), np.empty((self.L, self.K)), C.c_double(), C.c_double()
        self._check(self.lib.vmr_get_geometric(self._h, gt.ctypes.data, gl.ctypes.data, C.addressof(gn),
                                               C.addressof(gc)))
        return gt, gl, gn.value, gc.value

    def data_format(self):
        sp, nnz = C.c_int(), C.c_uint64()
        self._check(self.lib.vmr_data_format(self._h, C.byref(sp), C.byref(nnz)))
        return ("sparse" if sp.value else "dense"), int(nnz.value)

    def mask_format(self):
        li, n = C.c_int(), C.c_uint64()
        self._check(self.lib.vmr_mask_format(self._h, C.byref(li), C.byref(n)))
        return ("lists" if li.value else "words"), int(n.value)

    def sweep_shape(self):
        p, lv, n = C.c_int(), C.c_int(), C.c_uint64()
        self._check(self.lib.vmr_sweep_shape(self._h, C.byref(p), C.byref(lv), C.byref(n)))
        return int(p.value), int(lv.value), int(n.value)

    def profile(self, enable=True):
        self._check(self.lib.vmr_profile(self._h, int(enable)))

    def profile_read(self):
        out = {}
        for i, name in enumerate(_lib.KERNEL_NAMES):
            ms, n, b = C.c_double(), C.c_int64(), C.c_double()
            self._check(self.lib.vmr_profile_read(self._h, i, C.byref(ms), C.byref(n)))
            self._check(self.lib.vmr_kernel_bytes(self._h, i, C.byref(b)))
            out[name] = {"ms": ms.value, "launches": n.value, "bytes_per_launch": b.value}
        return out
```

Baseline: 6109.

## Skip level-0 entry rounds in K=2 rho sweep using precomputed x0 sums

For K=2 single-pass mutuality fits, entries are sorted by level. The rho sweep now reads only the rounds that hold non-level-0 reports and folds the level-0 contribution in as a precomputed per-tie x0 sum times the level-0 factor. A bound on the level-0 log-theta term lets it check overflow safety; when that check fails it walks the skipped rounds on a slow path, and a level-0 spread kernel rebuilds the histogram afterwards. This cuts per-iteration entry loads in the rho kernel, at the cost of extra setup passes, an added kernel launch, and more branchy code.

Result: slower. 5192 (-15.0%).

```diff
diff --git a/include/vimure_hip.h b/include/vimure_hip.h
--- a/include/vimure_hip.h
+++ b/include/vimure_hip.h
@@ -126,6 +126,8 @@
 
 int vmr_sweep_shape(vmr_handle h, int* passes, int* lds_levels, uint64_t* far_reports);
 
+int vmr_level0_shape(vmr_handle h, int* plain_sweeps_skip, uint64_t* rounds, uint64_t* rounds_skipped);
+
 int vmr_generate_y(int device, int L, int N, int K, int C, const double* w, const int32_t* grp, uint64_t seed, uint8_t* Y_dev);
 int vmr_generate_x(int device, int L, int N, int M, const uint8_t* Y_dev, const double* lam_dev, const double* theta, double eta,
                    double lambda_diff, uint64_t seed, int self_reporter, uint8_t* X_dev);
diff --git a/vimure_amd/_lib.py b/vimure_amd/_lib.py
--- a/vimure_amd/_lib.py
+++ b/vimure_amd/_lib.py
@@ -65,6 +65,7 @@
     "vmr_data_format": (C.c_int, [C.c_void_p, C.POINTER(C.c_int), C.POINTER(C.c_uint64)]),
     "vmr_mask_format": (C.c_int, [C.c_void_p, C.POINTER(C.c_int), C.POINTER(C.c_uint64)]),
     "vmr_sweep_shape": (C.c_int, [C.c_void_p, C.POINTER(C.c_int), C.POINTER(C.c_int), C.POINTER(C.c_uint64)]),
+    "vmr_level0_shape": (C.c_int, [C.c_void_p, C.POINTER(C.c_int), C.POINTER(C.c_uint64), C.POINTER(C.c_uint64)]),
     "vmr_generate_y": (C.c_int, [C.c_int, C.c_int, C.c_int, C.c_int, C.c_int, C.c_void_p, C.c_void_p, C.c_uint64, C.c_void_p]),
     "vmr_generate_x": (C.c_int, [C.c_int, C.c_int, C.c_int, C.c_int, C.c_void_p, C.c_void_p, C.c_void_p, C.c_double, C.c_double,
                                  C.c_uint64, C.c_int, C.c_void_p]),
diff --git a/vimure_amd/csrc/sorted_lists.hip b/vimure_amd/csrc/sorted_lists.hip
--- a/vimure_amd/csrc/sorted_lists.hip
+++ b/vimure_amd/csrc/sorted_lists.hip
@@ -119,7 +119,7 @@
   for (int l = 0; l < L; ++l) {
     unsigned* rpl = rp + (size_t)l * n;
     unsigned* rsl = h->rs + (size_t)l * (NS + 1);
-    const bool by_level = level_keys_ok && (double)nl[l] > (double)SL_PF * (double)T;
+    const bool by_level = level_keys_ok && ((double)nl[l] > (double)SL_PF * (double)T || (g.K == 2 && !g.det && !h->opt.no_level0));
     const int nb = by_level ? bits : 0;
     int rc;
     hipLaunchKernelGGL(k_sl_keys, dim3(tgrid), dim3(256), 0, h->stream, rpl, keys, vals, T);
diff --git a/vimure_amd/csrc/sweep_sl.h b/vimure_amd/csrc/sweep_sl.h
--- a/vimure_amd/csrc/sweep_sl.h
+++ b/vimure_amd/csrc/sweep_sl.h
@@ -40,6 +40,7 @@
   const unsigned* Ez;
   int elbo_cur;
   const double* lpd; const double* lpb;
+  int k2s;
 #ifdef SL_DEBUG
   unsigned long long* dbg_t;
 #endif
diff --git a/vimure_amd/csrc/sweep_sl.hip b/vimure_amd/csrc/sweep_sl.hip
--- a/vimure_amd/csrc/sweep_sl.hip
+++ b/vimure_amd/csrc/sweep_sl.hip
@@ -29,17 +29,21 @@
   return fma(fma(-d, r, 1.0), r, r);
 }
 #define SL_INL __attribute__((always_inline))
+#ifndef SL_K2S_BT
+#define SL_K2S_BT 4
+#endif
 #ifndef SL_BATCH2
 #define SL_BATCH2 8
 #endif
 template <int K> struct Batch { static constexpr int value = K <= 2 ? SL_BATCH2 : (K <= 4 ? 4 : 2); };
 
-template <int K, bool UPDATE, bool ELBO, bool ALLFULL, bool STORE = true, bool DET = false, bool LPD = false>
+template <int K, bool UPDATE, bool ELBO, bool ALLFULL, bool STORE = true, bool DET = false, bool LPD = false, bool LOCK = false>
 __device__ __forceinline__ void sweep_body(const SlArgs& a, const Geo& g, const unsigned bx, const unsigned gx) {
   extern __shared__ __align__(16) unsigned char smem[];
   constexpr int PFK = sl_pf(K);
   constexpr bool LV0 = !UPDATE && !ELBO && !DET;
   constexpr bool LV0R = UPDATE && K >= 3;
+  constexpr bool K2S = K == 2 && UPDATE && !ELBO && !DET && !LOCK;
   const int tid = threadIdx.x, lane = tid & 63, nthr = (int)blockDim.x;
   const int wv = __builtin_amdgcn_readfirstlane(tid >> 6), nw = nthr >> 6;
   const int Mp = g.Mp;
@@ -67,11 +71,13 @@
   const long long NS = (long long)((T + 63) / 64);
   const double gnu = a.par[o.sc + ((UPDATE || a.elbo_cur) ? SC_G_NU : SC_G_NU_STALE)];
   bool gz = false;
+  double gth_min = 1.0, lth_max = 0.0;
   for (int m = tid; m < Mp; m += nthr) {
     const double gv = a.par[o.G_th + (size_t)l * Mp + m];
     Gth[m] = gv;
     if (LV0 || LV0R) gz = gz || (m < g.M && gv == 0.0);
     if (UPDATE) Lth[m] = a.par[o.l_th + (size_t)l * Mp + m];
+    if (K2S && m < g.M) { gth_min = fmin(gth_min, gv); lth_max = fmax(lth_max, fabs(Lth[m])); }
   }
   for (int q = tid; q < nHc; q += nthr) Hc[q] = 0.0;
   if (a.sum_a) for (int q = tid; q < Mp * K; q += nthr) As[q] = 0.0;
@@ -86,6 +92,15 @@
   double Ela[K], Gla[K], Lla[K];
 #pragma unroll
   for (int k = 0; k < K; ++k) { Ela[k] = a.par[o.E_la + l * K + k]; Gla[k] = a.par[o.G_la + l * K + k]; Lla[k] = a.par[o.l_la + l * K + k]; if (LV0 || LV0R) gz = gz || Gla[k] == 0.0; }
+  if (K2S) {
+#pragma unroll
+    for (int k = 0; k < K; ++k) gz = gz || !(gth_min * Gla[k] > 0.0);
+    if (a.k2s) {
+#pragma unroll
+      for (int o2 = 32; o2 > 0; o2 >>= 1) lth_max = fmax(lth_max, __shfl_xor(lth_max, o2, 64));
+      if (lane == 0) red[wv] = lth_max;
+    }
+  }
   const double eps = g.eps;
   const double sc_h = DET ? __builtin_amdgcn_ldexp(1.0, g.det_sh) : 0.0, sc_r = DET ? __builtin_amdgcn_ldexp(1.0, g.det_shr) : 0.0;
   const double sc_a = DET ? __builtin_amdgcn_ldexp(1.0, DET_SH_A) : 0.0;
@@ -141,6 +156,7 @@
   long long s = step_of((unsigned)wv), sn = step_of((unsigned)(nw + wv));
   unsigned ea = 0;
   int R = 0;
+  int Re = 0;
   unsigned ymax = 0;
   unsigned rgv = 0;
   StepIn<K> P;
@@ -163,7 +179,7 @@
     }
     if (ELBO && Ql) d.qt = *at_bytes(Ql + row0, lane4);
     d.x0 = 0u;
-    if (LV0 && a.x0p) d.x0 = *at_bytes(a.x0p + (size_t)l * NS * 64 + row0, lane4);
+    if ((LV0 || K2S) && a.x0p) d.x0 = *at_bytes(a.x0p + (size_t)l * NS * 64 + row0, lane4);
 #pragma unroll
     for (int k = 0; k < K; ++k) { d.v[k] = 0.0; d.w[k] = 0.0; }
     if (LPDV) {
@@ -197,8 +213,16 @@
 #endif
   __builtin_amdgcn_s_waitcnt(0x0F70);
   bool lv0_off = false;
-  if (LV0 || LV0R) lv0_off = __syncthreads_or(gz ? 1 : 0) != 0;
+  if (LV0 || LV0R || K2S) lv0_off = __syncthreads_or(gz ? 1 : 0) != 0;
   else __syncthreads();
+  const bool k2s_on = K2S && a.k2s != 0 && !lv0_off;
+  double Bth = 0.0;
+  if (K2S && a.k2s) {
+    for (int w = 0; w < nw; ++w) Bth = fmax(Bth, red[w]);
+    Bth = readlane_f64(Bth, 0);
+  }
+  auto eff_rounds = [&](int Rr, unsigned sy_word) SL_INL -> int { return k2s_on ? min(Rr, (int)(sy_word >> 16)) : Rr; };
+  Re = eff_rounds(R, ymax);
 #ifdef SL_DEBUG
   if (dbt && lane == 0) dbt[5] = wall_clock64();
 #endif
@@ -300,7 +324,7 @@
     return (SL_INR(ent) ? inner : 0.0) + eps;
   };
   auto walk1_near = [&](const unsigned* e, auto npc, double (&U)[K]) SL_INL {
-    constexpr int NP = decltype(npc)::value, BT = Batch<K>::value;
+    constexpr int NP = decltype(npc)::value, BT = (K2S && Batch<K>::value > SL_K2S_BT) ? SL_K2S_BT : Batch<K>::value;
 #pragma unroll
     for (int j0 = 0; j0 < NP; j0 += BT) {
       double f[BT][K];
@@ -354,7 +378,7 @@
   auto deficit = [&](unsigned ent, double dfc) SL_INL {
     lds_add(&Hc[SL_YM(ent)], (double)SL_X(ent) * dfc, sc_h);
   };
-  auto compute = [&](auto rct, const StepIn<K>& cur, const size_t row0, const bool act, const unsigned ea_c, const int Rr, const unsigned sy_word) SL_INL {
+  auto compute = [&](auto rct, const StepIn<K>& cur, const size_t row0, const bool act, const unsigned ea_c, const int Rr, const unsigned sy_word, const int Rfull) SL_INL {
     const unsigned ymax = sy_word & 0xffffu, nf = a.farl ? sy_word >> 16 : 0x7fffffffu;
     const unsigned n1 = (LV0 && a.h0s && !lv0_off) ? sy_word >> 16 : 0x7fffffffu;
     constexpr int RCT = decltype(rct)::value;
@@ -391,6 +415,8 @@
     if (UPDATE || ELBO) Tt = mask_sum(cls, tie);
     double dfc = 0.0;
     bool irr = false;
+    bool sc = K2S && RCT >= 0 && k2s_on, slow = false;
+    const double x0d = sc ? (double)cur.x0 : 0.0;
 
     if (UPDATE) {
       double U[K];
@@ -451,10 +477,31 @@
       bool done = false;
       if (K == 2) {
         double c[K];
-#pragma unroll
-        for (int k = 0; k < K; ++k) c[k] = fma(-Tt, Ela[k], U[k]);
-        const double d = ((LPDV ? cur.v[0] : cur.v[K - 1] - cur.v[0]) + c[K - 1]) - c[0];
-        bool safe = fabs(c[0]) + lpb0 < 700.0 && fabs(c[K - 1]) + lpb1 < 700.0 && fabs(d) < 700.0;
+        double d = 0.0;
+        bool safe = true;
+        if (K2S && sc) {
+#pragma unroll
+          for (int k = 0; k < K; ++k) c[k] = fma(-Tt, Ela[k], fma(Lla[k], x0d, U[k]));
+          d = ((LPDV ? cur.v[0] : cur.v[K - 1] - cur.v[0]) + c[K - 1]) - c[0];
+          const double bx0 = x0d * Bth;
+          safe = fabs(c[0]) + bx0 + lpb0 < 700.0 && fabs(c[K - 1]) + bx0 + lpb1 < 700.0 && fabs(d) < 700.0;
+          if (!__all(safe)) {
+#pragma nounroll
+            for (int j = NP; j < Rfull; ++j) {
+              const unsigned e = *at_bytes(pe, lane4 + (unsigned)j * 256u);
+              const double dx = (double)SL_X(e);
+#pragma unroll
+              for (int k = 0; k < K; ++k) U[k] = fma(dx, F[SL_YM(e) * K + k], U[k]);
+            }
+            sc = false; slow = true;
+          }
+        }
+        if (!(K2S && sc)) {
+#pragma unroll
+          for (int k = 0; k < K; ++k) c[k] = fma(-Tt, Ela[k], U[k]);
+          d = ((LPDV ? cur.v[0] : cur.v[K - 1] - cur.v[0]) + c[K - 1]) - c[0];
+          safe = fabs(c[0]) + lpb0 < 700.0 && fabs(c[K - 1]) + lpb1 < 700.0 && fabs(d) < 700.0;
+        }
         if (!__all(safe)) {
           double v[K];
 #pragma unroll
@@ -509,6 +556,10 @@
         for (int k = 0; k < K; ++k) { if (DET) iaccF[k] += fxm(r[k], sc_a); else accF[k] += r[k]; }
       }
       if (!ALLFULL && a.sum_a) add_lists(tie, act && cls == 2u, r);
+      if (K2S && sc && a.h0s && act) {
+#pragma unroll
+        for (int k = 1; k < K; ++k) acc0[k] = fma(r[k], x0d, acc0[k]);
+      }
     } else if (a.do_hist) {
       double sm = 0.0;
 #pragma unroll
@@ -536,6 +587,15 @@
         if (irr) {
 #pragma unroll
           for (int j = 0; j < NP; ++j) deficit(cur.e[j], dfc);
+        }
+        if (K2S && slow && a.do_hist) {
+#pragma nounroll
+          for (int j = NP; j < Rfull; ++j) {
+            const unsigned e = *at_bytes(pe, lane4 + (unsigned)j * 256u);
+#pragma unroll
+            for (int k = 1; k < K; ++k) lds_add(&Hc[(unsigned)k * hcm + SL_YM(e)], (double)SL_X(e) * r[k], sc_h);
+            if (irr) deficit(e, dfc);
+          }
         }
       } else {
         const bool skip0 = LV0 && a.x0p != nullptr && a.do_hist == 1 && n1 != 0x7fffffffu && !irr;
@@ -608,9 +668,18 @@
     const unsigned ea2 = more ? (unsigned)__builtin_amdgcn_readlane((int)rgv, 0) : ea_c;
     const int R2 = more ? (int)(((unsigned)__builtin_amdgcn_readlane((int)rgv, 1) - ea2) >> 6) : 0;
     const unsigned ym2 = more ? (unsigned)__builtin_amdgcn_readlane((int)rgv, 2) : 0u;
+    const int Re2 = eff_rounds(R2, ym2);
     fetch_range(s3 < NS ? s3 : s);
-    fetch_tie(P, more ? s2 : s, RCT == 0 && a.lp0 != 0);
+    fetch_tie(P, more ? s2 : s, RCT == 0 && (!K2S || R == 0) && a.lp0 != 0);
     if (RCT >= 0 || PFK <= 8) fetch_ent(P, ea2, RC<NP>{});
+    if (K2S && RCT >= 0 && NP < PFK) {
+      const bool gen2 = Re2 > SL_PF || (ym2 & 0xffffu) >= lim_y;
+      if ((gen2 ? PFK : Re2) > NP) {
+        const unsigned* pe2 = El + ea2;
+#pragma unroll
+        for (int j = NP; j < PFK; ++j) P.e[j] = *at_bytes(pe2 + j * 64, lane4);
+      }
+    }
     else {
       const unsigned* pe = El + ea2;
 #pragma unroll
@@ -621,20 +690,20 @@
         }
       }
     }
-    compute(rct, cur, row0, act, ea_c, Rr, ymax);
+    compute(rct, cur, row0, act, ea_c, Rr, ymax, R);
     constexpr int NST = (UPDATE && STORE) ? (K % 2 == 0 ? K / 2 : K) : 0;
     static_assert(NST <= 8, "vmcnt immediate below");
     if (RCT >= 0) __builtin_amdgcn_s_waitcnt(0x0F70 | NST);
     else __builtin_amdgcn_s_waitcnt(0x0F70);
-    s = s2; sn = s3; ea = ea2; R = R2; ymax = ym2;
+    s = s2; sn = s3; ea = ea2; R = R2; ymax = ym2; Re = Re2;
   };
   auto run = [&](auto rct) SL_INL {
     constexpr int RCT = decltype(rct)::value;
-    do { body(rct); } while (s < NS && R == RCT && (ymax & 0xffffu) < lim_y);
+    do { body(rct); } while (s < NS && Re == RCT && (ymax & 0xffffu) < lim_y);
   };
   while (s < NS) {
-    if (R > SL_PF || (ymax & 0xffffu) >= lim_y) { body(RC<-1>{}); continue; }
-    switch (R) {
+    if (Re > SL_PF || (ymax & 0xffffu) >= lim_y) { body(RC<-1>{}); continue; }
+    switch (Re) {
       case 0: run(RC<0>{}); break;
       case 1: run(RC<1>{}); break;
       case 2: run(RC<2>{}); break;
@@ -793,7 +862,7 @@
       if (tid == 0) atomicAdd(&a.slotF[((size_t)l * NSLOT + (gb % NSLOT)) * K + k], v);
     }
   }
-  if (LV0 && a.h0s && a.do_hist == 1) {
+  if ((LV0 || K2S) && a.h0s && a.do_hist == 1) {
 #pragma unroll
     for (int k = 1; k < K; ++k) {
       const double v = block_sum_n(acc0[k], red);
@@ -828,7 +897,7 @@
 template <int K, bool UPDATE, bool ELBO, bool ALLFULL, bool STORE = true, bool LPD = false>
 __global__ __launch_bounds__(sl_tpb_max_b(K, ELBO, ALLFULL), sl_wpe_b(K, ELBO, ALLFULL)) void k_sweep_sl_b(const SlUnit* __restrict__ units, const int* __restrict__ blk_unit) {
   const SlUnit& u = units[blk_unit[blockIdx.x]];
-  sweep_body<K, UPDATE, ELBO, ALLFULL, STORE, false, LPD>(u.a, u.g, blockIdx.x - (unsigned)u.blk0, (unsigned)u.nblk);
+  sweep_body<K, UPDATE, ELBO, ALLFULL, STORE, false, LPD, true>(u.a, u.g, blockIdx.x - (unsigned)u.blk0, (unsigned)u.nblk);
 }
 
 template <bool UPDATE, bool ELBO, bool ALLFULL, bool STORE = true, bool DET = false, bool LPD = false>
diff --git a/vimure_amd/csrc/vimure_hip.hip b/vimure_amd/csrc/vimure_hip.hip
--- a/vimure_amd/csrc/vimure_hip.hip
+++ b/vimure_amd/csrc/vimure_hip.hip
@@ -1597,7 +1597,13 @@
 static SlArgs sl_args(const vmr_ctx* h, const SlShape& sh, int do_hist, int sum_a = 0) {
   return SlArgs{h->E, h->rs, h->ebase, h->perm, h->sy, h->cls_p, h->Qt_p, h->Rb, h->rq, h->Rm, h->rbase, h->rm2, h->rho, h->logpr, h->par, h->slotR,
                 h->lutg, h->Hg, h->slotF, h->slotA, 1, do_hist, sh.yt, sh.hc, sum_a, nullptr, nullptr, 0, 0, nullptr, h->lp0 ? 1 : 0, h->g.farl, (do_hist == 1 && h->g.two_pass && sh.hc >= 1) ? h->h0s : nullptr, (do_hist == 1 && h->g.two_pass && sh.hc >= 1 && h->h0s) ? h->x0p : nullptr,
-                (h->h0s && h->g.two_pass && !h->opt.no_lv0r) ? 1 : 0, h->E + h->n_slots, 0, h->lpd, h->lpb};
+                (h->h0s && h->g.two_pass && !h->opt.no_lv0r) ? 1 : 0, h->E + h->n_slots, 0, h->lpd, h->lpb, 0};
+}
+static void sl_take_k2s(const vmr_ctx* h, const SlShape& sh, SlArgs& a) {
+  if (!h->k2s || a.det || sh.yt != h->g.Y || (a.do_hist && sh.hc != h->g.Y)) return;
+  a.k2s = 1;
+  a.x0p = h->x0p;
+  a.h0s = a.do_hist == 1 ? h->h0s : nullptr;
 }
 static int sl_launch(vmr_ctx* h, int mode, const SlShape& sh, SlArgs& a) {
   sl_launch_fn fn = vmr_sl_launcher(h->g.K);
@@ -1642,7 +1648,7 @@
   if (v) atomicAdd(out, v);
 }
 __global__ __launch_bounds__(256) void k_far_first(unsigned* __restrict__ E, const unsigned* __restrict__ rsl, unsigned* __restrict__ syl, size_t NS, unsigned rows_near,
-                                                   unsigned* __restrict__ x0) {
+                                                   unsigned* __restrict__ x0, int tail_only) {
   const int lane = threadIdx.x & 63;
   for (size_t s = (size_t)blockIdx.x * 4 + (threadIdx.x >> 6); s < NS; s += (size_t)gridDim.x * 4) {
     const unsigned ea = rsl[s], R = (rsl[s + 1] - ea) >> 6;
@@ -1656,9 +1662,13 @@
         ++f;
       } else xs += SL_X(e);
     }
+#pragma unroll
+    for (int o2 = 32; o2 > 0; o2 >>= 1) f = max(f, (unsigned)__shfl_xor((int)f, o2, 64));
+    if (x0 && tail_only) {
+      xs = 0;
+      for (unsigned r = f; r < R; ++r) xs += SL_X(col[(size_t)r * 64]);
+    }
     if (x0) x0[s * 64 + (unsigned)lane] = xs;
-#pragma unroll
-    for (int o2 = 32; o2 > 0; o2 >>= 1) f = max(f, (unsigned)__shfl_xor((int)f, o2, 64));
     if (lane == 0) syl[s] = (syl[s] & 0xffffu) | (min(f, 0xffffu) << 16);
   }
 }
@@ -1892,6 +1902,7 @@
   SlArgs as = sl_args(h, shs, 0, 0);
   as.slotF = nullptr; as.slotA = nullptr;
   as.nu_stale = h->g.mut ? 1 : 0;
+  sl_take_k2s(h, shs, as);
   int rc = sl_launch(h, 0, shs, as);
   if (rc) return rc;
   HIPCHK(h, hipGetLastError());
@@ -2056,11 +2067,16 @@
     SlArgs as = sl_args(h, shs, do_hist, sum_a);
     if (nu_in_pass && do_hist) { as.nu_acc = h->nu_acc; as.elbo_dev = h->elbo_dev; as.commit_nu = commit_nu ? 1 : 0; }
     as.det = g.det ? h->det_buf : nullptr;
+    if (mode == 0) sl_take_k2s(h, shs, as);
     const bool lazy = !store && mode == 0 && do_hist && (nu_in_pass ? commit_nu : !g.mut) && g.fuse_full && (h->n_partial == 0 || g.ml) &&
                       !g.farl && !h->opt.always_store_rho;
     {
       Prof p(h, lazy ? VMR_KERNEL_RHO_NOSTORE : mode == 2 ? VMR_KERNEL_ELBO : mode == 1 ? VMR_KERNEL_RHO_ELBO : VMR_KERNEL_RHO);
       if ((rc = sl_launch(h, lazy ? 4 : mode, shs, as))) return rc;
+    }
+    if (as.k2s && as.h0s) {
+      hipLaunchKernelGGL(k_level0_spread, dim3(g.L), dim3(256), 0, h->stream, h->Hg, h->Cg, h->h0s, g);
+      HIPCHK(h, hipGetLastError());
     }
     if (mode != 2) h->rho_stale = lazy;
     if (g.farl && do_hist && (rc = launch_far(h, 0, nu_in_pass ? (commit_nu ? 1 : 0) : -1))) return rc;
@@ -2330,7 +2346,7 @@
   CK(hipMemcpy(eb.data(), h->ebase, (size_t)g.L * 8, hipMemcpyDeviceToHost));
   for (int l = 0; l < g.L; ++l) {
     hipLaunchKernelGGL(k_far_first, dim3((unsigned)std::min<size_t>(8192, (NS + 3) / 4)), dim3(256), 0, h->stream, h->E + eb[l], h->rs + (size_t)l * (NS + 1),
-                       h->sy + (size_t)l * NS, NS, (unsigned)g.hc * (unsigned)g.Mp, (unsigned*)nullptr);
+                       h->sy + (size_t)l * NS, NS, (unsigned)g.hc * (unsigned)g.Mp, (unsigned*)nullptr, 0);
     CK(hipGetLastError());
     CK(hipMemsetAsync(cnt, 0, 8, h->stream));
     hipLaunchKernelGGL(k_far_collect, dim3((unsigned)std::min<size_t>(8192, (NS + 3) / 4)), dim3(256), 0, h->stream, h->E + eb[l], h->rs + (size_t)l * (NS + 1), NS,
@@ -2510,14 +2526,17 @@
     if (o.tpb >= 64 && o.tpb <= 1024 && o.tpb % 64 == 0) h->sp_tpb = o.tpb;
     if (o.st_tpb >= 64 && o.st_tpb <= 1024 && o.st_tpb % 64 == 0) h->st_tpb = o.st_tpb;
     for (int v = 0; v < 4; ++v) need = std::max(need, sl_shape(h, v != 3, v == 1 || v == 2, v == 0 || v == 1 || v == 3).smem);
-    if (g.two_pass && g.mut && !g.det && g.Y > 1 && !o.no_level0) {
+    const bool lv0_k2 = !g.two_pass && !g.farl && K == 2 && g.mut && !g.det && g.Y > 1 && g.yt == g.Y && g.hc == g.Y && !o.no_level0 &&
+                        !o.no_level_sort && !o.no_x0;
+    if ((g.two_pass && g.mut && !g.det && g.Y > 1 && !o.no_level0) || lv0_k2) {
       const size_t T_ = (size_t)g.N * g.N, NS_ = (T_ + 63) / 64;
       std::vector<unsigned long long> eb(L);
       CK(hipMemcpy(eb.data(), h->ebase, (size_t)L * 8, hipMemcpyDeviceToHost));
       if (!o.no_x0) CK(hipMalloc(&h->x0p, (size_t)L * NS_ * 64 * 4));
+      h->k2s = lv0_k2;
       for (int l = 0; l < L; ++l)
         hipLaunchKernelGGL(k_far_first, dim3((unsigned)std::min<size_t>(8192, (NS_ + 3) / 4)), dim3(256), 0, h->stream, h->E + eb[l], h->rs + (size_t)l * (NS_ + 1),
-                           h->sy + (size_t)l * NS_, NS_, (unsigned)g.Mp, h->x0p ? h->x0p + (size_t)l * NS_ * 64 : nullptr);
+                           h->sy + (size_t)l * NS_, NS_, (unsigned)g.Mp, h->x0p ? h->x0p + (size_t)l * NS_ * 64 : nullptr, lv0_k2 ? 1 : 0);
       CK(hipGetLastError());
       if (h->x0p) {
         unsigned long long* ss = nullptr;
@@ -3841,6 +3860,15 @@
   return VMR_OK;
 }
 
+int vmr_level0_shape(vmr_handle h, int* plain_sweeps_skip, uint64_t* rounds, uint64_t* rounds_skipped) {
+  if (!h) return VMR_EINVAL;
+  const bool on = h->k2s && h->x0p && h->h0s;
+  if (plain_sweeps_skip) *plain_sweeps_skip = on ? 1 : 0;
+  if (rounds) *rounds = h->sparse ? (uint64_t)(h->n_slots / 64) : 0ull;
+  if (rounds_skipped) *rounds_skipped = on ? (uint64_t)((h->n_slots - h->stat_slots) / 64) : 0ull;
+  return VMR_OK;
+}
+
 int vmr_kernel_bytes(vmr_handle h, int kernel_class, double* bytes) {
   if (!h || !bytes) return VMR_EINVAL;
   const Geo& g = h->g;
@@ -3851,14 +3879,15 @@
     const double E = (g.wide ? 8.0 : 4.0) * (double)h->nnz, RP = 4.0 * (ties / 64.0 + g.L);
     const double mask = h->all_full ? 0.0 : ties + (h->rq ? 4.0 * ties + 2.0 * (double)h->n_rm : (double)h->n_partial * g.W * 8.0);
     const double Q = g.mut ? 4.0 * ties : 0.0;
+    const double Ek2 = 4.0 * (double)h->stat_slots + 4.0 * ties;
     const double Slp = h->lpd ? 8.0 * ties : Srho;
     switch (kernel_class) {
       case VMR_KERNEL_GAMMA_MASK: *bytes = ties + (h->rq ? 4.0 * ties + 2.0 * (double)h->n_rm : (double)h->n_partial * g.W * 8.0) + Srho; break;
       case VMR_KERNEL_GAMMA_COUNTS:
         *bytes = ((h->x0p && g.two_pass) ? 4.0 * (double)h->stat_slots + 4.0 * ties : E) + RP + Srho;
         break;
-      case VMR_KERNEL_RHO: *bytes = E + RP + mask + Slp + Srho; break;
-      case VMR_KERNEL_RHO_NOSTORE: *bytes = E + RP + mask + Slp; break;
+      case VMR_KERNEL_RHO: *bytes = (h->k2s ? Ek2 : E) + RP + mask + Slp + Srho; break;
+      case VMR_KERNEL_RHO_NOSTORE: *bytes = (h->k2s ? Ek2 : E) + RP + mask + Slp; break;
       case VMR_KERNEL_ELBO: *bytes = E + RP + mask + Q + 2.0 * Srho; break;
       case VMR_KERNEL_RHO_ELBO: *bytes = E + RP + mask + Q + 2.0 * Srho; break;
       default: *bytes = 0.0; break;
diff --git a/vimure_amd/csrc/vmr_internal.h b/vimure_amd/csrc/vmr_internal.h
--- a/vimure_amd/csrc/vmr_internal.h
+++ b/vimure_amd/csrc/vmr_internal.h
@@ -120,6 +120,7 @@
   double* h0s = nullptr;
   unsigned long long stat_slots = 0;
   unsigned* x0p = nullptr;
+  bool k2s = false;
   bool elbo_split = false;
   uint8_t* cls_p = nullptr;
   unsigned* Qt_p = nullptr;
diff --git a/vimure_amd/engine.py b/vimure_amd/engine.py
--- a/vimure_amd/engine.py
+++ b/vimure_amd/engine.py
@@ -527,6 +527,11 @@
         self._check(self.lib.vmr_sweep_shape(self._h, C.byref(p), C.byref(lv), C.byref(n)))
         return int(p.value), int(lv.value), int(n.value)
 
+    def level0_shape(self):
+        on, n, k = C.c_int(), C.c_uint64(), C.c_uint64()
+        self._check(self.lib.vmr_level0_shape(self._h, C.byref(on), C.byref(n), C.byref(k)))
+        return bool(on.value), int(n.value), int(k.value)
+
     def profile(self, enable=True):
         self._check(self.lib.vmr_profile(self._h, int(enable)))
 
```
